# HarborYuan/PolyphonicFormer

Hardware: AMD Instinct MI355X
Metric: frames/sec kernel-update+mask fwd, 1024x2048 N=153 S=3 (higher is better)
Workload: dtype bf16 (feature planes as given; query side: updator half hi/lo bf16, attention / FFN / towers one fp16 plane; one fp16 plane of dynamic kernels, fp16 logits); 1 GPU; cfg2: KernelUpdateIterHead.simple_test_mask_preds, 1024x2048, stride-8 128x256, N=153, S=3, L=133, random-init weights; hip_graph=True, streams=4, feature_input_dtype=bf16, mask_logit_input_dtype=float16, output_dtype=torch.float16, parallelism=frames sharded over 1 GPU(s), no data-path collective

## Files before the change

include/polyhead.h:

```cpp
#ifndef POLYHEAD_H_
#define POLYHEAD_H_

#include <stddef.h>
#include <stdint.h>

#ifdef __cplusplus
extern "C" {
#endif

#define PH_VERSION 100

enum { PH_OK = 0, PH_EINVAL = -1, PH_EUNSUPPORTED = -2, PH_ELAUNCH = -3, PH_EWORKSPACE = -4 };
enum { PH_PREC_BF16 = 1, PH_PREC_BF16_KSPLIT = 2, PH_PREC_SPLIT = 3, PH_PREC_F16 = 5, PH_PREC_BF16_KF16 = 6, PH_PREC_QHYBRID = 7 };
enum { PH_PLANES_C16 = 0x100 };
enum { PH_OUT_F32 = 0, PH_OUT_BF16 = 1, PH_OUT_F16 = 2 };
enum { PH_KERN_BF16_PLANES = 0, PH_KERN_F16 = 1 };
enum { PH_GN_TO_PLANES = 0, PH_GN_UP2_PLANES = 1, PH_GN_ACCUM = 2, PH_GN_TO_NCHW = 3, PH_GN_TO_CPLANES = 4 };
enum { PH_IN_F32_NCHW = 0, PH_IN_PLANES = 1 };

#define PH_C 256
#define PH_HEADS 8

int         ph_version(void);
const char* ph_last_error_string(void);

enum {
    PH_SWITCH_CONV_WGS = 0,
    PH_SWITCH_UP2_WGS = 1,
    PH_SWITCH_QUERY_NRT = 2,
    PH_SWITCH_QUERY_TIMELINE = 3,
    PH_SWITCH_CONV_TILE_ROWS = 4,
    PH_SWITCH_GNSUM_WGS = 5,
    PH_SWITCH_CPLANES_TPW = 6,
    PH_SWITCH_PAN_GENERIC = 7,
    PH_SWITCH_COUNT = 8
};
int ph_set_switch(int id, int value);
int ph_get_switch(int id, int* value);

static inline int64_t ph_hw_padded(int64_t hw) { return (hw + 127) / 128 * 128; }
static inline int     ph_n_padded(int n) { return (n + 31) / 32 * 32; }

int ph_ingest_features(const float* src, uint16_t* planes, int B, int64_t HW, int prec, void* stream);

int ph_binarize(const float* logits, int64_t logits_batch_stride , uint32_t* bits,
                int B, int N, int64_t HW, void* stream);
int ph_binarize_if(const void* logits, int dtype, int64_t logits_batch_stride, uint32_t* bits, int B, int N, int64_t HW,
                   const uint32_t* run_if , void* stream);

int ph_pool(const uint16_t* xplanes, const uint16_t* dplanes, const uint32_t* bits, float* partial,
            int B, int N, int64_t HW, int nsplit, int prec, void* stream);
int ph_pool_rows(const uint16_t* xplanes, const uint16_t* dplanes, const uint32_t* bits, int bits_rows, float* partial,
                 int B, int N, int64_t HW, int nsplit, int prec, void* stream);
int ph_pool_counts(const uint16_t* xplanes, const uint16_t* dplanes, const uint32_t* bits, float* partial, int32_t* pcount,
                   int B, int N, int64_t HW, int nsplit, int prec, void* stream);
int ph_pool_default_nsplit(int B, int64_t HW, int frame_invariant);

enum {
    PH_W_DYN = 0,
    PH_W_INP,
    PH_W_IG,
    PH_W_UG,
    PH_W_FC,
    PH_W_QKV,
    PH_W_OUT,
    PH_W_FFN1,
    PH_W_FFN2,
    PH_W_H0A,
    PH_W_H0B,
    PH_W_CLS,
    PH_W_KERN,
    PH_W_COUNT
};
enum {
    PH_V_DYN_CNT = 0,
    PH_V_DYN_B, PH_V_INP_B, PH_V_IG_B, PH_V_UG_B,
    PH_V_LN_IG_G, PH_V_LN_IG_B,
    PH_V_LN_UG_G, PH_V_LN_UG_B,
    PH_V_LN_PO_G, PH_V_LN_PO_B,
    PH_V_LN_IO_G, PH_V_LN_IO_B,
    PH_V_FC_B, PH_V_LN_FC_G, PH_V_LN_FC_B,
    PH_V_QKV_B, PH_V_OUT_B, PH_V_LN_ATT_G, PH_V_LN_ATT_B,
    PH_V_FFN1_B, PH_V_FFN2_B, PH_V_LN_FFN_G, PH_V_LN_FFN_B,
    PH_V_LN_H0A_G, PH_V_LN_H0A_B, PH_V_LN_H0B_G, PH_V_LN_H0B_B,
    PH_V_CLS_B, PH_V_KERN_B,
    PH_V_COUNT
};
typedef struct {
    int64_t w[2][PH_W_COUNT];
    int64_t v[2][PH_V_COUNT];
    int64_t wb_plane_elems;
    int32_t ffn_dim;
    int32_t num_classes;
} ph_stage_layout;

enum { PH_QUERY_PRE = 1, PH_QUERY_POST = 2, PH_QUERY_BOTH = 3, PH_QUERY_WIDE = 0x100 };
size_t ph_query_workspace_bytes(int B, int N, int prec);
size_t ph_query_workspace_updator_offset(int B, int N, int prec);
int ph_query_stage(const float* partial, int nsplit, const uint32_t* bits,
                   const float* k_in, const float* q_in,
                   const uint16_t* wb, const float* wf, const ph_stage_layout* layout,
                   float* obj, float* dobj, float* cls, int cls_sigmoid ,
                   uint16_t* kern, float* kbias,
                   void* workspace, size_t workspace_bytes,
                   int B, int N, int64_t HW, int prec ,
                   int kern_format ,
                   int phases, void* stream);
int ph_query_stage_counts(const float* partial, int nsplit, const uint32_t* bits, const int32_t* pcount, const float* k_in,
                          const float* q_in, const uint16_t* wb, const float* wf, const ph_stage_layout* layout,
                          float* obj, float* dobj, float* cls, int cls_sigmoid, uint16_t* kern, float* kbias,
                          void* workspace, size_t workspace_bytes, int B, int N, int64_t HW, int prec, int kern_format,
                          int phases, void* stream);

int ph_dynconv(const uint16_t* planes, const uint16_t* kern, int64_t kern_plane_stride, int64_t kern_batch_stride,
               const float* kbias, int64_t kbias_batch_stride, uint32_t* bits_out, void* logits_out, int out_dtype,
               int64_t out_batch_stride, int B, int N, int64_t HW, int prec, void* stream);

int ph_upsample2x(const void* src, void* dst, int dtype, int64_t planes , int H, int W, void* stream);

int ph_dynconv_up2_supported(int N, int H, int W, int prec, int out_dtype);
int ph_dynconv_up2(const uint16_t* planes, const uint16_t* kern, int64_t kern_batch_stride, const float* kbias,
                   int64_t kbias_batch_stride, void* logits_out , void* up_out, int out_dtype, int B, int N, int H,
                   int W, int prec, void* stream);
int ph_dynconv_up2_wgs(const uint16_t* planes, const uint16_t* kern, int64_t kern_batch_stride, const float* kbias,
                       int64_t kbias_batch_stride, void* logits_out , void* up_out, int out_dtype, int B, int N, int H,
                       int W, int prec, int workgroups, void* stream);

int ph_dynconv_poolx_supported(int N, int prec);
int ph_dynconv_poolx(const uint16_t* planes, const uint16_t* kern, int64_t kern_batch_stride, const float* kbias,
                     int64_t kbias_batch_stride, uint32_t* bits_out, float* partial, int nsplit, int B, int N, int64_t HW, int prec,
                     void* stream);

size_t ph_khead_workspace_bytes(int B, int64_t HW, int groups);
int ph_khead_conv_gn(const float* f0, const float* f1, const float* f2, const uint16_t* wplanes,
                     const float* gn_affine, int groups, float eps,
                     uint16_t* loc_planes, uint16_t* sem_planes, uint16_t* x_planes, uint16_t* dfe_planes,
                     float* x_f32 , float* dfe_f32 ,
                     void* workspace, size_t workspace_bytes, int B, int64_t HW, int prec, void* stream);
int ph_khead_fused(const void* f0, const void* f1, const void* f2, const uint16_t* wplanes,
                   const float* gn_affine, int groups, float eps,
                   const uint16_t* w2_init, int n_init, const uint16_t* w2_seg, const float* bias_seg, int n_seg,
                   const uint16_t* w2_dd, const float* bias_dd, int stuff_lo, int n_stuff,
                   uint16_t* x_planes, uint16_t* dfe_planes, float* x_f32 , float* dfe_f32 ,
                   float* mask_preds, float* seg_preds, float* depth_pred,
                   void* workspace, size_t workspace_bytes, int B, int64_t HW, int prec, int input_format, void* stream);
int ph_khead_fused_if(const void* f0, const void* f1, const void* f2, const uint16_t* wplanes,
                      const float* gn_affine, int groups, float eps,
                      const uint16_t* w2_init, int n_init, const uint16_t* w2_seg, const float* bias_seg, int n_seg,
                      const uint16_t* w2_dd, const float* bias_dd, int stuff_lo, int n_stuff,
                      uint16_t* x_planes, uint16_t* dfe_planes, float* x_f32 , float* dfe_f32 ,
                      void* mask_preds, void* seg_preds, void* depth_pred, int logits_dtype, const uint32_t* run_if ,
                      void* workspace, size_t workspace_bytes, int B, int64_t HW, int prec, int input_format, void* stream);
int ph_khead_onepass_supported(int B, int64_t HW, int groups, int prec, int input_format);
size_t ph_khead_onepass_workspace_bytes(int B, int64_t HW);
int ph_khead_onepass(const void* f0, const void* f1, const void* f2, const uint16_t* conv_frags,
                     const float* gn_affine, int groups, float eps,
                     const uint16_t* w2_init, int n_init, const uint16_t* w2_seg, const float* bias_seg, int n_seg,
                     const uint16_t* w2_dd, const float* bias_dd, int stuff_lo, int n_stuff,
                     uint16_t* x_planes, uint16_t* dfe_planes, float* x_f32 , float* dfe_f32 ,
                     void* mask_preds, void* seg_preds, void* depth_pred, int out_dtype,
                     uint32_t* bits , int bits_rows,
                     void* workspace, size_t workspace_bytes, int B, int64_t HW, int prec, int input_format, void* stream);
int ph_khead_onepass_status(const void* workspace, int B, void* stream);
int ph_khead_onepass_timeouts(const void* workspace, int B, int64_t HW, void* stream);
void ph_khead_onepass_set_timeout_us(int microseconds );
void ph_khead_onepass_set_timeline(void* buf);
int ph_khead_proposals(const float* partial, int nsplit, const float* w_init ,
                       const float* w_stuff , float* proposal_feats,
                       int B, int n_thing_queries, int n_stuff, void* stream);

int64_t ph_match_record_floats(int N, int G);
int ph_match_nsplit(int64_t HW, int B);
int ph_match_sums(const float* logits, const float* gt, const float* valid, float* partial, int B, int N, int G,
                  int64_t HW, void* stream);

int ph_mask_loss_sums(const float* pred, const float* target, const float* weight, const int32_t* pos_rows, int P, int64_t HW,
                      int nsplit, double* out, void* stream);
int ph_mask_loss_grad(const float* pred, const float* target, const float* weight, const int32_t* pos_rows, int P, int64_t HW,
                      const float* coef, float* grad, void* stream);
int ph_rank_loss_blocks(int64_t HW);
int ph_rank_loss_sum(const float* pred, const int32_t* rank_target, int B, int N, int64_t HW, int ignore_index, double* out,
                     void* stream);
int ph_rank_loss_grad(const float* pred, const int32_t* rank_target, int B, int N, int64_t HW, int ignore_index, float scale,
                      float* grad, void* stream);
int ph_depth_loss_blocks(int64_t total);
int ph_depth_loss_sums(const float* pred, const float* target, const float* weight, int64_t total, int depth_mode, double* out,
                       void* stream);
int ph_depth_loss_grad(const float* pred, const float* target, const float* weight, int64_t total, int depth_mode, float c0,
                       float c1, float c2, float c3, float* grad, void* stream);
int ph_focal_loss_blocks(int64_t total);
int ph_focal_loss_sum(const float* pred, const int64_t* labels, const float* weight, int64_t R, int L, float gamma, float alpha,
                      double* out, void* stream);
int ph_focal_loss_grad(const float* pred, const int64_t* labels, const float* weight, int64_t R, int L, float gamma, float alpha,
                       float scale, float* grad, void* stream);
int ph_seg_focal_sum(const float* pred, const int32_t* target, int B, int L, int64_t HW, float gamma, float alpha, double* out,
                     void* stream);
int ph_seg_focal_grad(const float* pred, const int32_t* target, int B, int L, int64_t HW, float gamma, float alpha, float scale,
                      float* grad, void* stream);

int ph_rank_target(const float* mask_targets, const uint8_t* pos, int B, int N, int64_t HW, int ignore_index, int32_t* out,
                   void* stream);
int ph_seg_target(const float* sem_seg, const int64_t* sem_cls, int S, const float* pos_masks, const int64_t* pos_labels, int P,
                  int L, int64_t HW, int64_t* out, void* stream);

int ph_depth_cost_sums(const float* depth_logits, const float* gt_depth, const float* gt_masks, int N, int G, int64_t HW,
                       int depth_mode, float eps, float* out, float* nvalid, void* stream);

int ph_rows_x_map(const float* A, int64_t a_batch_stride, int lda, int Mpad, int M, int K, const float* X, float* Y, int B, int64_t HW,
                  int binarize_x, void* stream);
int ph_map_x_map_t_nsplit(int B, int M, int64_t HW);
int ph_map_x_map_t(const float* G, const float* X, float* partial, float* out, int B, int M, int K, int64_t HW, int nsplit,
                  int binarize_g, void* stream);
int ph_upsample2x_bwd(const float* grad_out, float* grad_in, int64_t planes, int H, int W, void* stream);
int ph_rows_x_map_ex(const float* A, int64_t a_batch_stride, int lda, int Mpad, int M, int K, const float* X, float* Y, int B,
                     int64_t HW, int binarize_x, const float* bias, const float* add, void* stream);
int ph_map_x_map_t_ex(const float* G, const float* X, float* partial, float* out, int B, int M, int K, int64_t HW, int nsplit,
                      int binarize_g, float* rs_partial, float* rowsum, int sum_batch, void* stream);
int ph_conv3x3_taps(const float* W, float* taps, int M, int K, int transpose, int flip, int to_weight, void* stream);
int ph_conv3x3_train(const float* taps, int M, int K, const float* X, float* Y, int B, int Hi, int Wi, int Ho, int Wo, int stride,
                     int mode, void* stream);
int ph_conv3x3_wgrad(const float* dY, const float* X, float* partial, float* taps_out, int B, int M, int K, int Hi, int Wi, int Ho,
                     int Wo, int stride, int nsplit, void* stream);
int ph_gn_train_nsplit(int64_t HW, int cpg);
int ph_gn_train_bwd_nsplit(int64_t HW);
int ph_gn_train_fwd(const float* y, const float* gamma, const float* beta, int groups, float eps, const float* add, float* out,
                    float* out_sum, float* stats, double* partial, int B, int C, int64_t HW, void* stream);
int ph_gn_train_bwd(const float* y, const float* stats, const float* gamma, const float* beta, int groups, const float* dyA,
                    const float* dyB, float* dx, float* dgamma, float* dbeta, double* partial, int B, int C, int64_t HW, void* stream);
int ph_hard_count(const float* logits, float* out, int64_t rows, int64_t HW, void* stream);
int ph_map_x_map_t_wide_nsplit(int B, int M, int K, int64_t HW);
int ph_map_x_map_t_wide(const float* G, const float* X, float* partial, float* out, int B, int M, int K, int64_t HW, int nsplit,
                        float* rs_partial, float* rowsum, int sum_batch, void* stream);
int ph_nearest_up_add(float* fine, const float* coarse, int64_t planes, int H, int W, int Hc, int Wc, void* stream);
int ph_nearest_up_add_bwd(const float* g_fine, float* g_coarse, int64_t planes, int H, int W, int Hc, int Wc, int accumulate,
                          void* stream);
int ph_nchw_bias_add(float* y, const float* bias, int B, int C, int64_t HW, void* stream);
int ph_nchw_channel_sums_nsplit(int64_t HW);
int ph_nchw_channel_sums(const float* g, double* partial, float* out, int B, int C, int64_t HW, void* stream);

typedef struct {
    int32_t B, N, L, P, depth_rows, seg_L, has_rank, ignore, depth_mode;
    int64_t HW;
    float lw_mask, lw_dice, dice_eps, lw_rank, lw_depth, dw_si, dw_sq, dw_abs, lw_cls, cls_gamma, cls_alpha, cls_avg, lw_seg, seg_gamma,
        seg_alpha;
} ph_loss_cfg;
size_t ph_train_losses_scratch_bytes(const ph_loss_cfg* cfg);
int ph_train_losses(const ph_loss_cfg* cfg, const float* mask_pred, const float* cls_score, const float* depth_pred,
                    const float* seg_pred, const int32_t* pos_rows, const uint8_t* pos_u8, const int64_t* tptr, const int64_t* wptr,
                    const int32_t* dstart, const int64_t* dit_t, const int64_t* dit_w, const float* dit_s, const int64_t* labels,
                    const float* label_w, const int32_t* sstart, const int64_t* sit_m, const int32_t* sit_l, float* losses,
                    float* g_mask, float* g_cls, float* g_depth, float* g_seg, void* scratch, size_t scratch_bytes, void* stream);

int ph_gemm32(const float* A, int lda, int kcA, const float* B, int ldb, int kcB, float* C, int ldc, int M, int N, int K, int ksplit,
              const float* bias, void* stream);
#define PH_QTRAIN_NPARAM 44
size_t ph_qtrain_saved_floats(int B, int N, int L, int F);
size_t ph_qtrain_scratch_floats(int B, int N, int L, int F);
int ph_qtrain_forward(const float* const* params, const float* pooled, const float* cnt, const float* k, const float* q, float* cls,
                      float* kern, float* kbias, float* obj, float* saved, int B, int N, int L, int F, void* stream);
int ph_qtrain_backward(const float* const* params, const float* pooled, const float* cnt, const float* k, const float* q,
                       const float* saved, const float* g_cls, const float* g_kern, const float* g_kbias, const float* g_obj,
                       float* const* grads, float* g_pooled, float* g_k, float* g_q, float* scratch, int B, int N, int L, int F,
                       void* stream);

int ph_panoptic_select(const float* cls_scores, int64_t cls_batch_stride, int B, int N, int L, int num_proposals,
                       int num_thing_classes, int max_per_img, int32_t* q_idx, int32_t* labels, float* scores,
                       int64_t out_batch_stride, void* stream);
int ph_panoptic_activate(const void* mask_up, const void* depth_up, int dtype, const float* depth_init_up,
                         const int32_t* q_idx, int K, int h2, int w2, int depth_mode ,
                         float* act_mask, float* act_depth, float* act_depth0, void* stream);
int ph_panoptic_argmax(const float* act_mask, const float* scores, int K, const int32_t* geom, int from_probs,
                       int32_t* ids, int32_t* counts , void* stream);
int ph_panoptic_paste(const int32_t* ids, const int32_t* newid, const float* act_depth, const float* act_depth0,
                      const int32_t* geom, int from_probs, int32_t* pan, float* depth_basic, float* depth_final,
                      void* stream);

int ph_panoptic_accept(const int32_t* labels, const float* scores, const int32_t* counts , int64_t in_batch_stride, int B,
                       int K, int num_thing_classes, double instance_score_thr, double overlap_thr, int32_t* newid,
                       int64_t newid_batch_stride, int32_t* nseg, int32_t* seg , int64_t rec_batch_stride, void* stream);
int ph_panoptic_activate_batch(const void* mask_up, const void* depth_up, int dtype, const float* depth_init_up,
                               const int32_t* q_idx, int64_t q_batch_stride, int B, int N, int K, int h2, int w2, int depth_mode,
                               float* act_mask, float* act_depth, float* act_depth0, void* stream);
int ph_panoptic_argmax_batch(const float* act_mask, const float* scores, int64_t scores_batch_stride, int B, int K,
                             const int32_t* geom, int from_probs, int generic_only, int32_t* ids, int32_t* counts,
                             int64_t counts_batch_stride, void* stream);
int ph_panoptic_paste_batch(const int32_t* ids, const int32_t* newid, int64_t newid_batch_stride, const float* act_depth,
                            const float* act_depth0, int B, int K, const int32_t* geom, int from_probs, int32_t* pan,
                            float* depth_basic, float* depth_final, void* stream);
size_t ph_panoptic_merge_workspace_bytes(int B, int K, int h2, int w2, const int32_t* geom);
int ph_panoptic_merge(const float* cls , const void* mask_up, const void* depth_up, int dtype,
                      const float* depth_init_up , int B, int N, int L, int num_proposals, int num_thing_classes,
                      int max_per_img, int h2, int w2, const int32_t* geom , int depth_mode,
                      double instance_score_thr, double overlap_thr, void* workspace, size_t workspace_bytes,
                      int32_t* pan , float* depth_basic, float* depth_final,
                      int32_t* seg_records , void* stream);

size_t ph_segment_boxes_workspace_bytes(int nseg);
int ph_segment_boxes(const int32_t* pan, int H, int W, int nseg, float* rois, float* ext_boxes,
                     void* workspace, size_t workspace_bytes, void* stream);
int ph_roi_align_fpn(const float* const* feats, const int32_t* hw, const float* scales, int nlev, const float* rois,
                     int n, float finest_scale, uint16_t* out_cl, float* out_f32 , int prec, void* stream);
int ph_gemm_rows(const uint16_t* X, const uint16_t* Wp, int64_t w_plane_elems, const float* bias , int relu,
                 float* Yf , uint16_t* Yp , int M, int N, int K, int prec, void* stream);
int ph_im2col7(const uint16_t* in, uint16_t* out, int n, int prec, void* stream);
size_t ph_gemm_rows_workspace_bytes(int M, int N, int K);
int ph_gemm_rows_splitk(const uint16_t* X, int im2col7, const uint16_t* Wp, int64_t w_plane_elems, const float* bias ,
                        int relu, float* Yf , uint16_t* Yp , int M, int N, int K, int prec,
                        void* workspace, size_t workspace_bytes, void* stream);
size_t ph_track_affinity_workspace_bytes(int n, int m);
int ph_track_affinity(const float* emb, const int32_t* labels, const float* memo_emb, const int32_t* memo_labels, int n, int m,
                      int metric, int with_cats, float* score, void* workspace, size_t workspace_bytes, void* stream);
int ph_gn_relu_cl(const float* y, const float* gamma, const float* beta, int groups, float eps, uint16_t* out, int n,
                  int prec, void* stream);

int ph_nhwc_ingest(const float* src, const float* add , uint16_t* dst, int B, int64_t HW, int prec, void* stream);
size_t ph_conv_nhwc_partial_floats(int B, int Ho, int Wo);
int ph_conv_nhwc_workgroups_b(int ksize, int stride, int Ho, int Wo, int prec, int B);
int ph_conv_nhwc(const uint16_t* X, const uint16_t* Wp, int64_t w_plane_elems, float* Y, float* partial, int ksize, int stride,
                 int B, int H, int W, int prec, void* stream);
int ph_gn_finalize(const float* partial, float* stats, int nwg, int groups, int64_t HW, float eps, int B, void* stream);
int ph_gn_sum_planes(const float* const* ys, const float* const* stats, const float* const* gammas, const float* const* betas,
                     int nlev, int groups, uint16_t* planes, int B, int64_t HW, int prec, void* stream);
size_t ph_neck_out_convs_workspace_bytes(int B, int64_t HW, int groups);
int ph_neck_out_convs(const uint16_t* in_planes, int in_channels_last, const uint16_t* wplanes, const float* gn_affine, int groups,
                      float eps, uint16_t* out_planes0, uint16_t* out_planes1, uint16_t* out_planes2, float* out_f32_0,
                      float* out_f32_1, float* out_f32_2, void* workspace, size_t workspace_bytes, int B, int64_t HW, int prec,
                      void* stream);
int ph_gn_apply(const float* y, const float* stats , const float* gamma, const float* beta, int groups, int mode,
                int accumulate, uint16_t* planes , float* outf , int B, int H, int W, int prec,
                void* stream);

int ph_fpn_lateral(const void* x, int x_dtype, const uint16_t* Wp, int64_t w_plane_elems, const float* bias,
                   const uint16_t* coarse , int Hc, int Wc, uint16_t* out, int B, int K, int H, int W, int prec,
                   void* stream);
int ph_fpn_output(const float* y, const float* bias, float* out, int B, int64_t HW, void* stream);
int ph_fpn_output_planes(const float* y, const float* bias, const float* add , uint16_t* planes,
                         float* out_f32 , int B, int64_t HW, int prec , void* stream);

typedef struct {
    float init_score_thr, obj_score_thr, match_score_thr, memo_momentum, one_minus_momentum, nms_conf_thr, nms_backdrop_iou_thr,
        nms_class_iou_thr;
    int32_t memo_tracklet_frames, memo_backdrop_frames, with_cats, metric;
} ph_tracker_cfg;
typedef struct ph_tracker ph_tracker;
size_t ph_tracker_device_bytes(int capacity, int max_dets);
ph_tracker* ph_tracker_create(const ph_tracker_cfg* cfg, void* device_mem, size_t device_bytes, int capacity, int max_dets);
void ph_tracker_destroy(ph_tracker* t);
void ph_tracker_reset(ph_tracker* t);
int64_t ph_tracker_num_tracklets(const ph_tracker* t);
int ph_tracker_rows(const ph_tracker* t);
void ph_tracker_debug_times(const ph_tracker* t, double* out6);
int ph_tracker_match(ph_tracker* t, const float* boxes, const int64_t* labels, const float* embeds_dev, int n, int64_t frame_id,
                     int32_t* kept_out, int64_t* ids_out, void* stream);
int ph_tracker_match_frames(ph_tracker* t, const float* boxes, const int64_t* labels, const float* const* embeds_dev, const int32_t* counts,
                            int nframes, int64_t first_frame_id, int32_t* kept_out, int64_t* ids_out, int32_t* kept_counts, void* stream);

enum { PH_MODE_FP32 = 0, PH_MODE_MIXED = 1, PH_MODE_MIXED16 = 2, PH_MODE_FP16 = 3, PH_MODE_BF16 = 4 };
enum { PH_KNOB_AUTO = 0, PH_KNOB_ON = 1, PH_KNOB_OFF = 2, PH_KNOB_WHERE_SUPPORTED = 3 };
typedef struct {
    int32_t B, N, H, W;
    int32_t S;
    int32_t L;
    int32_t F;
    int32_t mode;
    int32_t out_dtype;
    int32_t frame_invariant;
    int32_t query_full_split;
    int32_t shares_gpu;
    int32_t poolx;
    int32_t fused_up;
    int32_t nsplit;
    int32_t nsplit_px;
    int32_t up2_wgs;
} ph_decode_cfg;

typedef struct {
    int32_t nsplit, nsplit_px, poolx, fused_up;
    int32_t up2_workgroups;
    int32_t feat_prec, query_prec, conv_prec, kern_format;
    int32_t feat_planes;
} ph_decode_geometry;

enum { PH_FEAT_F32 = 0, PH_FEAT_16 = 1, PH_FEAT_PLANES = 2 };
typedef struct {
    int32_t feat_format;
    int32_t m0_dtype;
    const void* x;
    const void* depth_feats;
    const float* k0;
    const float* q0;
    const void* m0;
    const uint32_t* bits;
    float* obj;
    float* dobj;
    float* cls;
    void* mask;
    void* mask_up;
    void* depth_up;
    void* depth;
// ... 452 lines not shown
```

polyphonicformer_amd/_lib.py:

```python
import contextlib
import ctypes as C
import os

import torch

from . import knobs

HERE = os.path.dirname(os.path.abspath(__file__))
LIB_PATH = os.path.join(HERE, "libpolyhead.so")
if knobs.get("PH_ALT_LIB"):
    LIB_PATH = os.path.abspath(knobs.get("PH_ALT_LIB"))

PH_PREC_BF16, PH_PREC_BF16_KSPLIT, PH_PREC_SPLIT, PH_PREC_F16, PH_PREC_BF16_KF16, PH_PREC_QHYBRID = 1, 2, 3, 5, 6, 7
PH_PLANES_C16 = 0x100
PH_QUERY_WIDE = 0x100
PH_OUT_F32, PH_OUT_BF16, PH_OUT_F16 = 0, 1, 2
PH_KERN_BF16_PLANES, PH_KERN_F16 = 0, 1
PH_GN_TO_PLANES, PH_GN_UP2_PLANES, PH_GN_ACCUM, PH_GN_TO_NCHW, PH_GN_TO_CPLANES = 0, 1, 2, 3, 4
PH_IN_F32_NCHW, PH_IN_PLANES = 0, 1

SWITCHES = ("conv_wgs", "up2_wgs", "query_nrt", "query_timeline", "conv_tile_rows", "gnsum_wgs", "cplanes_tpw", "pan_generic")

W_NAMES = ["DYN", "INP", "IG", "UG", "FC", "QKV", "OUT", "FFN1", "FFN2", "H0A", "H0B", "CLS", "KERN"]
V_NAMES = ["DYN_CNT", "DYN_B", "INP_B", "IG_B", "UG_B", "LN_IG_G", "LN_IG_B", "LN_UG_G", "LN_UG_B",
           "LN_PO_G", "LN_PO_B", "LN_IO_G", "LN_IO_B", "FC_B", "LN_FC_G", "LN_FC_B", "QKV_B", "OUT_B",
           "LN_ATT_G", "LN_ATT_B", "FFN1_B", "FFN2_B", "LN_FFN_G", "LN_FFN_B", "LN_H0A_G", "LN_H0A_B",
           "LN_H0B_G", "LN_H0B_B", "CLS_B", "KERN_B"]
W_IDX = {n: i for i, n in enumerate(W_NAMES)}
V_IDX = {n: i for i, n in enumerate(V_NAMES)}


class StageLayout(C.Structure):
    _fields_ = [("w", (C.c_int64 * len(W_NAMES)) * 2), ("v", (C.c_int64 * len(V_NAMES)) * 2),
                ("wb_plane_elems", C.c_int64), ("ffn_dim", C.c_int32), ("num_classes", C.c_int32)]


PH_MODE = {"fp32": 0, "split": 0, "mixed": 1, "mixed16": 2, "fp16": 3, "bf16": 4}
PH_KNOB_AUTO, PH_KNOB_ON, PH_KNOB_OFF, PH_KNOB_WHERE_SUPPORTED = 0, 1, 2, 3
PH_FEAT_F32, PH_FEAT_16, PH_FEAT_PLANES = 0, 1, 2
PH_DECODE_NPARAMS = 83


class DecodeCfg(C.Structure):
    _fields_ = [(n, C.c_int32) for n in ("B", "N", "H", "W", "S", "L", "F", "mode", "out_dtype", "frame_invariant", "query_full_split",
                                          "shares_gpu", "poolx", "fused_up", "nsplit", "nsplit_px", "up2_wgs")]


class DecodeGeometry(C.Structure):
    _fields_ = [(n, C.c_int32) for n in ("nsplit", "nsplit_px", "poolx", "fused_up", "up2_workgroups", "feat_prec", "query_prec",
                                          "conv_prec", "kern_format", "feat_planes")]


class DecodeIO(C.Structure):
    _fields_ = [("feat_format", C.c_int32), ("m0_dtype", C.c_int32)] + \
        [(n, C.c_void_p) for n in ("x", "depth_feats", "k0", "q0", "m0", "bits", "obj", "dobj", "cls", "mask", "mask_up", "depth_up",
                                   "depth")]


PH_KHEAD_NPARAMS = 14
KPACK_PIECES = ("wplanes", "gn", "init_planes", "seg_planes", "dd_planes", "seg_bias", "dd_bias", "init_frag", "seg_frag", "dd_frag",
                "conv_frag", "w_init_f32", "w_seg_f32", "w_dd_f32")
PH_KPACK_COUNT = len(KPACK_PIECES)


class KheadCfg(C.Structure):
    _fields_ = [(n, C.c_int32) for n in ("B", "H", "W", "num_proposals", "num_classes", "num_thing_classes", "cat_stuff", "groups",
                                          "mode", "logit_dtype", "emit_f32", "frame_invariant", "onepass", "nsplit")]


class KheadLayout(C.Structure):
    _fields_ = [("offset", C.c_uint64 * PH_KPACK_COUNT), ("bytes", C.c_uint64 * PH_KPACK_COUNT)]


class KheadGeometry(C.Structure):
    _fields_ = [(n, C.c_int32) for n in ("onepass", "nsplit", "N", "Npad", "HWp", "P", "prec", "n_stuff")]


class KheadIO(C.Structure):
    _fields_ = [("input_format", C.c_int32), ("reserved", C.c_int32)] + \
        [(n, C.c_void_p) for n in ("f0", "f1", "f2", "xp", "dp", "bits", "x_f32", "dfe_f32", "mask_preds", "seg_preds", "depth_pred",
                                   "proposal", "depth_proposal")]


PH_NECK_NPARAMS = 30
PH_NECK_NCONVS = 10
PH_NPACK_OUTS_W, PH_NPACK_OUTS_GN, PH_NPACK_COUNT = 30, 31, 32


class NeckCfg(C.Structure):
    _fields_ = [("B", C.c_int32), ("h", C.c_int32 * 4), ("w", C.c_int32 * 4)] + \
        [(n, C.c_int32) for n in ("groups", "mode", "num_outs", "pos_level", "emit_planes", "emit_f32", "fused_out", "c16",
                                  "tower_buffers")] + [("eps", C.c_float)]


class NeckLayout(C.Structure):
    _fields_ = [("offset", C.c_uint64 * PH_NPACK_COUNT), ("bytes", C.c_uint64 * PH_NPACK_COUNT)]


class NeckGeometry(C.Structure):
    _fields_ = [(n, C.c_int32) for n in ("Ho", "Wo", "HWp", "P", "prec", "fused_out", "c16", "tower_buffers", "nconvs")] + \
        [("tile_rows", C.c_int32 * PH_NECK_NCONVS)]


class NeckIO(C.Structure):
    _fields_ = [("feats", C.c_void_p * 4), ("posenc", C.c_void_p), ("out_planes", C.c_void_p * 3), ("out_f32", C.c_void_p * 3)]


PH_FPN_NPARAMS = PH_FPACK_COUNT = 16


class FpnCfg(C.Structure):
    _fields_ = [("B", C.c_int32), ("k", C.c_int32 * 4), ("h", C.c_int32 * 4), ("w", C.c_int32 * 4)] + \
        [(n, C.c_int32) for n in ("mode", "x_dtype", "emit_f32", "emit_planes")]


class FpnLayout(C.Structure):
    _fields_ = [("offset", C.c_uint64 * PH_FPACK_COUNT), ("bytes", C.c_uint64 * PH_FPACK_COUNT)]


class FpnGeometry(C.Structure):
    _fields_ = [("P", C.c_int32), ("prec", C.c_int32), ("tile_rows", C.c_int32 * 4)]


class FpnIO(C.Structure):
    _fields_ = [("stages", C.c_void_p * 4), ("out_f32", C.c_void_p * 4), ("out_planes", C.c_void_p * 4), ("planes_layout", C.c_int32 * 4),
                ("add", C.c_void_p * 4)]


PH_TRACK_MAX_CONVS = 8
PH_TPACK_FC, PH_TPACK_FC_B, PH_TPACK_EMB, PH_TPACK_EMB_B, PH_TPACK_COUNT = 24, 25, 26, 27, 28


class TrackCfg(C.Structure):
    _fields_ = [(n, C.c_int32) for n in ("num_convs", "fc_out_channels", "embed_channels", "groups", "prec")] + [("eps", C.c_float)]


class TrackLayout(C.Structure):
    _fields_ = [("offset", C.c_uint64 * PH_TPACK_COUNT), ("bytes", C.c_uint64 * PH_TPACK_COUNT)]


class AssocCfg(C.Structure):
    _fields_ = [(n, C.c_int32) for n in ("B", "Ho", "Wo", "K", "max_things", "num_thing_classes", "num_stuff_classes", "nlev")] + \
        [("h", C.c_int32 * 4), ("w", C.c_int32 * 4), ("inv_stride", C.c_float * 4), ("finest_scale", C.c_float), ("track", TrackCfg)]


class AssocGeometry(C.Structure):
    _fields_ = [(n, C.c_int32) for n in ("things_words", "P", "conv_splits", "conv_steps", "fc_splits", "fc_steps", "emb_splits",
                                          "emb_steps", "vec8", "reserved")] + [(n, C.c_uint64) for n in ("staging_bytes", "rois_offset", "roi_planes_offset")]


class AssocIO(C.Structure):
    _fields_ = [("pan", C.c_void_p), ("seg_records", C.c_void_p), ("levels", C.c_void_p * 4), ("level_stride", C.c_int64 * 4),
                ("sem_out", C.c_void_p), ("things_out", C.c_void_p), ("embeds_out", C.c_void_p), ("roi_planes", C.c_void_p)]


PH_DTRK_OK, PH_DTRK_EPOOL, PH_DTRK_EREFUSED, PH_DTRK_ECOUNT = 0, 1, 2, 3
DTRK_STATUS = ("matched", "num_tracklets", "rows", "error", "refused_frame", "frame_id", "free", "frames_seen")
PH_DTRK_ST_WORDS = len(DTRK_STATUS)


class TrackerCfg(C.Structure):
    _fields_ = [(n, C.c_float) for n in ("init_score_thr", "obj_score_thr", "match_score_thr", "memo_momentum", "one_minus_momentum",
                                         "nms_conf_thr", "nms_backdrop_iou_thr", "nms_class_iou_thr")] + \
        [(n, C.c_int32) for n in ("memo_tracklet_frames", "memo_backdrop_frames", "with_cats", "metric")]


class DtrackerLayout(C.Structure):
    _fields_ = [(n, C.c_uint64) for n in ("pool", "trk_id", "trk_seen", "trk_label", "trk_slot", "trk_box", "bd_count", "bd_label", "bd_slot",
                                          "bd_box", "free_stack", "status", "workspace", "total_bytes")] + \
        [(n, C.c_int32) for n in ("capacity", "max_dets", "generations", "reserved")]


class DtrackerIO(C.Structure):
    _fields_ = [("boxes", C.c_void_p), ("box_stride", C.c_int64), ("labels", C.c_void_p), ("label_stride", C.c_int64),
                ("counts", C.c_void_p), ("count_stride", C.c_int64), ("refuse", C.c_void_p), ("refuse_stride", C.c_int64),
                ("embeds", C.c_void_p), ("embed_stride", C.c_int64), ("kept_out", C.c_void_p), ("ids_out", C.c_void_p),
                ("kept_counts", C.c_void_p)]


PH_DVPQ_MAX_THR = 8


class DvpqCfg(C.Structure):
    _fields_ = [(n, C.c_int32) for n in ("B", "H", "W", "capacity", "nthr")] + [("thr", C.c_float * PH_DVPQ_MAX_THR)]


class DvpqIO(C.Structure):
    _fields_ = [(n, C.c_void_p) for n in ("pred_panseg", "pred_sem", "pred_track", "pred_depth", "gt_panseg", "gt_depth", "table_out",
                                          "depth_out")]


PH_ASSIGN_MAX, PH_ASSIGN_MAX_B, PH_ASSIGN_GT_WORDS = 256, 64, 8
PH_ASSIGN_OK, PH_ASSIGN_ENONFINITE, PH_ASSIGN_ESOLVE = 0, 1, 2
PH_EUNSUPPORTED = -2
ASSIGN_SECTIONS = ("tptr", "wptr", "labels", "pos_u8", "pos_rows", "dstart", "dit_t", "dit_w", "dit_s", "label_w", "sstart", "sit_m", "sit_l")


class AssignCfg(C.Structure):
    _fields_ = [(n, C.c_int32) for n in ("B", "Np", "N", "L", "n_thing", "n_stuff", "roi", "has_sem", "has_depth")] + \
        [("pos_weight", C.c_float), ("HW", C.c_int64)]


class AssignLayout(C.Structure):
    _fields_ = [(n, C.c_uint64) for n in ASSIGN_SECTIONS + ("total_bytes",)] + \
        [(n, C.c_int64) for n in ("P", "depth_items", "seg_items", "depth_rows")]


class LossCfg(C.Structure):
    _fields_ = [(n, C.c_int32) for n in ("B", "N", "L", "P", "depth_rows", "seg_L", "has_rank", "ignore", "depth_mode")] + \
        [("HW", C.c_int64)] + \
        [(n, C.c_float) for n in ("lw_mask", "lw_dice", "dice_eps", "lw_rank", "lw_depth", "dw_si", "dw_sq", "dw_abs", "lw_cls",
                                  "cls_gamma", "cls_alpha", "cls_avg", "lw_seg", "seg_gamma", "seg_alpha")]


PH_TRACK_LOSS_MAX_ROIS, PH_TRACK_LOSS_MAX_PAIRS = 128, 64


PH_GTBOX_MAX_FRAMES, PH_GTBOX_BILINEAR, PH_GTBOX_NEAREST = 64, 0, 1
PH_GTPREP_MAX_FRAMES, PH_GTPREP_MAX_SEGMENTS = 64, 254
PH_GTSEG_MAX_KEYS, PH_GTSEG_ROW_WORDS, PH_GTSEG_TABLE_WORDS = 262144, 6, 1 + 254 * 6
PH_GTSEG_I32, PH_GTSEG_U16 = 0, 1
PH_GTSEG_ETOOMANY, PH_GTSEG_EUNMAPPED, PH_GTSEG_EOUTSIDE = 1, 2, 4
PH_EINVAL, PH_EWORKSPACE = -1, -4
PH_IMGPREP_MAX_FRAMES = 64
PH_IMG_NCHW, PH_IMG_NHWC = 0, 1


class TrackLossCfg(C.Structure):
    _fields_ = [("pairs", C.c_int32), ("E", C.c_int32), ("lw_track", C.c_float), ("lw_aux", C.c_float), ("neg_pos_ub", C.c_int32),
                ("pos_margin", C.c_float), ("neg_margin", C.c_float), ("hard_mining", C.c_int32)]


PH_OPTIM_CHUNK, PH_OPTIM_MAX_TENSORS = 4096, 4096
PH_OPTIM_SKIP_NONFINITE, PH_OPTIM_ZERO_GRADS = 1, 2
PH_OPTIM_OK, PH_OPTIM_ENONFINITE = 0, 1


class OptimTensor(C.Structure):
    _fields_ = [(n, C.c_void_p) for n in ("p", "g", "m", "v")] + [("n", C.c_int64), ("lr", C.c_double), ("weight_decay", C.c_double),
                                                                  ("first_item", C.c_int64)]


class OptimCfg(C.Structure):
    _fields_ = [(n, C.c_double) for n in ("beta1", "beta2", "eps", "max_norm")] + [("flags", C.c_int32), ("max_blocks", C.c_int32)]


class OptimState(C.Structure):
    _fields_ = [("step", C.c_int64), ("skipped", C.c_int64), ("status", C.c_int32), ("skip", C.c_int32)] + \
        [(n, C.c_float) for n in ("grad_norm", "clip_coef", "bias1", "bias2_sqrt")]


STRUCTS = {"ph_stage_layout": StageLayout, "ph_decode_cfg": DecodeCfg, "ph_decode_geometry": DecodeGeometry, "ph_decode_io": DecodeIO,
           "ph_khead_cfg": KheadCfg, "ph_khead_layout": KheadLayout, "ph_khead_geometry": KheadGeometry, "ph_khead_io": KheadIO,
           "ph_neck_cfg": NeckCfg, "ph_neck_layout": NeckLayout, "ph_neck_geometry": NeckGeometry, "ph_neck_io": NeckIO,
           "ph_fpn_cfg": FpnCfg, "ph_fpn_layout": FpnLayout, "ph_fpn_geometry": FpnGeometry, "ph_fpn_io": FpnIO,
           "ph_track_cfg": TrackCfg, "ph_track_layout": TrackLayout, "ph_assoc_cfg": AssocCfg, "ph_assoc_geometry": AssocGeometry,
           "ph_assoc_io": AssocIO, "ph_tracker_cfg": TrackerCfg, "ph_dtracker_layout": DtrackerLayout, "ph_dtracker_io": DtrackerIO,
           "ph_dvpq_cfg": DvpqCfg, "ph_dvpq_io": DvpqIO, "ph_assign_cfg": AssignCfg, "ph_assign_layout": AssignLayout,
           "ph_loss_cfg": LossCfg, "ph_track_loss_cfg": TrackLossCfg, "ph_optim_tensor": OptimTensor, "ph_optim_cfg": OptimCfg,
           "ph_optim_state": OptimState}

_P, _I, _L, _Z = C.c_void_p, C.c_int, C.c_int64, C.c_size_t
SIGNATURES = {
    "ph_version": (C.c_int, []),
    "ph_last_error_string": (C.c_char_p, []),
    "ph_set_switch": (C.c_int, [_I, _I]),
    "ph_get_switch": (C.c_int, [_I, C.POINTER(C.c_int)]),
    "ph_ingest_features": (C.c_int, [_P, _P, _I, _L, _I, _P]),
    "ph_binarize": (C.c_int, [_P, _L, _P, _I, _I, _L, _P]),
    "ph_pool": (C.c_int, [_P, _P, _P, _P, _I, _I, _L, _I, _I, _P]),
    "ph_pool_rows": (C.c_int, [_P, _P, _P, _I, _P, _I, _I, _L, _I, _I, _P]),
    "ph_pool_counts": (C.c_int, [_P, _P, _P, _P, _P, _I, _I, _L, _I, _I, _P]),
    "ph_pool_default_nsplit": (C.c_int, [_I, _L, _I]),
    "ph_query_workspace_bytes": (C.c_size_t, [_I, _I, _I]),
    "ph_query_stage": (C.c_int, [_P, _I, _P, _P, _P, _P, _P, C.POINTER(StageLayout), _P, _P, _P, _I, _P, _P,
                                 _P, _Z, _I, _I, _L, _I, _I, _I, _P]),
    "ph_query_stage_counts": (C.c_int, [_P, _I, _P, _P, _P, _P, _P, _P, C.POINTER(StageLayout), _P, _P, _P, _I, _P, _P,
                                        _P, _Z, _I, _I, _L, _I, _I, _I, _P]),
    "ph_query_workspace_updator_offset": (C.c_size_t, [_I, _I, _I]),
    "ph_dynconv": (C.c_int, [_P, _P, _L, _L, _P, _L, _P, _P, _I, _L, _I, _I, _L, _I, _P]),
    "ph_khead_workspace_bytes": (C.c_size_t, [_I, _L, _I]),
    "ph_khead_conv_gn": (C.c_int, [_P, _P, _P, _P, _P, _I, C.c_float, _P, _P, _P, _P, _P, _P, _P, _Z, _I, _L, _I, _P]),
    "ph_khead_fused": (C.c_int, [_P, _P, _P, _P, _P, _I, C.c_float, _P, _I, _P, _P, _I, _P, _P, _I, _I, _P, _P, _P, _P,
                                 _P, _P, _P, _P, _Z, _I, _L, _I, _I, _P]),
    "ph_khead_onepass_supported": (C.c_int, [_I, _L, _I, _I, _I]),
    "ph_khead_onepass_workspace_bytes": (C.c_size_t, [_I, _L]),
    "ph_khead_onepass": (C.c_int, [_P, _P, _P, _P, _P, _I, C.c_float, _P, _I, _P, _P, _I, _P, _P, _I, _I, _P, _P, _P, _P,
                                   _P, _P, _P, _I, _P, _I, _P, _Z, _I, _L, _I, _I, _P]),
    "ph_khead_onepass_status": (C.c_int, [_P, _I, _P]),
    "ph_khead_onepass_timeouts": (C.c_int, [_P, _I, _L, _P]),
    "ph_khead_onepass_set_timeout_us": (None, [_I]),
    "ph_khead_fused_if": (C.c_int, [_P, _P, _P, _P, _P, _I, C.c_float, _P, _I, _P, _P, _I, _P, _P, _I, _I, _P, _P, _P, _P,
                                    _P, _P, _P, _I, _P, _P, _Z, _I, _L, _I, _I, _P]),
    "ph_binarize_if": (C.c_int, [_P, _I, _L, _P, _I, _I, _L, _P, _P]),
    "ph_selftest_hog": (C.c_int, [_I, _I, _I, _P, _P]),
    "ph_khead_onepass_set_timeline": (None, [_P]),
    "ph_khead_proposals": (C.c_int, [_P, _I, _P, _P, _P, _I, _I, _I, _P]),
    "ph_match_record_floats": (C.c_int64, [_I, _I]),
    "ph_match_nsplit": (C.c_int, [_L, _I]),
    "ph_match_sums": (C.c_int, [_P, _P, _P, _P, _I, _I, _I, _L, _P]),
    "ph_upsample2x": (C.c_int, [_P, _P, _I, _L, _I, _I, _P]),
    "ph_dynconv_poolx_supported": (C.c_int, [_I, _I]),
    "ph_dynconv_poolx": (C.c_int, [_P, _P, _L, _P, _L, _P, _P, _I, _I, _I, _L, _I, _P]),
    "ph_dynconv_up2_supported": (C.c_int, [_I, _I, _I, _I, _I]),
    "ph_dynconv_up2": (C.c_int, [_P, _P, _L, _P, _L, _P, _P, _I, _I, _I, _I, _I, _I, _P]),
    "ph_dynconv_up2_wgs": (C.c_int, [_P, _P, _L, _P, _L, _P, _P, _I, _I, _I, _I, _I, _I, _I, _P]),
    "ph_mask_loss_sums": (C.c_int, [_P, _P, _P, _P, _I, _L, _I, _P, _P]),
    "ph_mask_loss_grad": (C.c_int, [_P, _P, _P, _P, _I, _L, _P, _P, _P]),
    "ph_rank_loss_blocks": (C.c_int, [_L]),
    "ph_rank_loss_sum": (C.c_int, [_P, _P, _I, _I, _L, _I, _P, _P]),
    "ph_rank_loss_grad": (C.c_int, [_P, _P, _I, _I, _L, _I, C.c_float, _P, _P]),
    "ph_depth_loss_blocks": (C.c_int, [_L]),
    "ph_depth_loss_sums": (C.c_int, [_P, _P, _P, _L, _I, _P, _P]),
    "ph_depth_loss_grad": (C.c_int, [_P, _P, _P, _L, _I, C.c_float, C.c_float, C.c_float, C.c_float, _P, _P]),
    "ph_focal_loss_blocks": (C.c_int, [_L]),
    "ph_focal_loss_sum": (C.c_int, [_P, _P, _P, _L, _I, C.c_float, C.c_float, _P, _P]),
    "ph_focal_loss_grad": (C.c_int, [_P, _P, _P, _L, _I, C.c_float, C.c_float, C.c_float, _P, _P]),
    "ph_seg_focal_sum": (C.c_int, [_P, _P, _I, _I, _L, C.c_float, C.c_float, _P, _P]),
    "ph_seg_focal_grad": (C.c_int, [_P, _P, _I, _I, _L, C.c_float, C.c_float, C.c_float, _P, _P]),
    "ph_rank_target": (C.c_int, [_P, _P, _I, _I, _L, _I, _P, _P]),
    "ph_seg_target": (C.c_int, [_P, _P, _I, _P, _P, _I, _I, _L, _P, _P]),
    "ph_depth_cost_sums": (C.c_int, [_P, _P, _P, _I, _I, _L, _I, C.c_float, _P, _P, _P]),
    "ph_rows_x_map": (C.c_int, [_P, _L, _I, _I, _I, _I, _P, _P, _I, _L, _I, _P]),
    "ph_map_x_map_t_nsplit": (C.c_int, [_I, _I, _L]),
    "ph_map_x_map_t": (C.c_int, [_P, _P, _P, _P, _I, _I, _I, _L, _I, _I, _P]),
    "ph_upsample2x_bwd": (C.c_int, [_P, _P, _L, _I, _I, _P]),
    "ph_rows_x_map_ex": (C.c_int, [_P, _L, _I, _I, _I, _I, _P, _P, _I, _L, _I, _P, _P, _P]),
    "ph_map_x_map_t_ex": (C.c_int, [_P, _P, _P, _P, _I, _I, _I, _L, _I, _I, _P, _P, _I, _P]),
    "ph_conv3x3_taps": (C.c_int, [_P, _P, _I, _I, _I, _I, _I, _P]),
    "ph_conv3x3_train": (C.c_int, [_P, _I, _I, _P, _P, _I, _I, _I, _I, _I, _I, _I, _P]),
    "ph_conv3x3_wgrad": (C.c_int, [_P, _P, _P, _P, _I, _I, _I, _I, _I, _I, _I, _I, _I, _P]),
    "ph_gn_train_nsplit": (C.c_int, [_L, _I]),
    "ph_gn_train_bwd_nsplit": (C.c_int, [_L]),
    "ph_gn_train_fwd": (C.c_int, [_P, _P, _P, _I, C.c_float, _P, _P, _P, _P, _P, _I, _I, _L, _P]),
    "ph_gn_train_bwd": (C.c_int, [_P, _P, _P, _P, _I, _P, _P, _P, _P, _P, _P, _I, _I, _L, _P]),
    "ph_hard_count": (C.c_int, [_P, _P, _L, _L, _P]),
    "ph_map_x_map_t_wide_nsplit": (C.c_int, [_I, _I, _I, _L]),
    "ph_map_x_map_t_wide": (C.c_int, [_P, _P, _P, _P, _I, _I, _I, _L, _I, _P, _P, _I, _P]),
    "ph_nearest_up_add": (C.c_int, [_P, _P, _L, _I, _I, _I, _I, _P]),
    "ph_nearest_up_add_bwd": (C.c_int, [_P, _P, _L, _I, _I, _I, _I, _I, _P]),
    "ph_nchw_bias_add": (C.c_int, [_P, _P, _I, _I, _L, _P]),
    "ph_nchw_channel_sums_nsplit": (C.c_int, [_L]),
    "ph_nchw_channel_sums": (C.c_int, [_P, _P, _P, _I, _I, _L, _P]),
    "ph_train_losses_scratch_bytes": (C.c_size_t, [_P]),
    "ph_train_losses": (C.c_int, [_P] * 24 + [_Z, _P]),
    "ph_gemm32": (C.c_int, [_P, _I, _I, _P, _I, _I, _P, _I, _I, _I, _I, _I, _P, _P]),
    "ph_qtrain_saved_floats": (C.c_size_t, [_I, _I, _I, _I]),
    "ph_qtrain_scratch_floats": (C.c_size_t, [_I, _I, _I, _I]),
    "ph_qtrain_forward": (C.c_int, [_P, _P, _P, _P, _P, _P, _P, _P, _P, _P, _I, _I, _I, _I, _P]),
    "ph_qtrain_backward": (C.c_int, [_P, _P, _P, _P, _P, _P, _P, _P, _P, _P, _P, _P, _P, _P, _P, _I, _I, _I, _I, _P]),
    "ph_panoptic_select": (C.c_int, [_P, _L, _I, _I, _I, _I, _I, _I, _P, _P, _P, _L, _P]),
    "ph_panoptic_activate": (C.c_int, [_P, _P, _I, _P, _P, _I, _I, _I, _I, _P, _P, _P, _P]),
    "ph_panoptic_argmax": (C.c_int, [_P, _P, _I, C.POINTER(C.c_int32), _I, _P, _P, _P]),
    "ph_panoptic_paste": (C.c_int, [_P, _P, _P, _P, C.POINTER(C.c_int32), _I, _P, _P, _P, _P]),
    "ph_panoptic_accept": (C.c_int, [_P, _P, _P, _L, _I, _I, _I, C.c_double, C.c_double, _P, _L, _P, _P, _L, _P]),
    "ph_panoptic_activate_batch": (C.c_int, [_P, _P, _I, _P, _P, _L, _I, _I, _I, _I, _I, _I, _P, _P, _P, _P]),
    "ph_panoptic_argmax_batch": (C.c_int, [_P, _P, _L, _I, _I, C.POINTER(C.c_int32), _I, _I, _P, _P, _L, _P]),
    "ph_panoptic_paste_batch": (C.c_int, [_P, _P, _L, _P, _P, _I, _I, C.POINTER(C.c_int32), _I, _P, _P, _P, _P]),
    "ph_panoptic_merge_workspace_bytes": (C.c_size_t, [_I, _I, _I, _I, C.POINTER(C.c_int32)]),
    "ph_panoptic_merge": (C.c_int, [_P, _P, _P, _I, _P, _I, _I, _I, _I, _I, _I, _I, _I, C.POINTER(C.c_int32), _I, C.c_double,
                                    C.c_double, _P, _Z, _P, _P, _P, _P, _P]),
    "ph_segment_boxes_workspace_bytes": (C.c_size_t, [_I]),
    "ph_segment_boxes": (C.c_int, [_P, _I, _I, _I, _P, _P, _P, _Z, _P]),
    "ph_roi_align_fpn": (C.c_int, [C.POINTER(C.c_void_p), C.POINTER(C.c_int32), C.POINTER(C.c_float), _I, _P, _I, C.c_float,
                                   _P, _P, _I, _P]),
    "ph_gemm_rows": (C.c_int, [_P, _P, _L, _P, _I, _P, _P, _I, _I, _I, _I, _P]),
    "ph_track_affinity_workspace_bytes": (C.c_size_t, [_I, _I]),
    "ph_track_affinity": (C.c_int, [_P, _P, _P, _P, _I, _I, _I, _I, _P, _P, _Z, _P]),
    "ph_im2col7": (C.c_int, [_P, _P, _I, _I, _P]),
    "ph_gemm_rows_workspace_bytes": (C.c_size_t, [_I, _I, _I]),
    "ph_gemm_rows_splitk": (C.c_int, [_P, _I, _P, _L, _P, _I, _P, _P, _I, _I, _I, _I, _P, _Z, _P]),
    "ph_gn_relu_cl": (C.c_int, [_P, _P, _P, _I, C.c_float, _P, _I, _I, _P]),
    "ph_nhwc_ingest": (C.c_int, [_P, _P, _P, _I, _L, _I, _P]),
    "ph_conv_nhwc_partial_floats": (C.c_size_t, [_I, _I, _I]),
    "ph_conv_nhwc_workgroups_b": (C.c_int, [_I, _I, _I, _I, _I, _I]),
    "ph_conv_nhwc": (C.c_int, [_P, _P, _L, _P, _P, _I, _I, _I, _I, _I, _I, _P]),
    "ph_gn_finalize": (C.c_int, [_P, _P, _I, _I, _L, C.c_float, _I, _P]),
    "ph_gn_sum_planes": (C.c_int, [C.POINTER(C.c_void_p), C.POINTER(C.c_void_p), C.POINTER(C.c_void_p), C.POINTER(C.c_void_p),
                                   _I, _I, _P, _I, _L, _I, _P]),
    "ph_neck_out_convs_workspace_bytes": (C.c_size_t, [_I, _L, _I]),
    "ph_neck_out_convs": (C.c_int, [_P, _I, _P, _P, _I, C.c_float, _P, _P, _P, _P, _P, _P, _P, _Z, _I, _L, _I, _P]),
    "ph_gn_apply": (C.c_int, [_P, _P, _P, _P, _I, _I, _I, _P, _P, _I, _I, _I, _I, _P]),
    "ph_fpn_lateral": (C.c_int, [_P, _I, _P, _L, _P, _P, _I, _I, _P, _I, _I, _I, _I, _I, _P]),
    "ph_fpn_output": (C.c_int, [_P, _P, _P, _I, _L, _P]),
    "ph_fpn_output_planes": (C.c_int, [_P, _P, _P, _P, _P, _I, _L, _I, _P]),
    "ph_tracker_device_bytes": (C.c_size_t, [_I, _I]),
    "ph_tracker_create": (C.c_void_p, [_P, _P, _Z, _I, _I]),
    "ph_tracker_destroy": (None, [_P]),
    "ph_tracker_reset": (None, [_P]),
    "ph_tracker_num_tracklets": (C.c_int64, [_P]),
    "ph_tracker_rows": (C.c_int, [_P]),
    "ph_tracker_debug_times": (None, [_P, _P]),
    "ph_tracker_match": (C.c_int, [_P, _P, _P, _P, _I, _L, _P, _P, _P]),
    "ph_tracker_match_frames": (C.c_int, [_P, _P, _P, _P, _P, _I, _L, _P, _P, _P, _P]),
    "ph_decode_param_name": (C.c_char_p, [_I]),
    "ph_decode_param_numel": (C.c_int64, [C.POINTER(DecodeCfg), _I]),
    "ph_decode_pack_bytes": (C.c_size_t, [C.POINTER(DecodeCfg)]),
    "ph_decode_pack_layout": (C.c_int, [C.POINTER(DecodeCfg), C.POINTER(StageLayout), C.POINTER(C.c_size_t)]),
    "ph_decode_pack_stage": (C.c_int, [C.POINTER(DecodeCfg), C.POINTER(C.c_void_p), _P, _P]),
    "ph_decode_workspace_bytes": (C.c_size_t, [C.POINTER(DecodeCfg)]),
    "ph_decode_create": (C.c_int, [C.POINTER(DecodeCfg), C.POINTER(C.c_void_p), _P, _Z, C.POINTER(C.c_void_p)]),
    "ph_decode_info": (C.c_int, [_P, C.POINTER(DecodeGeometry)]),
    "ph_decode_geometry_of": (C.c_int, [C.POINTER(DecodeCfg), C.POINTER(DecodeGeometry)]),
    "ph_decode_destroy": (None, [_P]),
    "ph_decode_run": (C.c_int, [_P, C.POINTER(DecodeIO), _P]),
    "ph_khead_param_name": (C.c_char_p, [_I]),
    "ph_khead_param_numel": (C.c_int64, [C.POINTER(KheadCfg), _I]),
    "ph_khead_pack_bytes": (C.c_size_t, [C.POINTER(KheadCfg)]),
    "ph_khead_pack_layout": (C.c_int, [C.POINTER(KheadCfg), C.POINTER(KheadLayout)]),
    "ph_khead_pack": (C.c_int, [C.POINTER(KheadCfg), C.POINTER(C.c_void_p), _P, _P]),
    "ph_khead_plan_workspace_bytes": (C.c_size_t, [C.POINTER(KheadCfg)]),
    "ph_khead_plan_create": (C.c_int, [C.POINTER(KheadCfg), _P, _P, _Z, C.POINTER(C.c_void_p)]),
    "ph_khead_plan_info": (C.c_int, [_P, C.POINTER(KheadGeometry)]),
    "ph_khead_geometry_of": (C.c_int, [C.POINTER(KheadCfg), C.POINTER(KheadGeometry)]),
    "ph_khead_plan_destroy": (None, [_P]),
    "ph_khead_plan_run": (C.c_int, [_P, C.POINTER(KheadIO), _P]),
    "ph_khead_plan_status": (C.c_int, [_P, _P]),
    "ph_khead_plan_timeouts": (C.c_int, [_P, _P]),
    "ph_neck_param_name": (C.c_char_p, [_I]),
    "ph_neck_param_numel": (C.c_int64, [C.POINTER(NeckCfg), _I]),
    "ph_neck_pack_bytes": (C.c_size_t, [C.POINTER(NeckCfg)]),
    "ph_neck_pack_layout": (C.c_int, [C.POINTER(NeckCfg), C.POINTER(NeckLayout)]),
    "ph_neck_pack": (C.c_int, [C.POINTER(NeckCfg), C.POINTER(C.c_void_p), _P, _P]),
    "ph_neck_posenc": (C.c_int, [_I, _I, _I, C.c_double, C.c_double, C.c_double, _P, _P]),
    "ph_neck_plan_workspace_bytes": (C.c_size_t, [C.POINTER(NeckCfg)]),
    "ph_neck_plan_create": (C.c_int, [C.POINTER(NeckCfg), _P, _P, _Z, C.POINTER(C.c_void_p)]),
    "ph_neck_plan_info": (C.c_int, [_P, C.POINTER(NeckGeometry)]),
    "ph_neck_geometry_of": (C.c_int, [C.POINTER(NeckCfg), C.POINTER(NeckGeometry)]),
    "ph_neck_plan_destroy": (None, [_P]),
    "ph_neck_plan_run": (C.c_int, [_P, C.POINTER(NeckIO), _P]),
    "ph_neck_plan_run_level": (C.c_int, [_P, _I, C.POINTER(NeckIO), _P]),
    "ph_neck_plan_run_outputs": (C.c_int, [_P, C.POINTER(NeckIO), _P]),
    "ph_neck_plan_level_input": (C.c_int, [_P, _I, C.POINTER(C.c_void_p), C.POINTER(C.c_int32)]),
    "ph_neck_plan_run_level_planes": (C.c_int, [_P, _I, _P]),
    "ph_fpn_param_name": (C.c_char_p, [_I]),
    "ph_fpn_param_numel": (C.c_int64, [C.POINTER(FpnCfg), _I]),
    "ph_fpn_pack_bytes": (C.c_size_t, [C.POINTER(FpnCfg)]),
    "ph_fpn_pack_layout": (C.c_int, [C.POINTER(FpnCfg), C.POINTER(FpnLayout)]),
    "ph_fpn_pack": (C.c_int, [C.POINTER(FpnCfg), C.POINTER(C.c_void_p), _P, _P]),
    "ph_fpn_plan_workspace_bytes": (C.c_size_t, [C.POINTER(FpnCfg)]),
    "ph_fpn_plan_create": (C.c_int, [C.POINTER(FpnCfg), _P, _P, _Z, C.POINTER(C.c_void_p)]),
    "ph_fpn_plan_info": (C.c_int, [_P, C.POINTER(FpnGeometry)]),
    "ph_fpn_geometry_of": (C.c_int, [C.POINTER(FpnCfg), C.POINTER(FpnGeometry)]),
    "ph_fpn_plan_destroy": (None, [_P]),
    "ph_fpn_plan_run_laterals": (C.c_int, [_P, C.POINTER(FpnIO), _P]),
    "ph_fpn_plan_run_output": (C.c_int, [_P, _I, C.POINTER(FpnIO), _P]),
    "ph_fpn_plan_run": (C.c_int, [_P, C.POINTER(FpnIO), _P]),
    "ph_track_param_name": (C.c_char_p, [C.POINTER(TrackCfg), _I]),
    "ph_track_param_numel": (C.c_int64, [C.POINTER(TrackCfg), _I]),
    "ph_track_pack_bytes": (C.c_size_t, [C.POINTER(TrackCfg)]),
    "ph_track_pack_layout": (C.c_int, [C.POINTER(TrackCfg), C.POINTER(TrackLayout)]),
    "ph_track_pack": (C.c_int, [C.POINTER(TrackCfg), C.POINTER(C.c_void_p), _P, _P]),
    "ph_assoc_plan_workspace_bytes": (C.c_size_t, [C.POINTER(AssocCfg)]),
    "ph_assoc_plan_create": (C.c_int, [C.POINTER(AssocCfg), _P, _P, _Z, C.POINTER(C.c_void_p)]),
    "ph_assoc_plan_info": (C.c_int, [_P, C.POINTER(AssocGeometry)]),
    "ph_assoc_plan_destroy": (None, [_P]),
    "ph_assoc_plan_run": (C.c_int, [_P, C.POINTER(AssocIO), _P]),
    "ph_assoc_plan_match": (C.c_int, [_P, _P, _P, _P, _P, _P, _Z, _L, _P, _P, _P]),
    "ph_dtracker_device_bytes": (C.c_size_t, [C.POINTER(TrackerCfg), _I, _I]),
    "ph_dtracker_create": (C.c_int, [C.POINTER(TrackerCfg), _P, _Z, _I, _I, C.POINTER(C.c_void_p)]),
    "ph_dtracker_destroy": (None, [_P]),
    "ph_dtracker_reset": (C.c_int, [_P, _L, _P]),
    "ph_dtracker_get_layout": (C.c_int, [_P, C.POINTER(DtrackerLayout)]),
    "ph_dtracker_run": (C.c_int, [_P, C.POINTER(DtrackerIO), _I, _P]),
    "ph_assoc_plan_track": (C.c_int, [_P, _P, _P, _P, _P, _P, _P, _P]),
    "ph_dtracker_bank_bytes": (C.c_size_t, [C.POINTER(TrackerCfg), _I, _I, _I]),
    "ph_dtracker_bank_create": (C.c_int, [C.POINTER(TrackerCfg), _P, _Z, _I, _I, _I, C.POINTER(C.c_void_p)]),
    "ph_dtracker_get_streams": (C.c_int, [_P, C.POINTER(C.c_int), C.POINTER(C.c_uint64)]),
    "ph_dtracker_reset_streams": (C.c_int, [_P, _L, _L, _P]),
    "ph_dtracker_step": (C.c_int, [_P, C.POINTER(DtrackerIO), _P, _P]),
    "ph_assoc_plan_track_streams": (C.c_int, [_P, _P, _P, _P, _P, _P, _P, _P, _P]),
    "ph_dvpq_workspace_bytes": (C.c_size_t, [C.POINTER(DvpqCfg)]),
    "ph_dvpq_frames": (C.c_int, [C.POINTER(DvpqCfg), C.POINTER(DvpqIO), _P, _Z, _P]),
    "ph_assign_desc_layout": (C.c_int, [C.POINTER(AssignCfg), _P, _P, _P, C.POINTER(AssignLayout)]),
    "ph_assign_solve": (C.c_int, [_P, _I, _I, _I, _P, _L, _P, _P, _P]),
    "ph_assign_desc": (C.c_int, [C.POINTER(AssignCfg), _P, _P, _P, _P, _I, _P, _L, _P, _P, _P, _Z, _P]),
    "ph_track_loss_scratch_bytes": (C.c_size_t, [C.POINTER(TrackLossCfg), _I, _I]),
    "ph_track_loss": (C.c_int, [C.POINTER(TrackLossCfg), _P, _P, C.POINTER(C.c_int32), C.POINTER(C.c_int32), _P, _P, C.POINTER(C.c_int32),
                                _P, _P, _P, _P, _P, _Z, _P]),
    "ph_roi_align_fpn_bwd": (C.c_int, [_P, C.POINTER(C.c_int32), C.POINTER(C.c_float), _I, _P, _I, C.c_float, C.POINTER(C.c_void_p), _P]),
    "ph_gtmask_boxes_workspace_bytes": (C.c_size_t, [_I, C.POINTER(C.c_int32), _I, _I]),
    "ph_gtmask_boxes": (C.c_int, [C.POINTER(C.c_void_p), C.POINTER(C.c_int32), C.POINTER(C.c_int32), C.POINTER(C.c_int32), _P, _L, _I, _I,
                                  _I, _I, _I, _I, _I, _P, _P, _P, _P, _Z, _P]),
    "ph_gt_prepare": (C.c_int, [_P, _P, C.POINTER(C.c_int32), _P, _I, _I, _I, _I, _I, _I, _I, _I, _I, _I, _P, _P, _P, _P, _P, _P, _P]),
    "ph_gt_segments_workspace_bytes": (C.c_size_t, [_I, _I, _I]),
    "ph_gt_segments": (C.c_int, [_P, _I, _I, _I, _I, C.POINTER(C.c_int32), _I, _I, _I, _I, _P, _P, _P, _Z, _P]),
    "ph_gt_index_maps": (C.c_int, [_P, _I, _P, _I, _I, _I, C.POINTER(C.c_int32), _I, _I, _I, _I, _P, C.POINTER(C.c_int32), _P, _P, _P, _P,
                                   _I, _I, _I, _I, C.c_float, C.c_float, C.POINTER(C.c_float), _P, _P, _P]),
    "ph_image_prepare": (C.c_int, [_P, _I, _I, _I, _P, _P, _P, _P, _I, _I, _I, _I, C.POINTER(C.c_float), C.POINTER(C.c_float), _I, _I, _I,
                                   _P, _P]),
    "ph_optim_workspace_bytes": (C.c_size_t, [_P, _I]),
    "ph_optim_step": (C.c_int, [C.POINTER(OptimCfg), _P, _P, _I, C.c_float, _P, _P, _P, _Z, _P]),
    "ph_optim_zero_grads": (C.c_int, [_P, _P, _I, _I, _P]),
    "ph_selftest_mfma16": (C.c_int, [_P, _P, _P, _P]),
    "ph_selftest_mfma32": (C.c_int, [_P, _P, _P, _P]),
    "ph_selftest_readbw": (C.c_int, [_P, _L, _I, _P, _P]),
    "ph_selftest_trread": (C.c_int, [_P, _P, _P]),
}

_lib = None


class PolyheadError(RuntimeError):
    pass


def load():
    global _lib
    if _lib is not None:
        return _lib
    if not os.path.exists(LIB_PATH):
        raise PolyheadError(
            f"{LIB_PATH} is missing: build it with `python -m polyphonicformer_amd.build` "
            "(needs hipcc, gfx950). There is no fallback path.")
    lib = C.CDLL(LIB_PATH)
    for name, (res, args) in SIGNATURES.items():
        fn = getattr(lib, name)
        fn.restype, fn.argtypes = res, args
    _lib = lib
    return lib


def check(rc, what):
    if rc != 0:
        msg = load().ph_last_error_string()
        raise PolyheadError(f"{what} failed with code {rc}: {msg.decode() if msg else ''}")


@contextlib.contextmanager
def switches(**values):
    lib, old = load(), {}
    try:
        for name, v in values.items():
            i, cur = SWITCHES.index(name), C.c_int()
            check(lib.ph_get_switch(i, cur), "ph_get_switch")
            check(lib.ph_set_switch(i, v), f"ph_set_switch({name}, {v})")
            old[i] = cur.value
        yield
    finally:
        for i, v in old.items():
            check(lib.ph_set_switch(i, v), "ph_set_switch")


def ptr(t):
    return None if t is None else C.c_void_p(t.data_ptr())


def stream_ptr():
    return C.c_void_p(torch._C._cuda_getCurrentRawStream(torch._C._cuda_getDevice()))


def _tree(module):
    c = module.__dict__.get("_ph_tree")
    if c is not None:
        sig = tuple(id(ch) for _, m in c[1] for ch in m._modules.values())
        if sig == c[0]:
            return c[1]
    mods = [(n + "." if n else "", m) for n, m in module.named_modules()]
    module.__dict__["_ph_tree"] = (tuple(id(ch) for _, m in mods for ch in m._modules.values()), mods)
    return mods


def param_versions(module):
    return tuple((id(p), p._version) for _, m in _tree(module) for p in m._parameters.values() if p is not None)


def named_params(module):
    out, seen = {}, set()
    for pre, m in _tree(module):
        for k, p in m._parameters.items():
            if p is not None and id(p) not in seen:
                seen.add(id(p))
                out[pre + k] = p
    return out
```

polyphonicformer_amd/csrc/ph_pool.hip:

```cpp
#include "ph_common.h"

constexpr int POOL_CHUNK = 64;
constexpr int POOL_FT = 128 * POOL_CHUNK;
constexpr int POOL_NBUF = 4;

typedef unsigned u32x4_t __attribute__((ext_vector_type(4)));

__device__ __forceinline__ u32x4_t lds_read128_asm(uint32_t byte_addr) {
    u32x4_t v;
    asm volatile("ds_read_b128 %0, %1" : "=v"(v) : "v"(byte_addr));
    return v;
}
__device__ __forceinline__ uint32_t lds_read32_asm(uint32_t byte_addr) {
    uint32_t v;
    asm volatile("ds_read_b32 %0, %1" : "=v"(v) : "v"(byte_addr));
    return v;
}
__device__ __forceinline__ uint32_t lds_addr(const void* p) { return (uint32_t)(uintptr_t)(PH_LDS const void*)p; }

template <int E> __device__ __forceinline__ uint4 expand8(uint32_t byte) {
    constexpr uint32_t ONE = E == PH_E_F16 ? 0x3C00u : 0x3F80u;
    uint32_t r[4];
#pragma unroll
    for (int p = 0; p < 4; ++p) {
        const uint32_t lo = (byte >> (2 * p)) & 1u, hi = (byte >> (2 * p + 1)) & 1u;
        r[p] = lo * ONE + hi * (ONE << 16);
    }
    return make_uint4(r[0], r[1], r[2], r[3]);
}

__device__ __forceinline__ int pool_swz(int row) { return (row >> 1) & 7; }

template <int PA , int NRT , int E >
__global__ __launch_bounds__(256, 2) void k_pool(const uint16_t* __restrict__ xplanes, const uint16_t* __restrict__ dplanes,
                                              const uint32_t* __restrict__ bits, float* __restrict__ partial,
                                              int B, int64_t HWp, int nsplit, int bits_rows, int32_t* __restrict__ pcount) {
    constexpr int Npad = NRT * 32;
    constexpr int PER_CHUNK = 4 * PA;
    constexpr int NBI2 = (Npad + 63) / 64;
    constexpr int NR64 = NBI2 * 64;
    extern __shared__ __attribute__((aligned(16))) uint16_t lds[];
    uint4* lut = (uint4*)(lds + POOL_NBUF * PA * POOL_FT);
    uint32_t* lbits = (uint32_t*)(lut + 256);

    const int tid = threadIdx.x, lane = tid & 63;
    const int wave = __builtin_amdgcn_readfirstlane(tid >> 6);
    const int split = blockIdx.x, cg = blockIdx.y, b = blockIdx.z;
    const int map = cg >> 1;
    const int ch0 = (cg & 1) * 128;
    const int g = lane >> 5;
    const uint16_t* feat = (map == 0 ? xplanes : dplanes);
    const int64_t plane_stride = (int64_t)B * PH_C * HWp;
    const uint16_t* fbase = feat + ((int64_t)b * PH_C + ch0) * HWp;
    const int64_t words_per_row = HWp / 32;
    const uint32_t* brow = bits + (int64_t)b * bits_rows * words_per_row;

    const int nchunks = (int)(HWp / POOL_CHUNK);
    int c0 = (int)((int64_t)split * nchunks / nsplit), c1 = (int)((int64_t)(split + 1) * nchunks / nsplit);
    c0 &= ~1; c1 = split + 1 == nsplit ? nchunks : (c1 & ~1);
    const bool pair_wave = wave < NBI2;
    auto issue_pair_bits = [&](int c, int gb) {
        if (!pair_wave) return;
        int row = wave * 64 + lane;
        if (row > Npad - 1) row = Npad - 1;
        const uint32_t* src = brow + (int64_t)row * words_per_row + c * 2;
        uint32_t* dst = lbits + gb * (NR64 * 4) + wave * 256;
        __builtin_amdgcn_global_load_lds((const __attribute__((address_space(1))) void*)src, (PH_LDS void*)dst, 16, 0, 0);
    };

    lut[tid] = expand8<E>((uint32_t)tid);

    f32x16_t acc[NRT];
#pragma unroll
    for (int rt = 0; rt < NRT; ++rt)
#pragma unroll
        for (int r = 0; r < 16; ++r) acc[rt][r] = 0.f;
    const bool counting = pcount != nullptr && cg == 0 && wave == 0;
    int pc[NRT];
#pragma unroll
    for (int rt = 0; rt < NRT; ++rt) pc[rt] = 0;

    auto issue_piece = [&](int c, int buf, int k) {
        const int j = wave + 4 * k;
        const int p = j >> 4, jj = j & 15;
        const int row = jj * 8 + (lane >> 3);
        const int q = (lane & 7) ^ pool_swz(row);
        const uint16_t* src = fbase + p * plane_stride + (int64_t)row * HWp + (int64_t)c * POOL_CHUNK + q * 8;
        uint16_t* dst = lds + (buf * PA + p) * POOL_FT + jj * 512;
        __builtin_amdgcn_global_load_lds((const __attribute__((address_space(1))) void*)src, (PH_LDS void*)dst, 16, 0, PH_CPOL_STREAM);
    };
    auto issue_chunk = [&](int c, int buf) {
#pragma unroll
        for (int k = 0; k < PER_CHUNK; ++k) issue_piece(c, buf, k);
    };

    if (c0 < c1) issue_pair_bits(c0, 0);
#pragma unroll
    for (int d = 0; d < POOL_NBUF - 1; ++d)
        if (c0 + d < c1) issue_chunk(c0 + d, d);
    __syncthreads();

    const uint32_t lut_addr = lds_addr(lut);
    const int frow = wave * 32 + (lane & 31);
    int cur = 0;
    for (int c = c0; c < c1; ++c) {
        const int younger = (c1 - 1 - c) < (POOL_NBUF - 2) ? (c1 - 1 - c) : (POOL_NBUF - 2);
        const int pos = (c - c0) & 1;
        const bool extra = pos == 1 && younger >= 1 && pair_wave;
        if (younger >= 2) {
            if (extra) asm volatile("s_waitcnt vmcnt(%0)" ::"n"(8 * PA + 1) : "memory");
            else asm volatile("s_waitcnt vmcnt(%0)" ::"n"(8 * PA) : "memory");
        } else if (younger == 1) {
            if (extra) asm volatile("s_waitcnt vmcnt(%0)" ::"n"(4 * PA + 1) : "memory");
            else asm volatile("s_waitcnt vmcnt(%0)" ::"n"(4 * PA) : "memory");
        } else asm volatile("s_waitcnt vmcnt(0)" ::: "memory");
        __builtin_amdgcn_s_barrier();
        __builtin_amdgcn_sched_barrier(0);
        int nb = cur + POOL_NBUF - 1;
        if (nb >= POOL_NBUF) nb -= POOL_NBUF;
        const bool more = c + POOL_NBUF - 1 < c1;
        const uint32_t ft = lds_addr(lds + cur * PA * POOL_FT);
        const uint32_t wb = lds_addr(lbits + (((c - c0) >> 1) & 1) * (NR64 * 4));
        u32x4_t xf[PA][4];
#pragma unroll
        for (int p = 0; p < PA; ++p)
#pragma unroll
            for (int t = 0; t < 4; ++t)
                xf[p][t] = lds_read128_asm(ft + 2 * (p * POOL_FT + frow * POOL_CHUNK + (((g * 4 + t) ^ pool_swz(frow)) * 8)));
        uint32_t w[NRT];
#pragma unroll
        for (int rt = 0; rt < NRT; ++rt)
            w[rt] = lds_read32_asm(wb + 4 * ((rt * 32 + (lane & 31)) * 4 + pos * 2 + g));
        asm volatile("s_waitcnt lgkmcnt(0)" ::: "memory");
        __builtin_amdgcn_sched_barrier(0);
        if (counting) {
#pragma unroll
            for (int rt = 0; rt < NRT; ++rt) pc[rt] += __popc(w[rt]);
        }
        u32x4_t a[2][4];
#pragma unroll
        for (int t = 0; t < 4; ++t) a[0][t] = lds_read128_asm(lut_addr + (((w[0] >> (8 * t)) & 0xFFu) << 4));
#pragma unroll
        for (int rt = 0; rt < NRT; ++rt) {
            if (rt + 1 < NRT) {
#pragma unroll
                for (int t = 0; t < 4; ++t) a[(rt + 1) & 1][t] = lds_read128_asm(lut_addr + (((w[rt + 1] >> (8 * t)) & 0xFFu) << 4));
                asm volatile("s_waitcnt lgkmcnt(4)" ::: "memory");
            } else {
                asm volatile("s_waitcnt lgkmcnt(0)" ::: "memory");
            }
            __builtin_amdgcn_sched_barrier(0);
#pragma unroll
            for (int t = 0; t < 4; ++t)
#pragma unroll
                for (int p = 0; p < PA; ++p)
                    acc[rt] = mfma32e<E>(__builtin_bit_cast(uint4, a[rt & 1][t]), __builtin_bit_cast(uint4, xf[p][t]), acc[rt]);
            __builtin_amdgcn_sched_barrier(0);
            if (rt == 0 && pos == 0 && c + 2 < c1) issue_pair_bits(c + 2, (((c - c0) >> 1) + 1) & 1);
            if (more) {
#pragma unroll
                for (int k = rt; k < PER_CHUNK; k += NRT) issue_piece(c + POOL_NBUF - 1, nb, k);
            }
            __builtin_amdgcn_sched_barrier(0);
        }
        cur = cur + 1 == POOL_NBUF ? 0 : cur + 1;
    }

    if (counting) {
#pragma unroll
        for (int rt = 0; rt < NRT; ++rt) {
            const int tot = pc[rt] + __shfl_xor(pc[rt], 32);
            if (lane < 32) pcount[((int64_t)b * nsplit + split) * Npad + rt * 32 + lane] = tot;
        }
    }
    float* out = partial + (((int64_t)b * nsplit + split) * Npad) * 512 + map * 256 + ch0 + wave * 32 + (lane & 31);
#pragma unroll
    for (int rt = 0; rt < NRT; ++rt)
#pragma unroll
        for (int r = 0; r < 16; ++r) {
            const int row = rt * 32 + (r & 3) + 8 * (r >> 2) + 4 * g;
            out[(int64_t)row * 512] = acc[rt][r];
        }
}

template <int PA, int NRT, int E>
static void launch_pool(const uint16_t* x, const uint16_t* d, const uint32_t* bits, float* partial, int B, int64_t HWp,
                        int nsplit, int bits_rows, int32_t* pcount, hipStream_t s) {
    const size_t lds = (size_t)POOL_NBUF * PA * POOL_FT * sizeof(uint16_t) + 256 * 16 + (size_t)2 * ((NRT * 32 + 63) / 64) * 64 * 16;
    static const bool once = [&] {
        (void)hipFuncSetAttribute((const void*)k_pool<PA, NRT, E>, hipFuncAttributeMaxDynamicSharedMemorySize, (int)lds);
        return true;
    }();
    (void)once;
    hipLaunchKernelGGL((k_pool<PA, NRT, E>), dim3(nsplit, d ? 4 : 2, B), dim3(256), lds, s, x, d, bits, partial, B, HWp,
                       nsplit, bits_rows, pcount);
}

static int pool_run(const uint16_t* xplanes, const uint16_t* dplanes, const uint32_t* bits, int bits_rows, float* partial, int32_t* pcount,
                    int B, int N, int64_t HW, int nsplit, int prec, void* stream, const char* fn) {
    if (!(xplanes && bits && partial && B > 0 && N > 0 && HW > 0)) { ph_set_error("%s: bad pointer or size", fn); return PH_EINVAL; }
    if (!(prec == PH_PREC_BF16 || prec == PH_PREC_SPLIT || prec == PH_PREC_F16)) {
        ph_set_error("%s: prec must be PH_PREC_BF16, PH_PREC_SPLIT or PH_PREC_F16", fn);
        return PH_EINVAL;
    }
    if (N > 256) { ph_set_error("%s: at most 256 queries", fn); return PH_EINVAL; }
    const int64_t HWp = ph_hw_padded(HW);
    if (!(nsplit >= 1 && nsplit <= HWp / POOL_CHUNK)) { ph_set_error("%s: nsplit out of range", fn); return PH_EINVAL; }
    const int nrt = ph_n_padded(N) / 32;
    if (bits_rows == 0) bits_rows = nrt * 32;
    if (bits_rows < nrt * 32) { ph_set_error("%s: bits_rows must be >= N rounded up to 32", fn); return PH_EINVAL; }
    hipStream_t s = (hipStream_t)stream;
#define PH_POOL_CASE(R)                                                                         \
    case R:                                                                                     \
        if (prec == PH_PREC_BF16) launch_pool<1, R, PH_E_BF16>(xplanes, dplanes, bits, partial, B, HWp, nsplit, bits_rows, pcount, s); \
        else if (prec == PH_PREC_F16) launch_pool<1, R, PH_E_F16>(xplanes, dplanes, bits, partial, B, HWp, nsplit, bits_rows, pcount, s); \
        else launch_pool<2, R, PH_E_BF16>(xplanes, dplanes, bits, partial, B, HWp, nsplit, bits_rows, pcount, s);             \
        break;
    switch (nrt) {
        PH_POOL_CASE(1) PH_POOL_CASE(2) PH_POOL_CASE(3) PH_POOL_CASE(4)
        PH_POOL_CASE(5) PH_POOL_CASE(6) PH_POOL_CASE(7) PH_POOL_CASE(8)
        default: ph_set_error("%s: unsupported N", fn); return PH_EUNSUPPORTED;
    }
#undef PH_POOL_CASE
    PH_CHECK_LAUNCH();
    return PH_OK;
}

extern "C" int ph_pool(const uint16_t* xplanes, const uint16_t* dplanes, const uint32_t* bits, float* partial, int B,
                       int N, int64_t HW, int nsplit, int prec, void* stream) {
    return pool_run(xplanes, dplanes, bits, 0, partial, nullptr, B, N, HW, nsplit, prec, stream, __func__);
}

extern "C" int ph_pool_rows(const uint16_t* xplanes, const uint16_t* dplanes, const uint32_t* bits, int bits_rows, float* partial,
                            int B, int N, int64_t HW, int nsplit, int prec, void* stream) {
    return pool_run(xplanes, dplanes, bits, bits_rows, partial, nullptr, B, N, HW, nsplit, prec, stream, __func__);
}

extern "C" int ph_pool_counts(const uint16_t* xplanes, const uint16_t* dplanes, const uint32_t* bits, float* partial, int32_t* pcount,
                              int B, int N, int64_t HW, int nsplit, int prec, void* stream) {
    if (!pcount) { ph_set_error("ph_pool_counts: null pcount"); return PH_EINVAL; }
    return pool_run(xplanes, dplanes, bits, 0, partial, pcount, B, N, HW, nsplit, prec, stream, __func__);
}

extern "C" int ph_pool_default_nsplit(int B, int64_t HW, int frame_invariant) {
    const int64_t nchunks = ph_hw_padded(HW) / 128;
    int64_t ns = 512 / (4 * (int64_t)(frame_invariant || B < 1 ? 1 : B));
    if (ns > 32) ns = 32;
    if (ns > nchunks) ns = nchunks;
    return ns < 1 ? 1 : (int)ns;
}
```

polyphonicformer_amd/csrc/ph_query.hip:

```cpp
#include <stdlib.h>

#include "ph_common.h"

template <int E> __device__ __forceinline__ uint32_t q_f2e(float x) {
    if constexpr (E == PH_E_F16) return f2h(__builtin_amdgcn_fmed3f(x, -65504.f, 65504.f));
    else return f2bf(x);
}

constexpr int LDA = 264;
constexpr float LN_EPS = 1e-5f;

constexpr int NW = 8;
constexpr int CT = 2;
constexpr int WCOLS = CT * 16;
constexpr int NTHREADS = NW * 64;

template <int NRT> struct Tile { f32x4_t v[NRT][CT]; };


struct QArgs {
    const float* partial; const uint32_t* bits; const float* k_in; const float* q_in;
    const uint16_t* wb; const float* wf;
    float* obj; float* dobj; float* cls; uint16_t* kern; float* kbias;
    uint16_t* Qp; uint16_t* Kp; uint16_t* Vt; float* o1;
    ph_stage_layout lay;
    int nsplit, B, N, Npad, cls_sigmoid, kern_f16;
    int64_t HWp;
    const int32_t* pcount;
};

template <int NRT> __device__ __forceinline__ void tile_zero(f32x4_t (&a)[NRT][CT]) {
#pragma unroll
    for (int rt = 0; rt < NRT; ++rt)
#pragma unroll
        for (int ct = 0; ct < CT; ++ct) a[rt][ct] = f32x4_t{0.f, 0.f, 0.f, 0.f};
}

template <int NRT>
__device__ __forceinline__ void tile_add_bias(Tile<NRT>& t, const float* __restrict__ bias, int wave, int lane) {
#pragma unroll
    for (int ct = 0; ct < CT; ++ct) {
        const float bv = bias[wave * WCOLS + ct * 16 + (lane & 15)];
#pragma unroll
        for (int rt = 0; rt < NRT; ++rt)
#pragma unroll
            for (int r = 0; r < 4; ++r) t.v[rt][ct][r] += bv;
    }
}

template <int PA, int NRT, int E = PH_E_BF16>
__device__ __forceinline__ void tile_to_lds(const Tile<NRT>& t, uint16_t* dst, int plane, int wave, int lane) {
    const int i = lane & 15, g = lane >> 4;
#pragma unroll
    for (int rt = 0; rt < NRT; ++rt)
#pragma unroll
        for (int ct = 0; ct < CT; ++ct)
#pragma unroll
            for (int r = 0; r < 4; ++r) {
                const int off = (rt * 16 + g * 4 + r) * LDA + wave * WCOLS + ct * 16 + i;
                if (PA == 1) dst[off] = (uint16_t)q_f2e<E>(t.v[rt][ct][r]);
                else {
                    uint32_t hi, lo;
                    f2bf_split(t.v[rt][ct][r], hi, lo);
                    dst[off] = (uint16_t)hi;
                    dst[off + plane] = (uint16_t)lo;
                }
            }
}

template <int NRT, int NT>
__device__ __forceinline__ void ln_tiles(Tile<NRT> (&t)[NT], const float* const (&gam)[NT], const float* const (&bet)[NT],
                                         float* red, int wave, int lane) {
    constexpr int ROWS = NRT * 16;
    const int i = lane & 15, g = lane >> 4;
    float mean[NT][NRT][4];
#pragma unroll
    for (int n = 0; n < NT; ++n)
#pragma unroll
        for (int rt = 0; rt < NRT; ++rt)
#pragma unroll
            for (int r = 0; r < 4; ++r) {
                float s = 0.f;
#pragma unroll
                for (int ct = 0; ct < CT; ++ct) s += t[n].v[rt][ct][r];
                s = wave_group16_sum(s);
                if (i == 0) red[((0 * NT + n) * NW + wave) * ROWS + rt * 16 + g * 4 + r] = s;
            }
    __syncthreads();
#pragma unroll
    for (int n = 0; n < NT; ++n)
#pragma unroll
        for (int rt = 0; rt < NRT; ++rt) {
            __builtin_amdgcn_sched_barrier(0);
            asm volatile("" ::: "memory");
#pragma unroll
            for (int r = 0; r < 4; ++r) {
                const float* p = red + (0 * NT + n) * NW * ROWS + rt * 16 + g * 4 + r;
                float tot = 0.f;
#pragma unroll
                for (int w = 0; w < NW; ++w) tot += p[w * ROWS];
                mean[n][rt][r] = tot * (1.f / 256.f);
                float s = 0.f;
#pragma unroll
                for (int ct = 0; ct < CT; ++ct) {
                    const float d = t[n].v[rt][ct][r] - mean[n][rt][r];
                    t[n].v[rt][ct][r] = d;
                    s += d * d;
                }
                s = wave_group16_sum(s);
                if (i == 0) red[((1 * NT + n) * NW + wave) * ROWS + rt * 16 + g * 4 + r] = s;
            }
#pragma unroll
            for (int ct = 0; ct < CT; ++ct) asm volatile("" : "+v"(t[n].v[rt][ct]));
        }
    __syncthreads();
#pragma unroll
    for (int n = 0; n < NT; ++n) {
        float gm[CT], bt[CT];
#pragma unroll
        for (int ct = 0; ct < CT; ++ct) {
            gm[ct] = gam[n][wave * WCOLS + ct * 16 + i];
            bt[ct] = bet[n][wave * WCOLS + ct * 16 + i];
        }
#pragma unroll
        for (int rt = 0; rt < NRT; ++rt) {
            __builtin_amdgcn_sched_barrier(0);
            asm volatile("" ::: "memory");
#pragma unroll
            for (int r = 0; r < 4; ++r) {
                const float* p = red + (1 * NT + n) * NW * ROWS + rt * 16 + g * 4 + r;
                float tot = 0.f;
#pragma unroll
                for (int w = 0; w < NW; ++w) tot += p[w * ROWS];
                const float var = tot * (1.f / 256.f);
                const float rstd = fast_rsqrt(var + LN_EPS);
#pragma unroll
                for (int ct = 0; ct < CT; ++ct) t[n].v[rt][ct][r] = t[n].v[rt][ct][r] * rstd * gm[ct] + bt[ct];
            }
#pragma unroll
            for (int ct = 0; ct < CT; ++ct) asm volatile("" : "+v"(t[n].v[rt][ct]));
        }
    }
}

template <int PA, int NRT, int PART, bool QF16 = false>
__device__ __forceinline__ void store_qkv(const Tile<NRT>& T, const QArgs& a, const float* bias, int64_t qk_base,
                                          int64_t qk_plane, int64_t vt_base, int wave, int lane) {
    const int i = lane & 15, g = lane >> 4;
#pragma unroll
    for (int ct = 0; ct < CT; ++ct) {
        const int col = wave * WCOLS + ct * 16 + i;
        const float bv = bias[col];
#pragma unroll
        for (int rt = 0; rt < NRT; ++rt) {
            uint32_t hi[4], lo[4];
#pragma unroll
            for (int r = 0; r < 4; ++r) {
                float v = T.v[rt][ct][r] + bv;
                if (PART == 0) v *= 0.17677669529663687f;
                if (QF16) { hi[r] = q_f2e<PH_E_F16>(v); lo[r] = 0; }
                else if (PA == 2) f2bf_split(v, hi[r], lo[r]);
                else hi[r] = f2bf(v);
            }
            if (PART < 2) {
                uint16_t* dst = (PART == 0 ? a.Qp : a.Kp) + qk_base + (rt * 16 + g * 4) * 256 + col;
#pragma unroll
                for (int r = 0; r < 4; ++r) {
                    dst[r * 256] = (uint16_t)hi[r];
                    if (PA == 2 && !QF16) dst[qk_plane + r * 256] = (uint16_t)lo[r];
                }
            } else {
                uint16_t* dst = a.Vt + vt_base + (int64_t)col * a.Npad + rt * 16 + g * 4;
                *(uint2*)dst = make_uint2(pack2(hi[0], hi[1]), pack2(hi[2], hi[3]));
                if (PA == 2 && !QF16) *(uint2*)(dst + qk_plane) = make_uint2(pack2(lo[0], lo[1]), pack2(lo[2], lo[3]));
            }
        }
    }
}

constexpr int LDPT = 40;

struct WRef2 { const uint16_t* W; int ct0, ks_total, wks0; };
template <int PA> constexpr int kch() { return PA == 1 ? 4 : 2; }
template <int NCT> struct WStreamF { uint4 f[2][4][NCT]; };
template <int PA, int NCT> using WStream = WStreamF<NCT>;

template <int PA, int NCT>
__device__ __forceinline__ void w_chunk_load(uint4 (&d)[4][NCT], const WRef2& r, int kc, int64_t w_plane, int lane) {
#pragma unroll
    for (int p = 0; p < PA; ++p)
#pragma unroll
        for (int k = 0; k < kch<PA>(); ++k)
#pragma unroll
            for (int ct = 0; ct < NCT; ++ct)
                d[p * kch<PA>() + k][ct] = *(const uint4*)(r.W + p * w_plane + ((int64_t)(r.ct0 + ct) * r.ks_total + r.wks0 + kc * kch<PA>() + k) * 512 + lane * 8);
}
template <int PA, int NCT>
__device__ __forceinline__ void w_prime(WStream<PA, NCT>& ws, const WRef2& r, int64_t w_plane, int lane) {
    w_chunk_load<PA, NCT>(ws.f[0], r, 0, w_plane, lane);
}
struct NoNext { __device__ __forceinline__ void operator()() const {} };

template <int PA, int NRT, int NCT, int NKS, int E = PH_E_BF16, typename Next>
__device__ __forceinline__ void gemm_stream(f32x4_t (&acc)[NRT][NCT], const uint16_t* A, int lda, int a_plane, WStream<PA, NCT>& ws,
                                            const WRef2& r, int64_t w_plane, int lane, Next next) {
    constexpr int KCH = kch<PA>(), NCH = NKS / KCH;
    static_assert(NKS % KCH == 0 && NCH % 2 == 0, "a call is an even number of chunks");
    const int i = lane & 15, g = lane >> 4;
    __builtin_amdgcn_sched_barrier(0);
#pragma unroll
    for (int kc = 0; kc < NCH; ++kc) {
        if (kc + 1 < NCH) w_chunk_load<PA, NCT>(ws.f[(kc + 1) & 1], r, kc + 1, w_plane, lane);
        else next();
        __builtin_amdgcn_sched_barrier(0);
#pragma unroll
        for (int k = 0; k < KCH; ++k) {
            uint4 a[PA][NRT];
#pragma unroll
            for (int p = 0; p < PA; ++p)
#pragma unroll
                for (int rt = 0; rt < NRT; ++rt)
                    a[p][rt] = *(const uint4*)(A + p * a_plane + (rt * 16 + i) * lda + (kc * KCH + k) * 32 + g * 8);
#pragma unroll
            for (int ct = 0; ct < NCT; ++ct)
#pragma unroll
                for (int rt = 0; rt < NRT; ++rt) {
                    acc[rt][ct] = mfma16e<E>(a[0][rt], ws.f[kc & 1][k][ct], acc[rt][ct]);
                    if (PA == 2) {
                        acc[rt][ct] = mfma16(a[0][rt], ws.f[kc & 1][(PA - 1) * KCH + k][ct], acc[rt][ct]);
                        acc[rt][ct] = mfma16(a[PA - 1][rt], ws.f[kc & 1][k][ct], acc[rt][ct]);
                    }
                }
        }
        __builtin_amdgcn_sched_barrier(0);
    }
}

template <int PA, int NRT, int NCT, int E = PH_E_BF16>
__device__ __forceinline__ void frag_to_lds(const f32x4_t (&t)[NRT][NCT], uint16_t* dst, int ld, int plane, int col0, int lane) {
    const int i = lane & 15, g = lane >> 4;
#pragma unroll
    for (int rt = 0; rt < NRT; ++rt)
#pragma unroll
        for (int ct = 0; ct < NCT; ++ct)
#pragma unroll
            for (int r = 0; r < 4; ++r) {
                const int off = (rt * 16 + g * 4 + r) * ld + col0 + ct * 16 + i;
                if (PA == 1) dst[off] = (uint16_t)q_f2e<E>(t[rt][ct][r]);
                else {
                    uint32_t hi, lo;
                    f2bf_split(t[rt][ct][r], hi, lo);
                    dst[off] = (uint16_t)hi;
                    dst[off + plane] = (uint16_t)lo;
                }
            }
}

struct QArgs2 {
    QArgs q;
    unsigned long long* tl;
    float* pi;
};

#define PH_TL(k)                                                                                             \
    do {                                                                                                     \
        if (aa.tl && blockIdx.x == 0 && blockIdx.y == 0 && blockIdx.z == 0 && threadIdx.x == 0)              \
            aa.tl[(k)] = __builtin_amdgcn_s_memrealtime();                                                   \
    } while (0)

template <int PA, int NRT, bool QF16 = false>
__global__ __launch_bounds__(NTHREADS) void k_query_pre2(const QArgs2 aa) {
    const QArgs& a = aa.q;
    constexpr int ROWS = NRT * 16;
    constexpr int PLANE = ROWS * LDA;
    extern __shared__ __attribute__((aligned(16))) unsigned char smem[];
    uint16_t* act = (uint16_t*)smem;
    float* red = (float*)(act + PA * PLANE);
    float* cnt = red + 2 * 2 * NW * ROWS;

    const int tid = threadIdx.x, lane = tid & 63;
    const int wave = __builtin_amdgcn_readfirstlane(tid >> 6);
    const int i = lane & 15, g = lane >> 4;
    const int row0 = blockIdx.x * ROWS, br = blockIdx.y, b = blockIdx.z;
    const int N = a.N, Npad = a.Npad;
    const uint16_t* wb = a.wb;
    const int64_t wpl = a.lay.wb_plane_elems;
    const float* wf = a.wf;
    const int64_t* WO = a.lay.w[br];
    const int64_t* VO = a.lay.v[br];
    float* pi = aa.pi + ((((int64_t)b * 2 + br) * Npad + row0) * 2) * 256;

    WStream<PA, CT> ws;
    const WRef2 c_dyn_o{wb + WO[PH_W_DYN], 16 + wave * CT, 8, 0}, c_dyn_i{wb + WO[PH_W_DYN], wave * CT, 8, 0};
    const WRef2 c_inp_i{wb + WO[PH_W_INP], wave * CT, 8, 0}, c_inp_o{wb + WO[PH_W_INP], 16 + wave * CT, 8, 0};
    const WRef2 c_ug{wb + WO[PH_W_UG], wave * CT, 8, 0}, c_ig{wb + WO[PH_W_IG], wave * CT, 8, 0}, c_fc{wb + WO[PH_W_FC], wave * CT, 8, 0};
    const WRef2 c_q{wb + WO[PH_W_QKV], wave * CT, 8, 0}, c_k{wb + WO[PH_W_QKV], 16 + wave * CT, 8, 0}, c_v{wb + WO[PH_W_QKV], 32 + wave * CT, 8, 0};
    auto prime = [&](const WRef2& r) { return [&, r]() { w_prime<PA, CT>(ws, r, wpl, lane); }; };
    constexpr int PT = QF16 ? 1 : PA;
    constexpr int ET = QF16 ? PH_E_F16 : PH_E_BF16;
    auto primeT = [&](const WRef2& r) { return [&, r]() { w_prime<PT, CT>(ws, r, wpl, lane); }; };
    w_prime<PA, CT>(ws, c_dyn_o, wpl, lane);
    PH_TL(0);

    auto put16 = [&](int rr, int cb, const float (&v)[16]) {
#pragma unroll
        for (int e = 0; e < 16; e += 2) {
            uint32_t h0, l0, h1, l1;
            f2bf_split(v[e], h0, l0); f2bf_split(v[e + 1], h1, l1);
            *(uint32_t*)(act + rr * LDA + cb + e) = pack2(h0, h1);
            if (PA == 2) *(uint32_t*)(act + PLANE + rr * LDA + cb + e) = pack2(l0, l1);
        }
    };

    {
        const int r = tid >> 5, cb = (tid & 31) * 8;
        for (int rr = r; rr < ROWS; rr += NTHREADS / 32) {
            const int row = row0 + rr;
            float u[8];
#pragma unroll
            for (int e = 0; e < 8; ++e) u[e] = 0.f;
            int c = 0;
            if (row < Npad) {
                if (a.pcount) {
                    for (int s0 = tid & 31; s0 < a.nsplit; s0 += 32) c += a.pcount[((int64_t)b * a.nsplit + s0) * Npad + row];
                } else {
                    const uint4* bw = (const uint4*)(a.bits + ((int64_t)b * Npad + row) * (a.HWp / 32));
                    const int nq = (int)(a.HWp / 128);
                    for (int w0 = tid & 31; w0 < nq; w0 += 256) {
                        uint4 q[8];
#pragma unroll
                        for (int j = 0; j < 8; ++j) q[j] = w0 + 32 * j < nq ? bw[w0 + 32 * j] : make_uint4(0, 0, 0, 0);
#pragma unroll
                        for (int j = 0; j < 8; ++j) c += __popc(q[j].x) + __popc(q[j].y) + __popc(q[j].z) + __popc(q[j].w);
                    }
                }
                constexpr int TRIP = NRT == 1 ? 16 : 8;
                for (int s0 = 0; s0 < a.nsplit; s0 += TRIP) {
                    float4 v[TRIP][2];
#pragma unroll
                    for (int j = 0; j < TRIP; ++j) {
                        const float* p = a.partial + (((int64_t)b * a.nsplit + s0 + j) * Npad + row) * 512 + br * 256 + cb;
#pragma unroll
                        for (int e = 0; e < 2; ++e)
                            v[j][e] = s0 + j < a.nsplit ? *(const float4*)(p + 4 * e) : make_float4(0.f, 0.f, 0.f, 0.f);
                    }
#pragma unroll
                    for (int j = 0; j < TRIP; ++j)
#pragma unroll
                        for (int e = 0; e < 2; ++e) {
                            u[4 * e] += v[j][e].x; u[4 * e + 1] += v[j][e].y; u[4 * e + 2] += v[j][e].z; u[4 * e + 3] += v[j][e].w;
                        }
                }
            }
#pragma unroll
            for (int e = 0; e < 8; e += 2) {
                uint32_t h0, l0, h1, l1;
                f2bf_split(u[e], h0, l0); f2bf_split(u[e + 1], h1, l1);
                *(uint32_t*)(act + rr * LDA + cb + e) = pack2(h0, h1);
                if (PA == 2) *(uint32_t*)(act + PLANE + rr * LDA + cb + e) = pack2(l0, l1);
            }
            float cf = wave_group16_sum((float)c);
            cf += __shfl_xor(cf, 16);
            if ((tid & 31) == 0) cnt[rr] = cf;
        }
    }
    __syncthreads();

    PH_TL(1);
    const float* vc = wf + VO[PH_V_DYN_CNT];
    const float* bd = wf + VO[PH_V_DYN_B];
    {
        Tile<NRT> Po[1];
        tile_zero(Po[0].v);
        gemm_stream<PA, NRT, CT, 8>(Po[0].v, act, LDA, PLANE, ws, c_dyn_o, wpl, lane, prime(c_dyn_i));
#pragma unroll
        for (int ct = 0; ct < CT; ++ct) {
            const int col = wave * WCOLS + ct * 16 + i;
            const float vc1 = vc[256 + col], bd1 = bd[256 + col];
#pragma unroll
            for (int rt = 0; rt < NRT; ++rt)
#pragma unroll
                for (int r = 0; r < 4; ++r) Po[0].v[rt][ct][r] += cnt[rt * 16 + g * 4 + r] * vc1 + bd1;
        }
        const float* const gm[1] = {wf + VO[PH_V_LN_PO_G]};
        const float* const bt[1] = {wf + VO[PH_V_LN_PO_B]};
        ln_tiles<NRT, 1>(Po, gm, bt, red, wave, lane);
#pragma unroll
        for (int rt = 0; rt < NRT; ++rt)
#pragma unroll
            for (int ct = 0; ct < CT; ++ct)
#pragma unroll
                for (int r = 0; r < 4; ++r)
                    pi[((rt * 16 + g * 4 + r) * 2 + 0) * 256 + wave * WCOLS + ct * 16 + i] = Po[0].v[rt][ct][r];
    }
    Tile<NRT> Pin;
    tile_zero(Pin.v);
    gemm_stream<PA, NRT, CT, 8>(Pin.v, act, LDA, PLANE, ws, c_dyn_i, wpl, lane, prime(c_inp_i));
#pragma unroll
    for (int ct = 0; ct < CT; ++ct) {
        const int col = wave * WCOLS + ct * 16 + i;
        const float vc0 = vc[col], bd0 = bd[col];
#pragma unroll
        for (int rt = 0; rt < NRT; ++rt)
#pragma unroll
            for (int r = 0; r < 4; ++r) Pin.v[rt][ct][r] += cnt[rt * 16 + g * 4 + r] * vc0 + bd0;
    }
    __syncthreads();
    PH_TL(2);
    {
        const int r = tid >> 4, cb = (tid & 15) * 16;
        for (int rr = r; rr < ROWS; rr += NTHREADS / 16) {
            const int row = row0 + rr;
            float kv[16];
#pragma unroll
            for (int e = 0; e < 16; ++e) kv[e] = 0.f;
            if (row < N) {
                const float* kp = a.k_in + ((int64_t)b * N + row) * 256 + cb;
#pragma unroll
                for (int e = 0; e < 16; e += 4) {
                    const float4 v = *(const float4*)(kp + e);
                    kv[e] = v.x; kv[e + 1] = v.y; kv[e + 2] = v.z; kv[e + 3] = v.w;
                }
                if (br == 1) {
                    const float* qp = a.q_in + ((int64_t)b * N + row) * 256 + cb;
#pragma unroll
                    for (int e = 0; e < 16; e += 4) {
                        const float4 v = *(const float4*)(qp + e);
                        kv[e] += v.x; kv[e + 1] += v.y; kv[e + 2] += v.z; kv[e + 3] += v.w;
                    }
                }
            }
            put16(rr, cb, kv);
        }
    }
    __syncthreads();
    PH_TL(3);
    const float* bi = wf + VO[PH_V_INP_B];
    {
        Tile<NRT> Iin;
        tile_zero(Iin.v);
        gemm_stream<PA, NRT, CT, 8>(Iin.v, act, LDA, PLANE, ws, c_inp_i, wpl, lane, prime(c_inp_o));
#pragma unroll
        for (int ct = 0; ct < CT; ++ct) {
            const float bi0 = bi[wave * WCOLS + ct * 16 + i];
#pragma unroll
            for (int rt = 0; rt < NRT; ++rt)
#pragma unroll
                for (int r = 0; r < 4; ++r) Pin.v[rt][ct][r] = (Iin.v[rt][ct][r] + bi0) * Pin.v[rt][ct][r];
        }
    }
    {
        Tile<NRT> Io[1];
        tile_zero(Io[0].v);
        gemm_stream<PA, NRT, CT, 8>(Io[0].v, act, LDA, PLANE, ws, c_inp_o, wpl, lane, prime(c_ug));
#pragma unroll
        for (int ct = 0; ct < CT; ++ct) {
            const float bi1 = bi[256 + wave * WCOLS + ct * 16 + i];
#pragma unroll
            for (int rt = 0; rt < NRT; ++rt)
#pragma unroll
                for (int r = 0; r < 4; ++r) Io[0].v[rt][ct][r] += bi1;
        }
        const float* const gm[1] = {wf + VO[PH_V_LN_IO_G]};
        const float* const bt[1] = {wf + VO[PH_V_LN_IO_B]};
        ln_tiles<NRT, 1>(Io, gm, bt, red, wave, lane);
#pragma unroll
        for (int rt = 0; rt < NRT; ++rt)
#pragma unroll
            for (int ct = 0; ct < CT; ++ct)
#pragma unroll
                for (int r = 0; r < 4; ++r)
                    pi[((rt * 16 + g * 4 + r) * 2 + 1) * 256 + wave * WCOLS + ct * 16 + i] = Io[0].v[rt][ct][r];
    }
    tile_to_lds<PA, NRT>(Pin, act, PLANE, wave, lane);
    __syncthreads();

    PH_TL(4);
    {
        Tile<NRT> Fg;
        auto gate = [&](const WRef2& cur, auto&& next, int b_idx, int g_idx, int be_idx, int which, bool first) {
            Tile<NRT> G[1];
            tile_zero(G[0].v);
            gemm_stream<PA, NRT, CT, 8>(G[0].v, act, LDA, PLANE, ws, cur, wpl, lane, next);
            tile_add_bias(G[0], wf + VO[b_idx], wave, lane);
            const float* const gm[1] = {wf + VO[g_idx]};
            const float* const bt[1] = {wf + VO[be_idx]};
            ln_tiles<NRT, 1>(G, gm, bt, red, wave, lane);
#pragma unroll
            for (int rt = 0; rt < NRT; ++rt) {
                float pv[CT][4];
#pragma unroll
                for (int ct = 0; ct < CT; ++ct)
#pragma unroll
                    for (int r = 0; r < 4; ++r) pv[ct][r] = pi[((rt * 16 + g * 4 + r) * 2 + which) * 256 + wave * WCOLS + ct * 16 + i];
#pragma unroll
                for (int ct = 0; ct < CT; ++ct)
#pragma unroll
                    for (int r = 0; r < 4; ++r) {
                        const float t = fast_sigmoid(G[0].v[rt][ct][r]) * pv[ct][r];
                        Fg.v[rt][ct][r] = first ? t : Fg.v[rt][ct][r] + t;
                    }
            }
        };
        gate(c_ug, prime(c_ig), PH_V_UG_B, PH_V_LN_UG_G, PH_V_LN_UG_B, 0, true);
        gate(c_ig, prime(c_fc), PH_V_IG_B, PH_V_LN_IG_G, PH_V_LN_IG_B, 1, false);
        tile_to_lds<PA, NRT>(Fg, act, PLANE, wave, lane);
    }
    __syncthreads();

    PH_TL(5);
    {
        Tile<NRT> O[1];
        tile_zero(O[0].v);
        gemm_stream<PA, NRT, CT, 8>(O[0].v, act, LDA, PLANE, ws, c_fc, wpl, lane, primeT(c_q));
        tile_add_bias(O[0], wf + VO[PH_V_FC_B], wave, lane);
        const float* const gm[1] = {wf + VO[PH_V_LN_FC_G]};
        const float* const bt[1] = {wf + VO[PH_V_LN_FC_B]};
        ln_tiles<NRT, 1>(O, gm, bt, red, wave, lane);
        float* o1 = a.o1 + (((int64_t)b * 2 + br) * Npad + row0) * 256;
#pragma unroll
        for (int rt = 0; rt < NRT; ++rt)
#pragma unroll
            for (int ct = 0; ct < CT; ++ct)
#pragma unroll
                for (int r = 0; r < 4; ++r) {
                    const float v = fmaxf(O[0].v[rt][ct][r], 0.f);
                    O[0].v[rt][ct][r] = v;
                    o1[(rt * 16 + g * 4 + r) * 256 + wave * WCOLS + ct * 16 + i] = v;
                }
        tile_to_lds<PT, NRT, ET>(O[0], act, PLANE, wave, lane);
    }
    __syncthreads();

    PH_TL(6);
    const int64_t qk_base = (((int64_t)b * 2 + br) * Npad + row0) * 256;
    const int64_t qk_plane = (int64_t)a.B * 2 * Npad * 256;
    const int64_t vt_base = ((int64_t)b * 2 + br) * 256 * Npad + row0;
    const float* qkv_bias = wf + VO[PH_V_QKV_B];
    {
        Tile<NRT> T;
        tile_zero(T.v);
        gemm_stream<PT, NRT, CT, 8, ET>(T.v, act, LDA, PLANE, ws, c_q, wpl, lane, primeT(c_k));
        store_qkv<PA, NRT, 0, QF16>(T, a, qkv_bias, qk_base, qk_plane, vt_base, wave, lane);
        tile_zero(T.v);
        gemm_stream<PT, NRT, CT, 8, ET>(T.v, act, LDA, PLANE, ws, c_k, wpl, lane, primeT(c_v));
        store_qkv<PA, NRT, 1, QF16>(T, a, qkv_bias + 256, qk_base, qk_plane, vt_base, wave, lane);
        tile_zero(T.v);
        gemm_stream<PT, NRT, CT, 8, ET>(T.v, act, LDA, PLANE, ws, c_v, wpl, lane, NoNext());
        store_qkv<PA, NRT, 2, QF16>(T, a, qkv_bias + 512, qk_base, qk_plane, vt_base, wave, lane);
    }
    PH_TL(7);
}

template <int PA> constexpr int post2_hc() { return PA == 1 ? 256 : 128; }
template <int PA, int NRT> constexpr int post2_nhb() {
    return ((size_t)PA * NRT * 16 * LDA * 2 + 2 * (size_t)PA * NRT * 16 * (post2_hc<PA>() + 8) * 2 + 2 * 2 * NW * NRT * 16 * 4 + NW * PA * 16 * LDPT * 2 <= 150 * 1024) ? 2 : 1;
}

template <int PA, int NRT, int E = PH_E_BF16>
__global__ __launch_bounds__(NTHREADS) void k_query_post2(const QArgs2 aa) {
    const QArgs& a = aa.q;
    constexpr int ROWS = NRT * 16;
    constexpr int PLANE = ROWS * LDA;
    constexpr int HC = post2_hc<PA>(), LDH = HC + 8, CTH = HC / 128;
    constexpr int HPLANE = ROWS * LDH;
    constexpr int NHB = post2_nhb<PA, NRT>();
    extern __shared__ __attribute__((aligned(16))) unsigned char smem[];
    uint16_t* act = (uint16_t*)smem;
    uint16_t* hb = act + PA * PLANE;
    float* red = (float*)(hb + NHB * PA * HPLANE);
    uint16_t* ptile = (uint16_t*)(red + 2 * 2 * NW * ROWS);
    const int Npad = a.Npad, N = a.N;

    const int tid = threadIdx.x, lane = tid & 63;
    const int wave = __builtin_amdgcn_readfirstlane(tid >> 6);
    const int i = lane & 15, g = lane >> 4;
    const int row0 = blockIdx.x * ROWS, br = blockIdx.y, b = blockIdx.z;
    const uint16_t* wb = a.wb;
    const int64_t wpl = a.lay.wb_plane_elems;
    const float* wf = a.wf;
    const int64_t* WO = a.lay.w[br];
    const int64_t* VO = a.lay.v[br];

    const int64_t qk_plane = (int64_t)a.B * 2 * Npad * 256;
    const uint16_t* Qb = a.Qp + (((int64_t)b * 2 + br) * Npad + row0) * 256;
    const uint16_t* Kb = a.Kp + ((int64_t)b * 2 + br) * Npad * 256;
    const uint16_t* Vb = a.Vt + ((int64_t)b * 2 + br) * 256 * Npad;

    WStream<PA, CT> ws;
    WStream<PA, 1> ws1;
    const WRef2 c_out{wb + WO[PH_W_OUT], wave * CT, 8, 0};
    const WRef2 c_h0a{wb + WO[PH_W_H0A], wave * CT, 8, 0}, c_h0b{wb + WO[PH_W_H0B], wave * CT, 8, 0};
    const WRef2 c_kern{wb + WO[PH_W_KERN], wave * CT, 8, 0}, c_kb{wb + WO[PH_W_KERN], 16, 8, 0};
    auto prime = [&](const WRef2& r) { return [&, r]() { w_prime<PA, CT>(ws, r, wpl, lane); }; };
    auto ffn1_ref = [&](int c) { return WRef2{wb + WO[PH_W_FFN1], c * (HC / 16) + wave * CTH, 8, 0}; };
    auto ffn1_prime = [&](int c) {
        if constexpr (CTH == CT) w_prime<PA, CT>(ws, ffn1_ref(c), wpl, lane);
        else w_prime<PA, 1>(ws1, ffn1_ref(c), wpl, lane);
    };
    w_prime<PA, CT>(ws, c_out, wpl, lane);
    PH_TL(8);

    Tile<NRT> At;
    {
        const int h = wave;
        const int nkt = Npad / 16;
        uint16_t* Pt = ptile + wave * (PA * 16 * LDPT);
        uint4 qf[PA][NRT];
#pragma unroll
        for (int p = 0; p < PA; ++p)
#pragma unroll
            for (int rt = 0; rt < NRT; ++rt)
                qf[p][rt] = *(const uint4*)(Qb + p * qk_plane + (rt * 16 + i) * 256 + h * 32 + g * 8);
        float mx[NRT][4], sm[NRT][4];
#pragma unroll
        for (int rt = 0; rt < NRT; ++rt)
#pragma unroll
            for (int r = 0; r < 4; ++r) { mx[rt][r] = -INFINITY; sm[rt][r] = 0.f; }
        auto load_k = [&](uint4 (&kf)[PA], int kt) {
#pragma unroll
            for (int p = 0; p < PA; ++p) kf[p] = *(const uint4*)(Kb + p * qk_plane + (kt * 16 + i) * 256 + h * 32 + g * 8);
        };
        auto score = [&](const uint4 (&kf)[PA], int rt) {
            f32x4_t s = {0.f, 0.f, 0.f, 0.f};
            s = mfma16e<E>(qf[0][rt], kf[0], s);
            if (PA == 2) { s = mfma16(qf[0][rt], kf[PA - 1], s); s = mfma16(qf[PA - 1][rt], kf[0], s); }
            return s;
        };
        for (int kt = 0; kt < nkt; ++kt) {
            uint4 kf[PA];
            load_k(kf, kt);
            const bool valid = kt * 16 + i < N;
#pragma unroll
            for (int rt = 0; rt < NRT; ++rt) {
                const f32x4_t s = score(kf, rt);
#pragma unroll
                for (int r = 0; r < 4; ++r) mx[rt][r] = fmaxf(mx[rt][r], valid ? s[r] : -INFINITY);
            }
        }
#pragma unroll
        for (int rt = 0; rt < NRT; ++rt)
#pragma unroll
            for (int r = 0; r < 4; ++r) mx[rt][r] = wave_group16_max(mx[rt][r]);
        tile_zero(At.v);
        for (int ks = 0; ks < nkt / 2; ++ks) {
            uint4 kf[2][PA], vf[2][PA];
            load_k(kf[0], 2 * ks);
            load_k(kf[1], 2 * ks + 1);
#pragma unroll
            for (int ct = 0; ct < 2; ++ct)
#pragma unroll
                for (int p = 0; p < PA; ++p)
                    vf[ct][p] = *(const uint4*)(Vb + p * qk_plane + (int64_t)(h * 32 + ct * 16 + i) * Npad + ks * 32 + g * 8);
#pragma unroll
            for (int rt = 0; rt < NRT; ++rt) {
#pragma unroll
                for (int half = 0; half < 2; ++half) {
                    const f32x4_t s = score(kf[half], rt);
                    const bool valid = (2 * ks + half) * 16 + i < N;
#pragma unroll
                    for (int r = 0; r < 4; ++r) {
                        const float pv = valid ? fast_exp(s[r] - mx[rt][r]) : 0.f;
                        sm[rt][r] += pv;
                        const int off = (g * 4 + r) * LDPT + half * 16 + i;
                        if (PA == 2) {
                            uint32_t hi, lo;
                            f2bf_split(pv, hi, lo);
                            Pt[off] = (uint16_t)hi;
                            Pt[16 * LDPT + off] = (uint16_t)lo;
                        } else Pt[off] = (uint16_t)q_f2e<E>(pv);
                    }
                }
                uint4 pf[PA];
#pragma unroll
                for (int p = 0; p < PA; ++p) pf[p] = *(const uint4*)(Pt + p * 16 * LDPT + i * LDPT + g * 8);
#pragma unroll
                for (int ct = 0; ct < 2; ++ct) {
                    At.v[rt][ct] = mfma16e<E>(pf[0], vf[ct][0], At.v[rt][ct]);
                    if (PA == 2) {
                        At.v[rt][ct] = mfma16(pf[0], vf[ct][PA - 1], At.v[rt][ct]);
                        At.v[rt][ct] = mfma16(pf[PA - 1], vf[ct][0], At.v[rt][ct]);
                    }
                }
            }
        }
#pragma unroll
        for (int rt = 0; rt < NRT; ++rt)
#pragma unroll
            for (int r = 0; r < 4; ++r) {
                const float inv = fast_rcp(wave_group16_sum(sm[rt][r]));
#pragma unroll
                for (int ct = 0; ct < 2; ++ct) At.v[rt][ct][r] *= inv;
            }
    }
    tile_to_lds<PA, NRT, E>(At, act, PLANE, wave, lane);
    __syncthreads();

    PH_TL(9);
    Tile<NRT> O2[1];
    tile_zero(O2[0].v);
    gemm_stream<PA, NRT, CT, 8, E>(O2[0].v, act, LDA, PLANE, ws, c_out, wpl, lane, [&]() { ffn1_prime(0); });
    tile_add_bias(O2[0], wf + VO[PH_V_OUT_B], wave, lane);
    {
        const float* o1 = a.o1 + (((int64_t)b * 2 + br) * Npad + row0) * 256;
#pragma unroll
        for (int rt = 0; rt < NRT; ++rt)
#pragma unroll
            for (int ct = 0; ct < CT; ++ct)
#pragma unroll
                for (int r = 0; r < 4; ++r) O2[0].v[rt][ct][r] += o1[(rt * 16 + g * 4 + r) * 256 + wave * WCOLS + ct * 16 + i];
        const float* const gm[1] = {wf + VO[PH_V_LN_ATT_G]};
        const float* const bt[1] = {wf + VO[PH_V_LN_ATT_B]};
        ln_tiles<NRT, 1>(O2, gm, bt, red, wave, lane);
    }
    tile_to_lds<PA, NRT, E>(O2[0], act, PLANE, wave, lane);
    float* park = aa.pi + ((((int64_t)b * 2 + br) * Npad + row0) * 2) * 256;
#pragma unroll
    for (int rt = 0; rt < NRT; ++rt)
#pragma unroll
        for (int ct = 0; ct < CT; ++ct)
#pragma unroll
            for (int r = 0; r < 4; ++r) park[(rt * 16 + g * 4 + r) * 512 + wave * WCOLS + ct * 16 + i] = O2[0].v[rt][ct][r];
    __syncthreads();

    PH_TL(10);
    Tile<NRT> O3[1];
    tile_zero(O3[0].v);
    {
        const int nchunk = a.lay.ffn_dim / HC;
        const int ffn_ks = a.lay.ffn_dim / 32;
        for (int c = 0; c < nchunk; ++c) {
            uint16_t* hc = hb + (NHB == 2 ? (c & 1) : 0) * PA * HPLANE;
            const WRef2 w2{wb + WO[PH_W_FFN2], wave * CT, ffn_ks, c * (HC / 32)};
            f32x4_t Hc[NRT][CTH];
#pragma unroll
            for (int rt = 0; rt < NRT; ++rt)
#pragma unroll
                for (int ct = 0; ct < CTH; ++ct) Hc[rt][ct] = f32x4_t{0.f, 0.f, 0.f, 0.f};
            if constexpr (CTH == CT) gemm_stream<PA, NRT, CT, 8, E>(Hc, act, LDA, PLANE, ws, ffn1_ref(c), wpl, lane, prime(w2));
            else gemm_stream<PA, NRT, 1, 8, E>(Hc, act, LDA, PLANE, ws1, ffn1_ref(c), wpl, lane, prime(w2));
#pragma unroll
            for (int ct = 0; ct < CTH; ++ct) {
                const float bv = (wf + VO[PH_V_FFN1_B])[c * HC + (wave * CTH + ct) * 16 + i];
#pragma unroll
                for (int rt = 0; rt < NRT; ++rt)
#pragma unroll
                    for (int r = 0; r < 4; ++r) Hc[rt][ct][r] = fmaxf(Hc[rt][ct][r] + bv, 0.f);
            }
            if (NHB == 1 && c > 0) __syncthreads();
            frag_to_lds<PA, NRT, CTH, E>(Hc, hc, LDH, HPLANE, wave * CTH * 16, lane);
            __syncthreads();
            gemm_stream<PA, NRT, CT, HC / 32, E>(O3[0].v, hc, LDH, HPLANE, ws, w2, wpl, lane, [&]() {
                if (c + 1 < nchunk) ffn1_prime(c + 1);
                else w_prime<PA, CT>(ws, br == 0 ? c_h0b : c_h0a, wpl, lane);
            });
        }
    }
    PH_TL(11);
    tile_add_bias(O3[0], wf + VO[PH_V_FFN2_B], wave, lane);
#pragma unroll
    for (int rt = 0; rt < NRT; ++rt)
#pragma unroll
        for (int ct = 0; ct < CT; ++ct)
#pragma unroll
            for (int r = 0; r < 4; ++r) O3[0].v[rt][ct][r] += park[(rt * 16 + g * 4 + r) * 512 + wave * WCOLS + ct * 16 + i];
    {
        const float* const gm[1] = {wf + VO[PH_V_LN_FFN_G]};
        const float* const bt[1] = {wf + VO[PH_V_LN_FFN_B]};
        ln_tiles<NRT, 1>(O3, gm, bt, red, wave, lane);
    }
    {
        float* out = (br == 0 ? a.obj : a.dobj) + ((int64_t)b * N + row0) * 256;
#pragma unroll
        for (int rt = 0; rt < NRT; ++rt)
#pragma unroll
            for (int ct = 0; ct < CT; ++ct)
#pragma unroll
                for (int r = 0; r < 4; ++r) {
                    const int rr = rt * 16 + g * 4 + r;
                    if (row0 + rr < N) out[rr * 256 + wave * WCOLS + ct * 16 + i] = O3[0].v[rt][ct][r];
                }
    }
    tile_to_lds<PA, NRT, E>(O3[0], act, PLANE, wave, lane);
    __syncthreads();

    PH_TL(12);
    Tile<NRT> Hm[1];
    if (br == 0) {
        tile_zero(Hm[0].v);
        gemm_stream<PA, NRT, CT, 8, E>(Hm[0].v, act, LDA, PLANE, ws, c_h0b, wpl, lane, prime(c_h0a));
        {
            const float* const gm[1] = {wf + VO[PH_V_LN_H0B_G]};
            const float* const bt[1] = {wf + VO[PH_V_LN_H0B_B]};
            ln_tiles<NRT, 1>(Hm, gm, bt, red, wave, lane);
        }
        Tile<NRT> Hd[1];
        tile_zero(Hd[0].v);
        const int L = a.lay.num_classes, nct = (L + 15) / 16;
        auto cls_ref = [&](int ct) { return WRef2{wb + WO[PH_W_CLS], ct, 8, 0}; };
        gemm_stream<PA, NRT, CT, 8, E>(Hd[0].v, act, LDA, PLANE, ws, c_h0a, wpl, lane, [&]() {
            w_prime<PA, CT>(ws, c_kern, wpl, lane);
            if (wave < nct) w_prime<PA, 1>(ws1, cls_ref(wave), wpl, lane);
        });
        {
            const float* const gm[1] = {wf + VO[PH_V_LN_H0A_G]};
            const float* const bt[1] = {wf + VO[PH_V_LN_H0A_B]};
            ln_tiles<NRT, 1>(Hd, gm, bt, red, wave, lane);
        }
#pragma unroll
        for (int rt = 0; rt < NRT; ++rt)
#pragma unroll
            for (int ct = 0; ct < CT; ++ct)
#pragma unroll
                for (int r = 0; r < 4; ++r) {
                    Hd[0].v[rt][ct][r] = fmaxf(Hd[0].v[rt][ct][r], 0.f);
                    Hm[0].v[rt][ct][r] = fmaxf(Hm[0].v[rt][ct][r], 0.f);
                }
        tile_to_lds<PA, NRT, E>(Hd[0], act, PLANE, wave, lane);
        __syncthreads();
        const float* bc = wf + VO[PH_V_CLS_B];
        for (int ct = wave; ct < nct; ct += NW) {
            f32x4_t acc[NRT][1];
#pragma unroll
            for (int rt = 0; rt < NRT; ++rt) acc[rt][0] = f32x4_t{0.f, 0.f, 0.f, 0.f};
            gemm_stream<PA, NRT, 1, 8, E>(acc, act, LDA, PLANE, ws1, cls_ref(ct), wpl, lane, [&]() {
                if (ct + NW < nct) w_prime<PA, 1>(ws1, cls_ref(ct + NW), wpl, lane);
            });
            const int col = ct * 16 + i;
            if (col < L) {
                const float bv = bc[col];
#pragma unroll
                for (int rt = 0; rt < NRT; ++rt)
#pragma unroll
                    for (int r = 0; r < 4; ++r) {
                        const int row = row0 + rt * 16 + g * 4 + r;
                        if (row < N) {
                            const float z = acc[rt][0][r] + bv;
                            a.cls[((int64_t)b * N + row) * L + col] = a.cls_sigmoid ? fast_sigmoid(z) : z;
                        }
                    }
            }
        }
        __syncthreads();
    } else {
        tile_zero(Hm[0].v);
        gemm_stream<PA, NRT, CT, 8, E>(Hm[0].v, act, LDA, PLANE, ws, c_h0a, wpl, lane, prime(c_kern));
        const float* const gm[1] = {wf + VO[PH_V_LN_H0A_G]};
        const float* const bt[1] = {wf + VO[PH_V_LN_H0A_B]};
        ln_tiles<NRT, 1>(Hm, gm, bt, red, wave, lane);
    }
    tile_to_lds<PA, NRT, E>(Hm[0], act, PLANE, wave, lane);
    __syncthreads();
    {
        Tile<NRT> Kt;
        tile_zero(Kt.v);
        gemm_stream<PA, NRT, CT, 8, E>(Kt.v, act, LDA, PLANE, ws, c_kern, wpl, lane, [&]() {
            if (wave == 0) w_prime<PA, 1>(ws1, c_kb, wpl, lane);
        });
        const float* bk = wf + VO[PH_V_KERN_B];
        const int64_t kplane = (int64_t)2 * a.B * Npad * 256;
        uint16_t* kd = a.kern + (((int64_t)br * a.B + b) * Npad + row0) * 256;
#pragma unroll
        for (int ct = 0; ct < CT; ++ct) {
            const int col = wave * WCOLS + ct * 16 + i;
            const float bv = bk[col];
#pragma unroll
            for (int rt = 0; rt < NRT; ++rt)
#pragma unroll
                for (int r = 0; r < 4; ++r) {
                    const int off = (rt * 16 + g * 4 + r) * 256 + col;
                    if (a.kern_f16) {
                        kd[off] = (uint16_t)q_f2e<PH_E_F16>(Kt.v[rt][ct][r] + bv);
                    } else {
                        uint32_t hi, lo;
                        f2bf_split(Kt.v[rt][ct][r] + bv, hi, lo);
                        kd[off] = (uint16_t)hi;
                        if (PA == 2) kd[kplane + off] = (uint16_t)lo;
                    }
                }
        }
        if (wave == 0) {
            f32x4_t acc[NRT][1];
#pragma unroll
            for (int rt = 0; rt < NRT; ++rt) acc[rt][0] = f32x4_t{0.f, 0.f, 0.f, 0.f};
            gemm_stream<PA, NRT, 1, 8, E>(acc, act, LDA, PLANE, ws1, c_kb, wpl, lane, NoNext());
            if (i == 0) {
                const float bv = bk[256];
#pragma unroll
                for (int rt = 0; rt < NRT; ++rt)
#pragma unroll
                    for (int r = 0; r < 4; ++r)
                        a.kbias[((int64_t)br * a.B + b) * Npad + row0 + rt * 16 + g * 4 + r] = acc[rt][0][r] + bv;
            }
        }
    }
    PH_TL(13);
}

static size_t q_ws_bytes(int B, int Npad, int PA) {
    return (size_t)PA * 3 * B * 2 * Npad * 256 * sizeof(uint16_t) + (size_t)3 * B * 2 * Npad * 256 * sizeof(float);
}

extern "C" size_t ph_query_workspace_updator_offset(int B, int N, int prec) {
    return (size_t)((prec == PH_PREC_SPLIT || prec == PH_PREC_QHYBRID) ? 2 : 1) * 3 * B * 2 * ph_n_padded(N) * 256 * sizeof(uint16_t);
}

extern "C" size_t ph_query_workspace_bytes(int B, int N, int prec) {
    return q_ws_bytes(B, ph_n_padded(N), (prec == PH_PREC_SPLIT || prec == PH_PREC_QHYBRID) ? 2 : 1);
}

template <int PA, int NRT, bool HY = false>
static void launch_query2(const QArgs2& a, int phases, hipStream_t s) {
    constexpr int ROWS = NRT * 16;
    if constexpr (HY) {
        static_assert(PA == 2, "hybrid = split pre kernel");
        const size_t red = 2 * 2 * NW * ROWS * sizeof(float);
        const size_t lds_pre = (size_t)2 * ROWS * LDA * 2 + red + ROWS * sizeof(float);
        const size_t lds_post = (size_t)ROWS * LDA * 2 + (size_t)post2_nhb<1, NRT>() * ROWS * (post2_hc<1>() + 8) * 2 + red + (size_t)NW * 16 * LDPT * 2;
        static const bool once = [] {
            (void)hipFuncSetAttribute((const void*)k_query_pre2<2, NRT, true>, hipFuncAttributeMaxDynamicSharedMemorySize, 160 * 1024);
            (void)hipFuncSetAttribute((const void*)k_query_post2<1, NRT, PH_E_F16>, hipFuncAttributeMaxDynamicSharedMemorySize, 160 * 1024);
            return true;
        }();
        (void)once;
        const dim3 grid(a.q.Npad / ROWS, 2, a.q.B);
        if (phases & 1) hipLaunchKernelGGL((k_query_pre2<2, NRT, true>), grid, dim3(NTHREADS), lds_pre, s, a);
        if (phases & 2) hipLaunchKernelGGL((k_query_post2<1, NRT, PH_E_F16>), grid, dim3(NTHREADS), lds_post, s, a);
        return;
    }
    const size_t red = 2 * 2 * NW * ROWS * sizeof(float);
    const size_t lds_pre = (size_t)PA * ROWS * LDA * 2 + red + ROWS * sizeof(float);
    const size_t lds_post = (size_t)PA * ROWS * LDA * 2 + (size_t)post2_nhb<PA, NRT>() * PA * ROWS * (post2_hc<PA>() + 8) * 2 + red +
                            (size_t)NW * PA * 16 * LDPT * 2;
    static const bool once = [] {
        (void)hipFuncSetAttribute((const void*)k_query_pre2<PA, NRT>, hipFuncAttributeMaxDynamicSharedMemorySize, 160 * 1024);
        (void)hipFuncSetAttribute((const void*)k_query_post2<PA, NRT>, hipFuncAttributeMaxDynamicSharedMemorySize, 160 * 1024);
        return true;
    }();
    (void)once;
    const dim3 grid(a.q.Npad / ROWS, 2, a.q.B);
    if (phases & 1) hipLaunchKernelGGL((k_query_pre2<PA, NRT>), grid, dim3(NTHREADS), lds_pre, s, a);
    if (phases & 2) hipLaunchKernelGGL((k_query_post2<PA, NRT>), grid, dim3(NTHREADS), lds_post, s, a);
}

static int query_run(const PhQueryKnobs& kn, const float* partial, int nsplit, const uint32_t* bits, const int32_t* pcount, const float* k_in,
                     const float* q_in, const uint16_t* wb, const float* wf, const ph_stage_layout* layout, float* obj, float* dobj,
                     float* cls, int cls_sigmoid, uint16_t* kern, float* kbias, void* workspace,
                     size_t workspace_bytes, int B, int N, int64_t HW, int prec, int kern_format, int phases,
                     void* stream) {
    PH_CHECK_ARG((phases & ~(PH_QUERY_BOTH | PH_QUERY_WIDE)) == 0 && (phases & PH_QUERY_BOTH) != 0,
                 "phases must be PH_QUERY_PRE | PH_QUERY_POST [| PH_QUERY_WIDE]");
    PH_CHECK_ARG(partial && bits && k_in && q_in && wb && wf && layout && obj && dobj && cls && kern && kbias && workspace,
                 "null pointer");
    PH_CHECK_ARG(B > 0 && N > 0 && N <= 256 && HW > 0 && nsplit >= 1, "bad size");
    PH_CHECK_ARG(prec == PH_PREC_BF16 || prec == PH_PREC_SPLIT || prec == PH_PREC_QHYBRID, "prec must be PH_PREC_BF16, PH_PREC_SPLIT or PH_PREC_QHYBRID");
    PH_CHECK_ARG(kern_format == PH_KERN_BF16_PLANES || kern_format == PH_KERN_F16, "bad kern_format");
    PH_CHECK_ARG(prec != PH_PREC_QHYBRID || kern_format == PH_KERN_F16, "PH_PREC_QHYBRID emits the dynamic kernels as one fp16 plane (PH_KERN_F16)");
    PH_CHECK_ARG(layout->ffn_dim > 0 && layout->ffn_dim % 256 == 0, "ffn_dim must be a multiple of 256");
    PH_CHECK_ARG(layout->num_classes > 0 && layout->num_classes <= 1024, "bad num_classes");
    const bool hybrid = prec == PH_PREC_QHYBRID;
    const int PA = (prec == PH_PREC_SPLIT || hybrid) ? 2 : 1, Npad = ph_n_padded(N);
    const bool wide = (phases & PH_QUERY_WIDE) != 0;
    phases &= PH_QUERY_BOTH;
    if (workspace_bytes < q_ws_bytes(B, Npad, PA)) {
        ph_set_error("ph_query_stage: workspace too small (%zu < %zu)", workspace_bytes, q_ws_bytes(B, Npad, PA));
        return PH_EWORKSPACE;
    }
    QArgs a;
    a.partial = partial; a.bits = bits; a.pcount = pcount; a.k_in = k_in; a.q_in = q_in; a.wb = wb; a.wf = wf;
    a.obj = obj; a.dobj = dobj; a.cls = cls; a.kern = kern; a.kbias = kbias;
    const size_t pl = (size_t)PA * B * 2 * Npad * 256;
    a.Qp = (uint16_t*)workspace; a.Kp = a.Qp + pl; a.Vt = a.Kp + pl; a.o1 = (float*)(a.Vt + pl);
    a.lay = *layout; a.cls_sigmoid = cls_sigmoid; a.kern_f16 = kern_format == PH_KERN_F16; a.nsplit = nsplit; a.B = B; a.N = N; a.Npad = Npad; a.HWp = ph_hw_padded(HW);
    hipStream_t s = (hipStream_t)stream;
    QArgs2 a2;
    a2.q = a;
    unsigned long long* tl = kn.timeline;
    a2.tl = tl;
    a2.pi = a.o1 + (size_t)B * 2 * Npad * 256;
    const int t = Npad / 16;
    int nrt = 1;
    if (wide) {
        nrt = t % 5 == 0 ? 5 : (t % 4 == 0 ? 4 : (t % 3 == 0 ? 3 : (t % 2 == 0 ? 2 : 1)));
    } else {
        int smallest = 1;
        for (int c = 5; c >= 2; --c) {
            if (t % c) continue;
            smallest = c;
            if (nrt == 1 && (int64_t)B * 2 * (t / c) >= 200) nrt = c;
        }
        if (nrt == 1) nrt = smallest;
    }
    if (kn.nrt > 0) { nrt = kn.nrt; while (t % nrt) --nrt; }
#define PH_Q2(P, R) launch_query2<P, R>(a2, phases, s)
#define PH_QH(R) launch_query2<2, R, true>(a2, phases, s)
    if (hybrid) { switch (nrt) { case 5: PH_QH(5); break; case 4: PH_QH(4); break; case 3: PH_QH(3); break; case 2: PH_QH(2); break; default: PH_QH(1); } }
    else if (PA == 1) { switch (nrt) { case 5: PH_Q2(1, 5); break; case 4: PH_Q2(1, 4); break; case 3: PH_Q2(1, 3); break; case 2: PH_Q2(1, 2); break; default: PH_Q2(1, 1); } }
    else { switch (nrt) { case 5: PH_Q2(2, 5); break; case 4: PH_Q2(2, 4); break; case 3: PH_Q2(2, 3); break; case 2: PH_Q2(2, 2); break; default: PH_Q2(2, 1); } }
#undef PH_Q2
#undef PH_QH
    if (tl) {
        unsigned long long h[16];
        (void)hipStreamSynchronize(s);
        (void)hipMemcpy(h, tl, sizeof(h), hipMemcpyDeviceToHost);
        fprintf(stderr, "query timeline (100 MHz ticks, x10 ns):");
        for (int k = 1; k < 14; ++k) fprintf(stderr, " %s%lld", k == 8 ? "| " : "", (long long)(h[k] - h[k - 1]));
        fprintf(stderr, "\n");
    }
    PH_CHECK_LAUNCH();
    return PH_OK;
}

static PhQueryKnobs query_switches() {
    PhQueryKnobs k;
    k.nrt = ph_switch(PH_SWITCH_QUERY_NRT);
    if (ph_switch(PH_SWITCH_QUERY_TIMELINE)) {
        static unsigned long long* const tl = [] {
            unsigned long long* p = nullptr;
            if (hipMalloc((void**)&p, 16 * sizeof(unsigned long long)) == hipSuccess) (void)hipMemset(p, 0, 128);
            return p;
        }();
        k.timeline = tl;
    }
    return k;
}

extern "C" int ph_query_stage(const float* partial, int nsplit, const uint32_t* bits, const float* k_in, const float* q_in,
                              const uint16_t* wb, const float* wf, const ph_stage_layout* layout, float* obj, float* dobj,
                              float* cls, int cls_sigmoid, uint16_t* kern, float* kbias, void* workspace,
                              size_t workspace_bytes, int B, int N, int64_t HW, int prec, int kern_format, int phases,
                              void* stream) {
    return query_run(query_switches(), partial, nsplit, bits, nullptr, k_in, q_in, wb, wf, layout, obj, dobj, cls, cls_sigmoid, kern, kbias, workspace,
                     workspace_bytes, B, N, HW, prec, kern_format, phases, stream);
}

extern "C" int ph_query_stage_counts(const float* partial, int nsplit, const uint32_t* bits, const int32_t* pcount, const float* k_in,
                                     const float* q_in, const uint16_t* wb, const float* wf, const ph_stage_layout* layout,
                                     float* obj, float* dobj, float* cls, int cls_sigmoid, uint16_t* kern, float* kbias,
                                     void* workspace, size_t workspace_bytes, int B, int N, int64_t HW, int prec, int kern_format,
                                     int phases, void* stream) {
    if (!pcount) { ph_set_error("ph_query_stage_counts: null pcount"); return PH_EINVAL; }
    return query_run(query_switches(), partial, nsplit, bits, pcount, k_in, q_in, wb, wf, layout, obj, dobj, cls, cls_sigmoid, kern, kbias,
                     workspace, workspace_bytes, B, N, HW, prec, kern_format, phases, stream);
}

int ph_query_stage_counts_k(const PhQueryKnobs& kn, const float* partial, int nsplit, const uint32_t* bits, const int32_t* pcount,
                            const float* k_in, const float* q_in, const uint16_t* wb, const float* wf, const ph_stage_layout* layout,
                            float* obj, float* dobj, float* cls, int cls_sigmoid, uint16_t* kern, float* kbias, void* workspace,
                            size_t workspace_bytes, int B, int N, int64_t HW, int prec, int kern_format, int phases, void* stream) {
    if (!pcount) { ph_set_error("ph_query_stage_counts: null pcount"); return PH_EINVAL; }
    return query_run(kn, partial, nsplit, bits, pcount, k_in, q_in, wb, wf, layout, obj, dobj, cls, cls_sigmoid, kern, kbias, workspace,
                     workspace_bytes, B, N, HW, prec, kern_format, phases, stream);
}
```

polyphonicformer_amd/engine.py:

```python
import contextlib
import ctypes as C
import math

import torch

from . import _lib, knobs
from .pack import pack_stage

import collections

Mode = collections.namedtuple("Mode", "name feat query conv kern_fmt FP KP feat_dtype")
_QH = _lib.PH_PREC_SPLIT if knobs.get("PH_QUERY_FULL_SPLIT") else _lib.PH_PREC_QHYBRID
MODES = {
    "bf16": Mode("bf16", _lib.PH_PREC_BF16, _lib.PH_PREC_BF16, _lib.PH_PREC_BF16, _lib.PH_KERN_BF16_PLANES, 1, 1, torch.bfloat16),
    "mixed": Mode("mixed", _lib.PH_PREC_BF16, _lib.PH_PREC_SPLIT, _lib.PH_PREC_BF16_KSPLIT, _lib.PH_KERN_BF16_PLANES, 1, 2, torch.bfloat16),
    "mixed16": Mode("mixed16", _lib.PH_PREC_BF16, _QH, _lib.PH_PREC_BF16_KF16, _lib.PH_KERN_F16, 1, 1, torch.bfloat16),
    "fp16": Mode("fp16", _lib.PH_PREC_F16, _QH, _lib.PH_PREC_F16, _lib.PH_KERN_F16, 1, 1, torch.float16),
    "fp32": Mode("fp32", _lib.PH_PREC_SPLIT, _lib.PH_PREC_SPLIT, _lib.PH_PREC_SPLIT, _lib.PH_KERN_BF16_PLANES, 2, 2, None),
}
MODES["split"] = MODES["fp32"]
PREC = {"bf16": _lib.PH_PREC_BF16, "split": _lib.PH_PREC_SPLIT, "fp32": _lib.PH_PREC_SPLIT,
        "mixed": _lib.PH_PREC_SPLIT, "mixed16": _lib.PH_PREC_SPLIT, "fp16": _lib.PH_PREC_SPLIT}
KHEAD_PREC = dict(PREC, fp16=_lib.PH_PREC_F16)
OUT_CODE = {torch.float32: _lib.PH_OUT_F32, torch.bfloat16: _lib.PH_OUT_BF16, torch.float16: _lib.PH_OUT_F16}


def mode_of(p):
    if isinstance(p, Mode):
        return p
    if isinstance(p, str):
        return MODES[p]
    return {_lib.PH_PREC_BF16: MODES["bf16"], _lib.PH_PREC_SPLIT: MODES["fp32"], _lib.PH_PREC_F16: MODES["fp16"]}[p]


def hw_padded(hw):
    return (hw + 127) // 128 * 128


def n_padded(n):
    return (n + 31) // 32 * 32


def _require_gpu(t, name):
    if not t.is_cuda:
        raise _lib.PolyheadError(f"{name} must live on the GPU: libpolyhead has no CPU path")


class StagePack:

    def __init__(self, sd, prefix, num_classes, prec, device):
        wb, wf, lay = pack_stage(sd, prefix, num_classes, prec)
        self.wb = wb.to(device)
        self.wf = wf.to(device)
        self.lay = lay
        self.num_classes = num_classes
        self.prec = prec


def default_nsplit(B, HW, frame_invariant=False):
    n = knobs.get("PH_POOL_NSPLIT")
    if n is not None:
        return n
    return int(_lib.load().ph_pool_default_nsplit(B, HW, int(bool(frame_invariant))))


def ingest(x, prec, out=None):
    _require_gpu(x, "x")
    B, Cc, H, W = x.shape
    if Cc != 256:
        raise _lib.PolyheadError("libpolyhead supports 256 channels (the shipped configs)")
    x = x.contiguous().float()
    P = 2 if prec == _lib.PH_PREC_SPLIT else 1
    if out is None:
        out = torch.empty((P, B, 256, hw_padded(H * W)), dtype=torch.int16, device=x.device)
    lib = _lib.load()
    _lib.check(lib.ph_ingest_features(_lib.ptr(x), _lib.ptr(out), B, H * W, prec, _lib.stream_ptr()), "ph_ingest_features")
    return out


def binarize(m, out=None):
    _require_gpu(m, "mask_preds")
    B, N, H, W = m.shape
    m = m.contiguous() if m.dtype in OUT_CODE else m.contiguous().float()
    if out is None:
        out = torch.empty((B, n_padded(N), hw_padded(H * W) // 32), dtype=torch.int32, device=m.device)
    lib = _lib.load()
    _lib.check(lib.ph_binarize_if(_lib.ptr(m), OUT_CODE[m.dtype], 0, _lib.ptr(out), B, N, H * W, None, _lib.stream_ptr()), "ph_binarize")
    return out


def pool(xp, dp, bits, N, HW, prec, nsplit=None, out=None, counts=None):
    B = xp.shape[1]
    if nsplit is None:
        nsplit = default_nsplit(B, HW)
    if out is None:
        out = torch.empty((B, nsplit, n_padded(N), 512), dtype=torch.float32, device=xp.device)
    lib = _lib.load()
    if counts is not None:
        _lib.check(lib.ph_pool_counts(_lib.ptr(xp), _lib.ptr(dp), _lib.ptr(bits), _lib.ptr(out), _lib.ptr(counts), B, N, HW, nsplit, prec,
                                      _lib.stream_ptr()), "ph_pool_counts")
    else:
        _lib.check(lib.ph_pool(_lib.ptr(xp), _lib.ptr(dp), _lib.ptr(bits), _lib.ptr(out), B, N, HW, nsplit, prec,
                               _lib.stream_ptr()), "ph_pool")
    return out


def query_stage(partial, bits, k_in, q_in, pack, N, HW, cls_sigmoid=False, outs=None, workspace=None, phases=3,
                kern_fmt=_lib.PH_KERN_BF16_PLANES, counts=None):
    B, nsplit = partial.shape[0], partial.shape[1]
    dev = partial.device
    prec = pack.prec
    P = 1 if kern_fmt == _lib.PH_KERN_F16 else (2 if prec == _lib.PH_PREC_SPLIT else 1)
    Npad = n_padded(N)
    lib = _lib.load()
    if outs is None:
        outs = dict(obj=torch.empty((B, N, 256), dtype=torch.float32, device=dev),
                    dobj=torch.empty((B, N, 256), dtype=torch.float32, device=dev),
                    cls=torch.empty((B, N, pack.num_classes), dtype=torch.float32, device=dev),
                    kern=torch.empty((P, 2, B, Npad, 256), dtype=torch.int16, device=dev),
                    kbias=torch.empty((2, B, Npad), dtype=torch.float32, device=dev))
    if workspace is None:
        workspace = torch.empty((lib.ph_query_workspace_bytes(B, N, prec),), dtype=torch.uint8, device=dev)
    tail = (_lib.ptr(k_in), _lib.ptr(q_in), _lib.ptr(pack.wb), _lib.ptr(pack.wf), C.byref(pack.lay),
            _lib.ptr(outs["obj"]), _lib.ptr(outs["dobj"]), _lib.ptr(outs["cls"]), 1 if cls_sigmoid else 0, _lib.ptr(outs["kern"]),
            _lib.ptr(outs["kbias"]), _lib.ptr(workspace), workspace.numel(), B, N, HW, prec, kern_fmt, phases, _lib.stream_ptr())
    if counts is not None:
        _lib.check(lib.ph_query_stage_counts(_lib.ptr(partial), nsplit, _lib.ptr(bits), _lib.ptr(counts), *tail), "ph_query_stage_counts")
    else:
        _lib.check(lib.ph_query_stage(_lib.ptr(partial), nsplit, _lib.ptr(bits), *tail), "ph_query_stage")
    return outs


def dynconv(planes, kern, kbias, branch, N, HW, prec, bits_out=None, logits_out=None, out_dtype=_lib.PH_OUT_F32):
    B, Npad = kern.shape[2], kern.shape[3]
    lib = _lib.load()
    kptr = C.c_void_p(kern.data_ptr() + branch * B * Npad * 256 * 2)
    bptr = C.c_void_p(kbias.data_ptr() + branch * B * Npad * 4)
    _lib.check(lib.ph_dynconv(_lib.ptr(planes), kptr, 2 * B * Npad * 256, Npad * 256, bptr, Npad, _lib.ptr(bits_out),
                              _lib.ptr(logits_out), out_dtype, N * HW, B, N, HW, prec, _lib.stream_ptr()), "ph_dynconv")
    return bits_out if bits_out is not None else logits_out


def dynconv_poolx(planes, kern, kbias, N, HW, prec, bits_out, partial):
    B, Npad = kern.shape[2], kern.shape[3]
    lib = _lib.load()
    _lib.check(lib.ph_dynconv_poolx(_lib.ptr(planes), _lib.ptr(kern), Npad * 256, _lib.ptr(kbias), Npad, _lib.ptr(bits_out), _lib.ptr(partial),
                                    partial.shape[1], B, N, HW, prec, _lib.stream_ptr()), "ph_dynconv_poolx")
    return bits_out


def pool_depth_only(dp, bits, N, HW, prec, partial, counts):
    B, nsplit = partial.shape[0], partial.shape[1]
    lib = _lib.load()
    _lib.check(lib.ph_pool_counts(_lib.ptr(dp), None, _lib.ptr(bits), C.c_void_p(partial.data_ptr() + 256 * 4), _lib.ptr(counts), B, N, HW, nsplit, prec,
                                  _lib.stream_ptr()), "ph_pool_counts(depth)")


def dynconv_up2(planes, kern, kbias, branch, N, H, W, prec, up_out, logits_out=None, out_dtype=_lib.PH_OUT_F16, workgroups=0):
    B, Npad = kern.shape[2], kern.shape[3]
    lib = _lib.load()
    kptr = C.c_void_p(kern.data_ptr() + branch * B * Npad * 256 * 2)
    bptr = C.c_void_p(kbias.data_ptr() + branch * B * Npad * 4)
    _lib.check(lib.ph_dynconv_up2_wgs(_lib.ptr(planes), kptr, Npad * 256, bptr, Npad, _lib.ptr(logits_out), _lib.ptr(up_out), out_dtype,
                                      B, N, H, W, prec, int(workgroups), _lib.stream_ptr()), "ph_dynconv_up2")
    return up_out


def static_conv(planes, wplanes, bias, N, HW, prec, logits_out, out_rows):
    B = planes.shape[1]
    Npad = wplanes.shape[1]
    lib = _lib.load()
    _lib.check(lib.ph_dynconv(_lib.ptr(planes), _lib.ptr(wplanes), Npad * 256, 0, _lib.ptr(bias), 0, None,
                              _lib.ptr(logits_out), _lib.PH_OUT_F32, out_rows * HW, B, N, HW, prec, _lib.stream_ptr()),
               "ph_dynconv(static)")
    return logits_out


def upsample2x(src, out=None):
    _require_gpu(src, "src")
    src = src.contiguous()
    H, W = src.shape[-2:]
    planes = src.numel() // (H * W)
    if out is None:
        out = torch.empty(tuple(src.shape[:-2]) + (2 * H, 2 * W), dtype=src.dtype, device=src.device)
    if src.dtype not in OUT_CODE:
        raise _lib.PolyheadError("upsample2x: fp32, bf16 or fp16 only")
    dt = OUT_CODE[src.dtype]
    lib = _lib.load()
    _lib.check(lib.ph_upsample2x(_lib.ptr(src), _lib.ptr(out), dt, planes, H, W, _lib.stream_ptr()), "ph_upsample2x")
    return out


def _knob_code(off, on, on_code):
    return _lib.PH_KNOB_OFF if off else (on_code if on else _lib.PH_KNOB_AUTO)


def native_cfg(B, N, H, W, S, L, F, prec, out_dtype=torch.float32, frame_invariant=False, shares_gpu=False, nsplit=None):
    mode = mode_of(prec)
    poolx, up2 = knobs.get("PH_CONV_POOLX"), knobs.get("PH_CONV_UP2")
    return _lib.DecodeCfg(B=B, N=N, H=H, W=W, S=S, L=L, F=F, mode=_lib.PH_MODE[mode.name], out_dtype=OUT_CODE[out_dtype],
                          frame_invariant=int(bool(frame_invariant)),
                          query_full_split=int(mode.name in ("mixed16", "fp16") and mode.query == _lib.PH_PREC_SPLIT),
                          shares_gpu=int(bool(shares_gpu)),
                          poolx=_knob_code(poolx == "0", poolx == "1", _lib.PH_KNOB_WHERE_SUPPORTED),
                          fused_up=_knob_code(up2 == "0", up2 == "1", _lib.PH_KNOB_WHERE_SUPPORTED),
                          nsplit=int(nsplit or knobs.get("PH_POOL_NSPLIT") or 0),
                          nsplit_px=0 if frame_invariant else knobs.get("PH_POOLX_NSPLIT") or 0,
                          up2_wgs=knobs.get("PH_UP2_SHARED_WGS") or 0)


def _cfg_error(what):
    msg = _lib.load().ph_last_error_string()
    return _lib.PolyheadError(f"{what}: {msg.decode() if msg else ''}")


class DecodePlan:

    def __init__(self, packs, B, N, H, W, prec, out_dtype=torch.float32, device="cuda:0", nsplit=None, frame_invariant=False,
                 shares_gpu=False):
        self.packs, self.S = packs, len(packs)
        self.frame_invariant, self.shares_gpu = frame_invariant, shares_gpu
        self.feat_is_bf16 = False
        self.debug_bits = None
        self.on_first_pool = None
        self.B, self.N, self.H, self.W, self.HW = B, N, H, W, H * W
        self.mode = mode_of(prec)
        self.prec, self.out_dtype = self.mode.feat, out_dtype
        if any(p.prec != self.mode.query for p in packs):
            raise _lib.PolyheadError(f"stage packs are not packed for mode '{self.mode.name}'")
        L = packs[0].num_classes
        self.cfg = native_cfg(B, N, H, W, self.S, L, packs[0].lay.ffn_dim, self.mode, out_dtype, frame_invariant, shares_gpu, nsplit)
        geo = _lib.DecodeGeometry()
        if _lib.load().ph_decode_geometry_of(C.byref(self.cfg), C.byref(geo)) != 0:
            raise _cfg_error("ph_decode_geometry_of")
        self.nsplit, self.nsplit_px, self.poolx, self.fused_up = geo.nsplit, geo.nsplit_px, bool(geo.poolx), bool(geo.fused_up)
        dev = torch.device(device)
        P, KP = self.mode.FP, self.mode.KP
        Npad, HWp = n_padded(N), hw_padded(self.HW)
        e = lambda shape, dt: torch.empty(shape, dtype=dt, device=dev)
        self.x = e((B, 256, H, W), torch.float32)
        self.dfe = e((B, 256, H, W), torch.float32)
        self.k0 = e((B, N, 256), torch.float32)
        self.q0 = e((B, N, 256), torch.float32)
        self.m0 = e((B, N, H, W), torch.float32)
        z = (lambda shape, dt: torch.zeros(shape, dtype=dt, device=dev)) if HWp != self.HW else e
        self.xp = z((P, B, 256, HWp), torch.int16)
        self.dp = z((P, B, 256, HWp), torch.int16)
        self.bits = e((B, Npad, HWp // 32), torch.int32)
        self.partial = e((B, self.nsplit, Npad, 512), torch.float32)
        self.pcount = e((B, self.nsplit, Npad), torch.int32)
        self.ws = e((_lib.load().ph_query_workspace_bytes(B, N, self.mode.query),), torch.uint8)
        self.stage_out = [dict(obj=e((B, N, 256), torch.float32), dobj=e((B, N, 256), torch.float32),
                               cls=e((B, N, L), torch.float32), kern=e((KP, 2, B, Npad, 256), torch.int16),
                               kbias=e((2, B, Npad), torch.float32)) for _ in range(self.S)]
        self.mask = e((B, N, H, W), out_dtype)
        self.depth = e((B, N, H, W), out_dtype)
        self.mask_up = e((B, N, 2 * H, 2 * W), out_dtype)
        self.depth_up = e((B, N, 2 * H, 2 * W), out_dtype)
        self.graph = None
        self.handoff_runs = 0
        self.want_depth_lowres = False
        self.up2_shared_wgs = self.cfg.up2_wgs or \
            (3 * torch.cuda.get_device_properties(device).multi_processor_count // 2 if dev.type == "cuda" else 0)
        if self.poolx:
            self.partial_px = e((B, self.nsplit_px, Npad, 512), torch.float32)
            self.pcount_px = e((B, self.nsplit_px, Npad), torch.int32)

    @property
    def out_code(self):
        return OUT_CODE[self.out_dtype]

    def renew_outputs(self):
        if self.graph is not None:
            raise _lib.PolyheadError("renew_outputs on a captured plan")
        e = lambda t: torch.empty_like(t)
        self.mask, self.depth, self.mask_up, self.depth_up = e(self.mask), e(self.depth), e(self.mask_up), e(self.depth_up)
        last = self.stage_out[-1]
        for k in ("obj", "dobj", "cls"):
            last[k] = e(last[k])

    def set_inputs(self, x, dfe, k0, q0, m0):
        self.feat_is_bf16 = x.dtype in (torch.bfloat16, torch.float16) and dfe.dtype == x.dtype
        if self.feat_is_bf16:
            if self.mode.feat_dtype != x.dtype:
                raise _lib.PolyheadError(f"{x.dtype} feature inputs need a mode with that plane format (bf16: 'bf16' / "
                                         f"'mixed' / 'mixed16', fp16: 'fp16'; this plan: '{self.mode.name}')")
            self.xp.view(x.dtype)[0, :, :, :self.HW].copy_(x.reshape(self.B, 256, self.HW))
            self.dp.view(x.dtype)[0, :, :, :self.HW].copy_(dfe.reshape(self.B, 256, self.HW))
        else:
            self.x.copy_(x)
            self.dfe.copy_(dfe)
        self.k0.copy_(k0.reshape(self.B, self.N, 256))
        self.q0.copy_(q0.reshape(self.B, self.N, 256))
        if m0.dtype in OUT_CODE and self.m0.dtype != m0.dtype:
            self.m0 = torch.empty_like(self.m0, dtype=m0.dtype)
            self.graph = None
        self.m0.copy_(m0)

    def ingest(self):
        if not self.feat_is_bf16:
            ingest(self.x, self.prec, out=self.xp)
            ingest(self.dfe, self.prec, out=self.dp)
        binarize(self.m0, out=self.bits)

    def stages(self, xp=None, dp=None):
        xp = self.xp if xp is None else xp
        dp = self.dp if dp is None else dp
        k, q = self.k0, self.q0
        for s in range(self.S):
            last = s == self.S - 1
            if self.debug_bits is not None:
                self.debug_bits.append(self.bits.clone())
            if s > 0 and self.poolx:
                pool_depth_only(dp, self.bits, self.N, self.HW, self.prec, self.partial_px, self.pcount_px)
                part, cnt = self.partial_px, self.pcount_px
            else:
                pool(xp, dp, self.bits, self.N, self.HW, self.prec, self.nsplit, out=self.partial, counts=self.pcount)
                part, cnt = self.partial, self.pcount
            if s == 0 and self.on_first_pool is not None:
                self.on_first_pool()
            o = query_stage(part, self.bits, k, q, self.packs[s], self.N, self.HW, cls_sigmoid=last,
                            outs=self.stage_out[s], workspace=self.ws, kern_fmt=self.mode.kern_fmt, counts=cnt,
                            phases=3 | (_lib.PH_QUERY_WIDE if self.shares_gpu else 0))
            cv = self.mode.conv
            if not last:
                if self.poolx:
                    dynconv_poolx(xp, o["kern"], o["kbias"], self.N, self.HW, cv, self.bits, self.partial_px)
                else:
                    dynconv(xp, o["kern"], o["kbias"], 0, self.N, self.HW, cv, bits_out=self.bits)
            else:
                if self.fused_up:
                    wg = self.up2_shared_wgs if (self.shares_gpu and self.B * self.H >= 4 * self.up2_shared_wgs) else 0
                    dynconv_up2(xp, o["kern"], o["kbias"], 0, self.N, self.H, self.W, cv, self.mask_up, logits_out=self.mask,
                                out_dtype=self.out_code, workgroups=wg)
                    dynconv_up2(dp, o["kern"], o["kbias"], 1, self.N, self.H, self.W, cv, self.depth_up,
                                logits_out=self.depth if self.want_depth_lowres else None, out_dtype=self.out_code, workgroups=wg)
                else:
                    dynconv(xp, o["kern"], o["kbias"], 0, self.N, self.HW, cv, logits_out=self.mask, out_dtype=self.out_code)
                    upsample2x(self.mask, out=self.mask_up)
                    dynconv(dp, o["kern"], o["kbias"], 1, self.N, self.HW, cv, logits_out=self.depth, out_dtype=self.out_code)
                    upsample2x(self.depth, out=self.depth_up)
            k, q = o["obj"], o["dobj"]

    def run(self):
        self.ingest()
        self.stages()

    def run_from_planes(self, xp, dp, bits, k0, q0):
        self.handoff_runs += 1
        self.bits.copy_(bits)
        self.k0.copy_(k0.reshape(self.B, self.N, 256))
        self.q0.copy_(q0.reshape(self.B, self.N, 256))
        self.stages(xp, dp)

    def capture(self):
        s = torch.cuda.Stream()
        s.wait_stream(torch.cuda.current_stream())
        with torch.cuda.stream(s):
            self.run()
        torch.cuda.current_stream().wait_stream(s)
        torch.cuda.synchronize()
        self.graph = torch.cuda.CUDAGraph()
        with torch.cuda.graph(self.graph):
            self.run()
        return self.graph

    def replay(self):
        self.graph.replay()

    def outputs(self):
        last = self.stage_out[-1]
        depth = self.depth if (not self.fused_up or self.want_depth_lowres) else None
        return dict(obj=last["obj"], dobj=last["dobj"], cls=last["cls"], mask=self.mask, depth=depth,
                    mask_up=self.mask_up, depth_up=self.depth_up)


def _gather_params(module, device, count, name_of, numel_of, slots=None):
    sd = module.state_dict() if hasattr(module, "state_dict") else module
    params = []
    for i in range(count):
        name = name_of(i).decode()
        t = sd[name].detach().to(device=device, dtype=torch.float32).contiguous()
        if t.numel() != numel_of(i):
            raise _lib.PolyheadError(f"{name}: {t.numel()} elements, the cfg needs {numel_of(i)}")
        params.append(t)
    return params, (C.c_void_p * (slots or count))(*[t.data_ptr() for t in params])


def _pack_on_device(params_from, cfg, device, symbols, nparams, slots=None, name_takes_cfg=False):
    lib, ref = _lib.load(), C.byref(cfg)
    bytes_fn, name_fn, numel_fn, pack_fn = (getattr(lib, s) for s in symbols)
    nbytes = bytes_fn(ref)
    if nbytes == 0:
        raise _cfg_error(symbols[0])
    name_of = (lambda i: name_fn(ref, i)) if name_takes_cfg else name_fn
    params, ptrs = _gather_params(params_from, device, nparams, name_of, lambda i: numel_fn(ref, i), slots)
    blob = torch.empty((nbytes,), dtype=torch.uint8, device=device)
    with torch.cuda.device(device):
        _lib.check(pack_fn(ref, ptrs, _lib.ptr(blob), _lib.stream_ptr()), symbols[3])
    return blob


def _pack_piece(blob, layout, i, dtype, shape):
    off, nb = int(layout.offset[i]), int(layout.bytes[i])
    return blob[off:off + nb].view(dtype).reshape(shape) if nb else None


_GRADE_OF_MODE = {code: KHEAD_PREC[name] for name, code in _lib.PH_MODE.items()}
_MODE_NAME = {code: name for name, code in _lib.PH_MODE.items() if name != "split"}


class _NativePack:
    _symbols, _layout_type, _slots, _name_takes_cfg = (), None, None, False

    def __init__(self, blob, cfg):
        lay = self._layout_type()
        _lib.check(getattr(_lib.load(), self._symbols[4])(C.byref(cfg), C.byref(lay)), self._symbols[4])
        self.blob, self.layout, self.cfg = blob, lay, type(cfg).from_buffer_copy(bytes(cfg))
        self.mode = getattr(cfg, "mode", None)
        self.prec = cfg.prec if self.mode is None else _GRADE_OF_MODE[self.mode]
        self.P = 2 if self.prec == _lib.PH_PREC_SPLIT else 1
        self._pieces(cfg)

    def piece(self, i, dtype, shape):
        return _pack_piece(self.blob, self.layout, i, dtype, shape)

    @classmethod
    def pack_on_device(cls, module, cfg, device):
        return cls(_pack_on_device(module, cfg, device, cls._symbols[:4], cls._nparams(cfg), cls._slots, cls._name_takes_cfg), cfg)


class _OwnsHandles:
    _destroy_symbol = None

    def _destroy(self):
        for h in list(getattr(self, "_handles", {}).values()) + [getattr(self, "_h", None)]:
            if h is not None and h.value and _lib._lib is not None:
                getattr(_lib._lib, self._destroy_symbol)(h)
        self._handles, self._h = {}, None

    __del__ = _destroy


def _on(dev):
    return torch.cuda.device(dev) if dev.type == "cuda" else contextlib.nullcontext()


class _NativePlan(_OwnsHandles):
    _symbols, _geometry_type, _zeroed = (), None, False

    def _alloc_workspace(self):
        with _on(self.device):
            nbytes = getattr(_lib.load(), self._symbols[0])(C.byref(self.cfg))
            if nbytes == 0:
                raise _cfg_error(self._symbols[0])
            self.workspace = (torch.zeros if self._zeroed else torch.empty)((nbytes,), dtype=torch.uint8, device=self.device)

    def _create(self, pack, **fields):
        cfg = type(self.cfg).from_buffer_copy(bytes(self.cfg))
        for k, v in fields.items():
            setattr(cfg, k, int(v))
        h = C.c_void_p()
        with _on(self.device):
            _lib.check(getattr(_lib.load(), self._symbols[1])(C.byref(cfg), pack, _lib.ptr(self.workspace), self.workspace.numel(),
                                                             C.byref(h)), self._symbols[1])
        return h

    def _handle_of(self, **fields):
        key = tuple(fields.values())
        if key not in self._handles:
            self._handles[key] = self._create(_lib.ptr(self.pack.blob), **fields)
        return self._handles[key]

    def _info(self, h):
        geo = self._geometry_type()
        _lib.check(getattr(_lib.load(), self._symbols[2])(h, C.byref(geo)), self._symbols[2])
        return geo


def _fan_out_towers(streams, device, tower):
    if streams is None:
        streams = [torch.cuda.Stream(device=device) for _ in range(4)]
    cur = torch.cuda.current_stream()
    for lvl in (0, 3, 2, 1):
        streams[lvl].wait_stream(cur)
        with torch.cuda.stream(streams[lvl]):
            tower(lvl)
    for st in streams:
        cur.wait_stream(st)
    return streams


def native_pack_stage(module, cfg, device):
    return _pack_on_device(module, cfg, device, ("ph_decode_pack_bytes", "ph_decode_param_name", "ph_decode_param_numel",
                                                 "ph_decode_pack_stage"), _lib.PH_DECODE_NPARAMS)


def native_pack_from(pack, cfg):
    lib = _lib.load()
    lay, off = _lib.StageLayout(), C.c_size_t()
    _lib.check(lib.ph_decode_pack_layout(C.byref(cfg), C.byref(lay), C.byref(off)), "ph_decode_pack_layout")
    if bytes(lay) != bytes(pack.lay):
        raise _lib.PolyheadError("the StagePack's layout differs from the native pack layout of this cfg")
    blob = torch.zeros((lib.ph_decode_pack_bytes(C.byref(cfg)),), dtype=torch.uint8, device=pack.wb.device)
    wb = pack.wb.contiguous().view(torch.uint8).reshape(-1)
    wf = pack.wf.contiguous().view(torch.uint8).reshape(-1)
    blob[:wb.numel()].copy_(wb)
    blob[off.value:off.value + wf.numel()].copy_(wf)
    return blob


class NativeDecodePlan(_NativePlan):
    _symbols, _geometry_type, _destroy_symbol = ("ph_decode_workspace_bytes", "ph_decode_create", "ph_decode_info"), _lib.DecodeGeometry, \
        "ph_decode_destroy"

    def __init__(self, packs, B, N, H, W, prec, out_dtype=torch.float32, device="cuda:0", nsplit=None, frame_invariant=False,
                 shares_gpu=False, num_classes=None, ffn_dim=None):
        self.S, self.B, self.N, self.H, self.W, self.HW = len(packs), B, N, H, W, H * W
        self.mode = mode_of(prec)
        self.prec, self.out_dtype, self.frame_invariant, self.shares_gpu = self.mode.feat, out_dtype, frame_invariant, shares_gpu
        dev = torch.device(device)
        self.device = dev
        if all(isinstance(p, StagePack) for p in packs):
            if any(p.prec != self.mode.query for p in packs):
                raise _lib.PolyheadError(f"stage packs are not packed for mode '{self.mode.name}'")
            L, F = packs[0].num_classes, packs[0].lay.ffn_dim
        else:
            L, F = num_classes, ffn_dim
        self.cfg = native_cfg(B, N, H, W, self.S, L, F, self.mode, out_dtype, frame_invariant, shares_gpu, nsplit)
        self._alloc_workspace()
        self.packs = [native_pack_from(p, self.cfg) if isinstance(p, StagePack) else p for p in packs]
        self._h = self._create((C.c_void_p * self.S)(*[p.data_ptr() for p in self.packs]))
        self.geometry = geo = self._info(self._h)
        self.nsplit, self.nsplit_px, self.poolx, self.fused_up = geo.nsplit, geo.nsplit_px, bool(geo.poolx), bool(geo.fused_up)
        Npad, HWp = n_padded(N), hw_padded(self.HW)
        self.xp = torch.empty((self.mode.FP, B, 256, HWp), dtype=torch.int16, device="meta")
        self.bits = torch.empty((B, Npad, HWp // 32), dtype=torch.int32, device="meta")
        self.want_depth_lowres = False
        self.graph = None
        self.handoff_runs = 0
        self._in = None
        self.io = _lib.DecodeIO()
        self._alloc_outputs()

    @property
    def out_code(self):
        return OUT_CODE[self.out_dtype]

    def _alloc_outputs(self):
        e = lambda shape, dt: torch.empty(shape, dtype=dt, device=self.device)
        B, N, H, W = self.B, self.N, self.H, self.W
        self.obj, self.dobj = e((B, N, 256), torch.float32), e((B, N, 256), torch.float32)
        self.cls = e((B, N, self.cfg.L), torch.float32)
        self.mask, self.mask_up, self.depth_up = e((B, N, H, W), self.out_dtype), e((B, N, 2 * H, 2 * W), self.out_dtype), \
            e((B, N, 2 * H, 2 * W), self.out_dtype)
        self.depth = e((B, N, H, W), self.out_dtype) if (not self.fused_up or self.want_depth_lowres) else None
        io = self.io
        io.obj, io.dobj, io.cls = self.obj.data_ptr(), self.dobj.data_ptr(), self.cls.data_ptr()
        io.mask, io.mask_up, io.depth_up = self.mask.data_ptr(), self.mask_up.data_ptr(), self.depth_up.data_ptr()

    def renew_outputs(self):
        if self.graph is not None:
            raise _lib.PolyheadError("renew_outputs on a captured plan")
        self._alloc_outputs()

    def set_inputs(self, x, dfe, k0, q0, m0):
        B, N = self.B, self.N
        f16 = x.dtype in (torch.bfloat16, torch.float16) and dfe.dtype == x.dtype
        if f16 and self.mode.feat_dtype != x.dtype:
            raise _lib.PolyheadError(f"{x.dtype} feature inputs need a mode with that plane format (bf16: 'bf16' / "
                                     f"'mixed' / 'mixed16', fp16: 'fp16'; this plan: '{self.mode.name}')")
        for t, nm, numel in ((x, "x", B * 256 * self.HW), (dfe, "depth_feats", B * 256 * self.HW), (k0, "proposal_feats", B * N * 256),
                             (q0, "depth_proposal", None), (m0, "mask_preds", B * N * self.HW)):
            _require_gpu(t, nm)
            if numel is not None and t.numel() != numel:
                raise _lib.PolyheadError(f"{nm}: {tuple(t.shape)} does not fit the plan (B={B}, N={N}, H={self.H}, W={self.W})")
        cast = (lambda t: t.contiguous()) if f16 else (lambda t: t.float().contiguous())
        new = dict(x=cast(x), dfe=cast(dfe), k0=k0.reshape(B, N, 256).float().contiguous(),
                   q0=q0.reshape(B, N, 256).float().contiguous(),
                   m0=m0.contiguous() if m0.dtype in OUT_CODE else m0.float().contiguous())
        if self.graph is not None and self._in is not None and self._in.get("feat") == 1 and all(
                self._in[k].dtype == v.dtype for k, v in new.items()):
            for k, v in new.items():
                self._in[k].copy_(v)
            return
        self.graph = None
        self._in = dict(new, feat=1)
        self._point_inputs(_lib.PH_FEAT_16 if f16 else _lib.PH_FEAT_F32)

    def _point_inputs(self, feat_format, bits=None):
        i, io = self._in, self.io
        io.feat_format = feat_format
        io.x, io.depth_feats, io.k0, io.q0 = i["x"].data_ptr(), i["dfe"].data_ptr(), i["k0"].data_ptr(), i["q0"].data_ptr()
        io.m0 = None if bits is not None else i["m0"].data_ptr()
        io.m0_dtype = OUT_CODE.get(i["m0"].dtype, _lib.PH_OUT_F32) if bits is None else _lib.PH_OUT_F32
        io.bits = None if bits is None else bits.data_ptr()

    def run(self):
        io = self.io
        if (not self.fused_up or self.want_depth_lowres) and self.depth is None:
            self.depth = torch.empty((self.B, self.N, self.H, self.W), dtype=self.out_dtype, device=self.device)
        io.depth = self.depth.data_ptr() if (not self.fused_up or self.want_depth_lowres) else None
        _lib.check(_lib.load().ph_decode_run(self._h, C.byref(io), _lib.stream_ptr()), "ph_decode_run")

    def run_from_planes(self, xp, dp, bits, k0, q0):
        if tuple(xp.shape) != tuple(self.xp.shape) or tuple(dp.shape) != tuple(self.xp.shape) or tuple(bits.shape) != tuple(self.bits.shape):
            raise _lib.PolyheadError("run_from_planes: planes / bits of another geometry")
        self.handoff_runs += 1
        B, N = self.B, self.N
        self.graph = None
        self._in = dict(x=xp.contiguous(), dfe=dp.contiguous(), k0=k0.reshape(B, N, 256).float().contiguous(),
                        q0=q0.reshape(B, N, 256).float().contiguous(), m0=None, bits=bits.contiguous())
        self._point_inputs(_lib.PH_FEAT_PLANES, bits=self._in["bits"])
        self.run()

    def capture(self):
        if self._in is None or self._in.get("feat") != 1:
            raise _lib.PolyheadError("capture needs set_inputs first")
        ff = self.io.feat_format
        self._in = dict({k: v.clone() for k, v in self._in.items() if k != "feat"}, feat=1)
        self._point_inputs(ff)
        s = torch.cuda.Stream()
        s.wait_stream(torch.cuda.current_stream())
        with torch.cuda.stream(s):
            self.run()
        torch.cuda.current_stream().wait_stream(s)
        torch.cuda.synchronize()
# ... 941 lines not shown
```

polyphonicformer_amd/knobs.py:

```python
import collections
import os

Knob = collections.namedtuple("Knob", "name kind default effect reader doc")

KNOBS = {k.name: k for k in (
    Knob("PH_QUERY_FULL_SPLIT", "flag", False, "import", "engine.MODES",
         "`mixed16` / `fp16` run the all-hi/lo query kernels instead of the hybrid ones (§4.3c)"),
    Knob("PH_CONV_POOLX", "text", "auto", "plan cfg", "engine.native_cfg",
         "`0` never / `1` wherever it exists: the stage-boundary conv also pools (`ph_dynconv_poolx`); anything else: the library's rule"),
    Knob("PH_CONV_UP2", "text", "auto", "plan cfg", "engine.native_cfg",
         "`0` never / `1` wherever it exists: final stage as `ph_dynconv_up2`; anything else: the library's rule (fused from B·H ≥ 512, §4.4b)"),
    Knob("PH_POOL_NSPLIT", "int", None, "plan cfg", "engine.native_cfg, native_khead_cfg, default_nsplit",
         "pixel ranges of the pooling kernels (cfg field `nsplit`; an `nsplit` argument wins).  Known oddity: `0` means the "
         "library's rule in the cfg builders, while `engine.default_nsplit` returns the 0"),
    Knob("PH_POOLX_NSPLIT", "int", None, "plan cfg", "engine.native_cfg",
         "pixel ranges of the fused conv + pooling (cfg field `nsplit_px`); not read for a `frame_invariant` plan"),
    Knob("PH_UP2_SHARED_WGS", "int", None, "plan cfg", "engine.native_cfg",
         "workgroups of the fused final-stage kernel of a plan that `shares_gpu` (default 1.5 per CU: 0 … +1.3 % on the step, "
         "`profiles/r06/knob_sweep.txt`)"),
    Knob("PH_KHEAD_TWOPASS", "flag", False, "plan cfg", "engine.native_khead_cfg",
         "KernelHead post-neck by `ph_khead_fused` (two passes) instead of `ph_khead_onepass` (§4.5b; cfg field `onepass`); "
         "an `onepass=True` argument beside it is an error"),
    Knob("PH_NECK_OUT2", "text", "1", "plan cfg", "engine.native_neck_cfg",
         "`0`: the neck's three output convs per map (round 3's form; cfg field `fused_out`); `2` / `3`: removed measurement "
         "forms, refused; anything else: the library's rule"),
    Knob("PH_NECK_C16", "text", "1", "plan cfg", "engine.native_neck_cfg",
         "`0`: no channels-last planes into level 0's stride-2 conv (cfg field `c16`)"),
    Knob("PH_NECK_STREAMS", "text", "1", "plan cfg", "engine.native_neck_cfg",
         "`0` never / `2` always: the four level towers on their own streams (cfg field `tower_buffers`); anything else: from 4 frames"),
    Knob("PH_VIDEO_API_EAGER", "flag", False, "video", "video (the module API's simple_test)",
         "the per-frame module call launches its heads eagerly instead of replaying a one-slot `VideoStreamRunner` graph"),
    Knob("PH_VIDEO_HOST_SELECT", "flag", False, "video", "video.VideoStreamRunner",
         "the merge's candidate selection on the host, the module API's form (the default of `device_select`: on the device)"),
    Knob("PH_VIDEO_SLOT_PRIO", "text", "", "video", "video.VideoStreamRunner",
         "`low`: the slots' head streams one priority level below the caller's stream; anything else: the same priority"),
    Knob("PH_VIDEO_BORROW", "text", "1", "video", "video.VideoStreamRunner",
         "`0`: every launch copies its frames into slot-owned buffers, none reads the caller's tensors"),
    Knob("PH_VIDEO_CLIP_TOWERS", "text", "1", "video", "video.VideoStreamRunner",
         "neck level towers on their own streams inside the slots' graphs: `0` never, `2` also in the sequential one-frame "
         "loop, anything else from 2 frames per launch"),
    Knob("PH_VIDEO_CLIP_BATCH", "int", None, "video", "video.VideoStreamRunner",
         "frames per heads launch of a clip (unset, empty or 0: half the clip, at most 8; 1: one frame per launch)"),
    Knob("PH_ALT_LIB", "raw", "", "import", "_lib",
         "path of a variant build of libpolyhead.so to load instead (`tools/build_variant.py`, same-box A/B timing)"),
    Knob("PH_EXTRA_HIPCC_FLAGS", "raw", "", "build", "build.build_library",
         "extra hipcc arguments for every source, e.g. `-DK1_TIMELINE` (phase stamps of the one-pass kernel; right results, costs registers)"),
)}


_UNSET = {k.name: k.default for k in KNOBS.values()}
_KIND = {k.name: k.kind for k in KNOBS.values()}


def get(name, _environ=os.environ):
    try:
        v = _environ[name]
    except KeyError:
        return _UNSET[name]
    kind = _KIND[name]
    if kind == "text" or kind == "raw":
        return v
    if kind == "flag":
        return bool(v)
    if not v:
        return None
    try:
        return int(v)
    except ValueError:
        raise ValueError(f"{name}={v!r} is not an integer") from None


def markdown():
    rows = ["| variable | kind | unset | takes effect | read by | meaning |", "|---|---|---|---|---|---|"]
    for k in KNOBS.values():
        unset = {"flag": "off", "int": "none"}.get(k.kind) or (f"`{k.default}`" if k.default else "empty")
        rows.append(f"| `{k.name}` | {k.kind} | {unset} | {k.effect} | `{k.reader}` | {k.doc} |")
    return "\n".join(rows)


if __name__ == "__main__":
    print(markdown())
```

Baseline: 16840 frames/s.

## Pair the last two stages' depth pooling into one launch via split query stage

Splits stage S-2's query into mask-only and depth-only branch launches so the mask branch's kernels can run the fused conv+pool for the last stage first. Both depth-feature poolings (for stage S-2 and stage S-1) then run in one paired pool kernel that reads each depth plane tile once and accumulates against two bit sets. The aim is to remove one full pass over the depth planes and one launch. In exchange the query stage is split into two launches, the pool kernel holds twice the accumulators, and the schedule is reordered.

New measurement: 17310 frames/s (median of 6 runs). 1.03x the previous value.

```diff
diff --git a/include/polyhead.h b/include/polyhead.h
--- a/include/polyhead.h
+++ b/include/polyhead.h
@@ -54,6 +54,9 @@
                  int B, int N, int64_t HW, int nsplit, int prec, void* stream);
 int ph_pool_counts(const uint16_t* xplanes, const uint16_t* dplanes, const uint32_t* bits, float* partial, int32_t* pcount,
                    int B, int N, int64_t HW, int nsplit, int prec, void* stream);
+int ph_pool_depth_pair_supported(int N, int prec);
+int ph_pool_depth_pair(const uint16_t* dplanes, const uint32_t* bitsA, const uint32_t* bitsB, float* partialA, float* partialB,
+                       int32_t* pcountA, int32_t* pcountB, int B, int N, int64_t HW, int nsplit, int prec, void* stream);
 int ph_pool_default_nsplit(int B, int64_t HW, int frame_invariant);
 
 enum {
@@ -94,7 +97,7 @@
     int32_t num_classes;
 } ph_stage_layout;
 
-enum { PH_QUERY_PRE = 1, PH_QUERY_POST = 2, PH_QUERY_BOTH = 3, PH_QUERY_WIDE = 0x100 };
+enum { PH_QUERY_PRE = 1, PH_QUERY_POST = 2, PH_QUERY_BOTH = 3, PH_QUERY_WIDE = 0x100, PH_QUERY_MASK_ONLY = 0x200, PH_QUERY_DEPTH_ONLY = 0x400 };
 size_t ph_query_workspace_bytes(int B, int N, int prec);
 size_t ph_query_workspace_updator_offset(int B, int N, int prec);
 int ph_query_stage(const float* partial, int nsplit, const uint32_t* bits,
diff --git a/polyphonicformer_amd/_lib.py b/polyphonicformer_amd/_lib.py
--- a/polyphonicformer_amd/_lib.py
+++ b/polyphonicformer_amd/_lib.py
@@ -14,6 +14,7 @@
 PH_PREC_BF16, PH_PREC_BF16_KSPLIT, PH_PREC_SPLIT, PH_PREC_F16, PH_PREC_BF16_KF16, PH_PREC_QHYBRID = 1, 2, 3, 5, 6, 7
 PH_PLANES_C16 = 0x100
 PH_QUERY_WIDE = 0x100
+PH_QUERY_MASK_ONLY, PH_QUERY_DEPTH_ONLY = 0x200, 0x400
 PH_OUT_F32, PH_OUT_BF16, PH_OUT_F16 = 0, 1, 2
 PH_KERN_BF16_PLANES, PH_KERN_F16 = 0, 1
 PH_GN_TO_PLANES, PH_GN_UP2_PLANES, PH_GN_ACCUM, PH_GN_TO_NCHW, PH_GN_TO_CPLANES = 0, 1, 2, 3, 4
@@ -301,6 +302,8 @@
     "ph_match_sums": (C.c_int, [_P, _P, _P, _P, _I, _I, _I, _L, _P]),
     "ph_upsample2x": (C.c_int, [_P, _P, _I, _L, _I, _I, _P]),
     "ph_dynconv_poolx_supported": (C.c_int, [_I, _I]),
+    "ph_pool_depth_pair_supported": (C.c_int, [_I, _I]),
+    "ph_pool_depth_pair": (C.c_int, [_P, _P, _P, _P, _P, _P, _P, _I, _I, _L, _I, _I, _P]),
     "ph_dynconv_poolx": (C.c_int, [_P, _P, _L, _P, _L, _P, _P, _I, _I, _I, _L, _I, _P]),
     "ph_dynconv_up2_supported": (C.c_int, [_I, _I, _I, _I, _I]),
     "ph_dynconv_up2": (C.c_int, [_P, _P, _L, _P, _L, _P, _P, _I, _I, _I, _I, _I, _I, _P]),
diff --git a/polyphonicformer_amd/csrc/ph_pool.hip b/polyphonicformer_amd/csrc/ph_pool.hip
--- a/polyphonicformer_amd/csrc/ph_pool.hip
+++ b/polyphonicformer_amd/csrc/ph_pool.hip
@@ -31,13 +31,18 @@
 
 __device__ __forceinline__ int pool_swz(int row) { return (row >> 1) & 7; }
 
-template <int PA , int NRT , int E >
+template <int PA , int NRT , int E , int NS = 1 >
 __global__ __launch_bounds__(256, 2) void k_pool(const uint16_t* __restrict__ xplanes, const uint16_t* __restrict__ dplanes,
                                               const uint32_t* __restrict__ bits, float* __restrict__ partial,
-                                              int B, int64_t HWp, int nsplit, int bits_rows, int32_t* __restrict__ pcount) {
+                                              int B, int64_t HWp, int nsplit, int bits_rows, int32_t* __restrict__ pcount,
+                                              const uint32_t* __restrict__ bitsB, float* __restrict__ partialB,
+                                              int32_t* __restrict__ pcountB) {
     constexpr int Npad = NRT * 32;
+    constexpr int CTW = NS;
     constexpr int PER_CHUNK = 4 * PA;
-    constexpr int NBI2 = (Npad + 63) / 64;
+    constexpr int NBI2 = (NS * Npad + 63) / 64;
+    constexpr int NBW = (NBI2 + 3) / 4;
+    static_assert(NBW <= 2 && (NS == 1 || NS == 2), "mask-word DMA: at most two instructions per wave");
     constexpr int NR64 = NBI2 * 64;
     extern __shared__ __attribute__((aligned(16))) uint16_t lds[];
     uint4* lut = (uint4*)(lds + POOL_NBUF * PA * POOL_FT);
@@ -54,28 +59,39 @@
     const uint16_t* fbase = feat + ((int64_t)b * PH_C + ch0) * HWp;
     const int64_t words_per_row = HWp / 32;
     const uint32_t* brow = bits + (int64_t)b * bits_rows * words_per_row;
+    const uint32_t* browB = NS == 2 ? bitsB + (int64_t)b * bits_rows * words_per_row : nullptr;
 
     const int nchunks = (int)(HWp / POOL_CHUNK);
     int c0 = (int)((int64_t)split * nchunks / nsplit), c1 = (int)((int64_t)(split + 1) * nchunks / nsplit);
     c0 &= ~1; c1 = split + 1 == nsplit ? nchunks : (c1 & ~1);
     const bool pair_wave = wave < NBI2;
+    const int nbw = NBW == 1 ? (pair_wave ? 1 : 0) : (wave + 4 < NBI2 ? 2 : 1);
     auto issue_pair_bits = [&](int c, int gb) {
-        if (!pair_wave) return;
-        int row = wave * 64 + lane;
-        if (row > Npad - 1) row = Npad - 1;
-        const uint32_t* src = brow + (int64_t)row * words_per_row + c * 2;
-        uint32_t* dst = lbits + gb * (NR64 * 4) + wave * 256;
-        __builtin_amdgcn_global_load_lds((const __attribute__((address_space(1))) void*)src, (PH_LDS void*)dst, 16, 0, 0);
+#pragma unroll
+        for (int j = 0; j < NBW; ++j) {
+            const int ins = wave + 4 * j;
+            if (ins >= NBI2) return;
+            int row = ins * 64 + lane;
+            if (row > NS * Npad - 1) row = NS * Npad - 1;
+            const uint32_t* src = (NS == 2 && row >= Npad ? browB + (int64_t)(row - Npad) * words_per_row
+                                                          : brow + (int64_t)row * words_per_row) + c * 2;
+            uint32_t* dst = lbits + gb * (NR64 * 4) + ins * 256;
+            __builtin_amdgcn_global_load_lds((const __attribute__((address_space(1))) void*)src, (PH_LDS void*)dst, 16, 0, 0);
+        }
     };
 
     lut[tid] = expand8<E>((uint32_t)tid);
 
-    f32x16_t acc[NRT];
+    f32x16_t acc[NRT][CTW];
 #pragma unroll
     for (int rt = 0; rt < NRT; ++rt)
 #pragma unroll
-        for (int r = 0; r < 16; ++r) acc[rt][r] = 0.f;
-    const bool counting = pcount != nullptr && cg == 0 && wave == 0;
+        for (int j = 0; j < CTW; ++j)
+#pragma unroll
+            for (int r = 0; r < 16; ++r) acc[rt][j][r] = 0.f;
+    const int set = NS == 2 ? wave >> 1 : 0;
+    const int wch = NS == 2 ? (wave & 1) * 64 : wave * 32;
+    const bool counting = pcount != nullptr && cg == 0 && (NS == 2 ? (wave & 1) == 0 : wave == 0);
     int pc[NRT];
 #pragma unroll
     for (int rt = 0; rt < NRT; ++rt) pc[rt] = 0;
@@ -101,17 +117,19 @@
     __syncthreads();
 
     const uint32_t lut_addr = lds_addr(lut);
-    const int frow = wave * 32 + (lane & 31);
+    const int frow = wch + (lane & 31);
     int cur = 0;
     for (int c = c0; c < c1; ++c) {
         const int younger = (c1 - 1 - c) < (POOL_NBUF - 2) ? (c1 - 1 - c) : (POOL_NBUF - 2);
         const int pos = (c - c0) & 1;
-        const bool extra = pos == 1 && younger >= 1 && pair_wave;
+        const int extra = pos == 1 && younger >= 1 ? nbw : 0;
         if (younger >= 2) {
-            if (extra) asm volatile("s_waitcnt vmcnt(%0)" ::"n"(8 * PA + 1) : "memory");
+            if (NBW == 2 && extra == 2) asm volatile("s_waitcnt vmcnt(%0)" ::"n"(8 * PA + 2) : "memory");
+            else if (extra) asm volatile("s_waitcnt vmcnt(%0)" ::"n"(8 * PA + 1) : "memory");
             else asm volatile("s_waitcnt vmcnt(%0)" ::"n"(8 * PA) : "memory");
         } else if (younger == 1) {
-            if (extra) asm volatile("s_waitcnt vmcnt(%0)" ::"n"(4 * PA + 1) : "memory");
+            if (NBW == 2 && extra == 2) asm volatile("s_waitcnt vmcnt(%0)" ::"n"(4 * PA + 2) : "memory");
+            else if (extra) asm volatile("s_waitcnt vmcnt(%0)" ::"n"(4 * PA + 1) : "memory");
             else asm volatile("s_waitcnt vmcnt(%0)" ::"n"(4 * PA) : "memory");
         } else asm volatile("s_waitcnt vmcnt(0)" ::: "memory");
         __builtin_amdgcn_s_barrier();
@@ -121,40 +139,59 @@
         const bool more = c + POOL_NBUF - 1 < c1;
         const uint32_t ft = lds_addr(lds + cur * PA * POOL_FT);
         const uint32_t wb = lds_addr(lbits + (((c - c0) >> 1) & 1) * (NR64 * 4));
-        u32x4_t xf[PA][4];
-#pragma unroll
-        for (int p = 0; p < PA; ++p)
-#pragma unroll
-            for (int t = 0; t < 4; ++t)
-                xf[p][t] = lds_read128_asm(ft + 2 * (p * POOL_FT + frow * POOL_CHUNK + (((g * 4 + t) ^ pool_swz(frow)) * 8)));
+        u32x4_t xf[CTW][PA][4];
+#pragma unroll
+        for (int j = 0; j < CTW; ++j)
+#pragma unroll
+            for (int p = 0; p < PA; ++p)
+#pragma unroll
+                for (int t = 0; t < 4; ++t)
+                    xf[j][p][t] = lds_read128_asm(ft + 2 * (p * POOL_FT + (frow + 32 * j) * POOL_CHUNK + (((g * 4 + t) ^ pool_swz(frow)) * 8)));
         uint32_t w[NRT];
 #pragma unroll
         for (int rt = 0; rt < NRT; ++rt)
-            w[rt] = lds_read32_asm(wb + 4 * ((rt * 32 + (lane & 31)) * 4 + pos * 2 + g));
+            w[rt] = lds_read32_asm(wb + 4 * ((set * Npad + rt * 32 + (lane & 31)) * 4 + pos * 2 + g));
         asm volatile("s_waitcnt lgkmcnt(0)" ::: "memory");
         __builtin_amdgcn_sched_barrier(0);
         if (counting) {
 #pragma unroll
             for (int rt = 0; rt < NRT; ++rt) pc[rt] += __popc(w[rt]);
         }
+        auto lut_read = [&](uint32_t word, int t) { return lds_read128_asm(lut_addr + (((word >> (8 * t)) & 0xFFu) << 4)); };
+        auto mfma_step = [&](int rt, const u32x4_t& at, int t) {
+#pragma unroll
+            for (int p = 0; p < PA; ++p)
+#pragma unroll
+                for (int j = 0; j < CTW; ++j)
+                    acc[rt][j] = mfma32e<E>(__builtin_bit_cast(uint4, at), __builtin_bit_cast(uint4, xf[j][p][t]), acc[rt][j]);
+        };
         u32x4_t a[2][4];
 #pragma unroll
-        for (int t = 0; t < 4; ++t) a[0][t] = lds_read128_asm(lut_addr + (((w[0] >> (8 * t)) & 0xFFu) << 4));
+        for (int t = 0; t < 4; ++t) a[0][t] = lut_read(w[0], t);
 #pragma unroll
         for (int rt = 0; rt < NRT; ++rt) {
+            constexpr int AHEAD = CTW == 2 ? 2 : 4;
             if (rt + 1 < NRT) {
 #pragma unroll
-                for (int t = 0; t < 4; ++t) a[(rt + 1) & 1][t] = lds_read128_asm(lut_addr + (((w[rt + 1] >> (8 * t)) & 0xFFu) << 4));
-                asm volatile("s_waitcnt lgkmcnt(4)" ::: "memory");
+                for (int t = 0; t < AHEAD; ++t) a[(rt + 1) & 1][t] = lut_read(w[rt + 1], t);
+                if (AHEAD == 2) asm volatile("s_waitcnt lgkmcnt(2)" ::: "memory");
+                else asm volatile("s_waitcnt lgkmcnt(4)" ::: "memory");
             } else {
                 asm volatile("s_waitcnt lgkmcnt(0)" ::: "memory");
             }
             __builtin_amdgcn_sched_barrier(0);
 #pragma unroll
-            for (int t = 0; t < 4; ++t)
-#pragma unroll
-                for (int p = 0; p < PA; ++p)
-                    acc[rt] = mfma32e<E>(__builtin_bit_cast(uint4, a[rt & 1][t]), __builtin_bit_cast(uint4, xf[p][t]), acc[rt]);
+            for (int t = 0; t < AHEAD; ++t) mfma_step(rt, a[rt & 1][t], t);
+            if (AHEAD < 4) {
+                __builtin_amdgcn_sched_barrier(0);
+                if (rt + 1 < NRT) {
+#pragma unroll
+                    for (int t = AHEAD; t < 4; ++t) a[(rt + 1) & 1][t] = lut_read(w[rt + 1], t);
+                }
+                __builtin_amdgcn_sched_barrier(0);
+#pragma unroll
+                for (int t = AHEAD; t < 4; ++t) mfma_step(rt, a[rt & 1][t], t);
+            }
             __builtin_amdgcn_sched_barrier(0);
             if (rt == 0 && pos == 0 && c + 2 < c1) issue_pair_bits(c + 2, (((c - c0) >> 1) + 1) & 1);
             if (more) {
@@ -167,33 +204,37 @@
     }
 
     if (counting) {
+        int32_t* pcs = set ? pcountB : pcount;
 #pragma unroll
         for (int rt = 0; rt < NRT; ++rt) {
             const int tot = pc[rt] + __shfl_xor(pc[rt], 32);
-            if (lane < 32) pcount[((int64_t)b * nsplit + split) * Npad + rt * 32 + lane] = tot;
+            if (lane < 32) pcs[((int64_t)b * nsplit + split) * Npad + rt * 32 + lane] = tot;
         }
     }
-    float* out = partial + (((int64_t)b * nsplit + split) * Npad) * 512 + map * 256 + ch0 + wave * 32 + (lane & 31);
+    float* out = (set ? partialB : partial) + (((int64_t)b * nsplit + split) * Npad) * 512 + map * 256 + ch0 + wch + (lane & 31);
 #pragma unroll
     for (int rt = 0; rt < NRT; ++rt)
 #pragma unroll
-        for (int r = 0; r < 16; ++r) {
-            const int row = rt * 32 + (r & 3) + 8 * (r >> 2) + 4 * g;
-            out[(int64_t)row * 512] = acc[rt][r];
-        }
-}
-
-template <int PA, int NRT, int E>
+        for (int j = 0; j < CTW; ++j)
+#pragma unroll
+            for (int r = 0; r < 16; ++r) {
+                const int row = rt * 32 + (r & 3) + 8 * (r >> 2) + 4 * g;
+                out[(int64_t)row * 512 + 32 * j] = acc[rt][j][r];
+            }
+}
+
+template <int PA, int NRT, int E, int NS = 1>
 static void launch_pool(const uint16_t* x, const uint16_t* d, const uint32_t* bits, float* partial, int B, int64_t HWp,
-                        int nsplit, int bits_rows, int32_t* pcount, hipStream_t s) {
-    const size_t lds = (size_t)POOL_NBUF * PA * POOL_FT * sizeof(uint16_t) + 256 * 16 + (size_t)2 * ((NRT * 32 + 63) / 64) * 64 * 16;
+                        int nsplit, int bits_rows, int32_t* pcount, hipStream_t s, const uint32_t* bitsB = nullptr,
+                        float* partialB = nullptr, int32_t* pcountB = nullptr) {
+    const size_t lds = (size_t)POOL_NBUF * PA * POOL_FT * sizeof(uint16_t) + 256 * 16 + (size_t)2 * ((NS * NRT * 32 + 63) / 64) * 64 * 16;
     static const bool once = [&] {
-        (void)hipFuncSetAttribute((const void*)k_pool<PA, NRT, E>, hipFuncAttributeMaxDynamicSharedMemorySize, (int)lds);
+        (void)hipFuncSetAttribute((const void*)k_pool<PA, NRT, E, NS>, hipFuncAttributeMaxDynamicSharedMemorySize, (int)lds);
         return true;
     }();
     (void)once;
-    hipLaunchKernelGGL((k_pool<PA, NRT, E>), dim3(nsplit, d ? 4 : 2, B), dim3(256), lds, s, x, d, bits, partial, B, HWp,
-                       nsplit, bits_rows, pcount);
+    hipLaunchKernelGGL((k_pool<PA, NRT, E, NS>), dim3(nsplit, d ? 4 : 2, B), dim3(256), lds, s, x, d, bits, partial, B, HWp,
+                       nsplit, bits_rows, pcount, bitsB, partialB, pcountB);
 }
 
 static int pool_run(const uint16_t* xplanes, const uint16_t* dplanes, const uint32_t* bits, int bits_rows, float* partial, int32_t* pcount,
@@ -242,6 +283,37 @@
     return pool_run(xplanes, dplanes, bits, 0, partial, pcount, B, N, HW, nsplit, prec, stream, __func__);
 }
 
+extern "C" int ph_pool_depth_pair_supported(int N, int prec) {
+    return N > 0 && N <= 160 && (prec == PH_PREC_BF16 || prec == PH_PREC_F16);
+}
+
+extern "C" int ph_pool_depth_pair(const uint16_t* dplanes, const uint32_t* bitsA, const uint32_t* bitsB, float* partialA, float* partialB,
+                                  int32_t* pcountA, int32_t* pcountB, int B, int N, int64_t HW, int nsplit, int prec, void* stream) {
+    PH_CHECK_ARG(dplanes && bitsA && bitsB && partialA && partialB && pcountA && pcountB && B > 0 && N > 0 && HW > 0, "bad pointer or size");
+    if (!ph_pool_depth_pair_supported(N, prec)) {
+        ph_set_error("ph_pool_depth_pair: unsupported query count or plane format (use ph_pool_counts once per mask set)");
+        return PH_EUNSUPPORTED;
+    }
+    const int64_t HWp = ph_hw_padded(HW);
+    PH_CHECK_ARG(nsplit >= 1 && nsplit <= HWp / POOL_CHUNK, "nsplit out of range");
+    const int nrt = ph_n_padded(N) / 32;
+    hipStream_t s = (hipStream_t)stream;
+#define PH_PAIR_CASE(R)                                                                                                                  \
+    case R:                                                                                                                              \
+        if (prec == PH_PREC_BF16)                                                                                                        \
+            launch_pool<1, R, PH_E_BF16, 2>(dplanes, nullptr, bitsA, partialA + 256, B, HWp, nsplit, R * 32, pcountA, s, bitsB, partialB + 256, pcountB); \
+        else                                                                                                                             \
+            launch_pool<1, R, PH_E_F16, 2>(dplanes, nullptr, bitsA, partialA + 256, B, HWp, nsplit, R * 32, pcountA, s, bitsB, partialB + 256, pcountB);  \
+        break;
+    switch (nrt) {
+        PH_PAIR_CASE(1) PH_PAIR_CASE(2) PH_PAIR_CASE(3) PH_PAIR_CASE(4) PH_PAIR_CASE(5)
+        default: ph_set_error("ph_pool_depth_pair: unsupported N"); return PH_EUNSUPPORTED;
+    }
+#undef PH_PAIR_CASE
+    PH_CHECK_LAUNCH();
+    return PH_OK;
+}
+
 extern "C" int ph_pool_default_nsplit(int B, int64_t HW, int frame_invariant) {
     const int64_t nchunks = ph_hw_padded(HW) / 128;
     int64_t ns = 512 / (4 * (int64_t)(frame_invariant || B < 1 ? 1 : B));
diff --git a/polyphonicformer_amd/csrc/ph_query.hip b/polyphonicformer_amd/csrc/ph_query.hip
--- a/polyphonicformer_amd/csrc/ph_query.hip
+++ b/polyphonicformer_amd/csrc/ph_query.hip
@@ -260,6 +260,7 @@
     QArgs q;
     unsigned long long* tl;
     float* pi;
+    int br0, nbr;
 };
 
 #define PH_TL(k)                                                                                             \
@@ -281,7 +282,7 @@
     const int tid = threadIdx.x, lane = tid & 63;
     const int wave = __builtin_amdgcn_readfirstlane(tid >> 6);
     const int i = lane & 15, g = lane >> 4;
-    const int row0 = blockIdx.x * ROWS, br = blockIdx.y, b = blockIdx.z;
+    const int row0 = blockIdx.x * ROWS, br = blockIdx.y + aa.br0, b = blockIdx.z;
     const int N = a.N, Npad = a.Npad;
     const uint16_t* wb = a.wb;
     const int64_t wpl = a.lay.wb_plane_elems;
@@ -575,7 +576,7 @@
     const int tid = threadIdx.x, lane = tid & 63;
     const int wave = __builtin_amdgcn_readfirstlane(tid >> 6);
     const int i = lane & 15, g = lane >> 4;
-    const int row0 = blockIdx.x * ROWS, br = blockIdx.y, b = blockIdx.z;
+    const int row0 = blockIdx.x * ROWS, br = blockIdx.y + aa.br0, b = blockIdx.z;
     const uint16_t* wb = a.wb;
     const int64_t wpl = a.lay.wb_plane_elems;
     const float* wf = a.wf;
@@ -923,7 +924,7 @@
             return true;
         }();
         (void)once;
-        const dim3 grid(a.q.Npad / ROWS, 2, a.q.B);
+        const dim3 grid(a.q.Npad / ROWS, a.nbr, a.q.B);
         if (phases & 1) hipLaunchKernelGGL((k_query_pre2<2, NRT, true>), grid, dim3(NTHREADS), lds_pre, s, a);
         if (phases & 2) hipLaunchKernelGGL((k_query_post2<1, NRT, PH_E_F16>), grid, dim3(NTHREADS), lds_post, s, a);
         return;
@@ -938,7 +939,7 @@
         return true;
     }();
     (void)once;
-    const dim3 grid(a.q.Npad / ROWS, 2, a.q.B);
+    const dim3 grid(a.q.Npad / ROWS, a.nbr, a.q.B);
     if (phases & 1) hipLaunchKernelGGL((k_query_pre2<PA, NRT>), grid, dim3(NTHREADS), lds_pre, s, a);
     if (phases & 2) hipLaunchKernelGGL((k_query_post2<PA, NRT>), grid, dim3(NTHREADS), lds_post, s, a);
 }
@@ -948,8 +949,9 @@
                      float* cls, int cls_sigmoid, uint16_t* kern, float* kbias, void* workspace,
                      size_t workspace_bytes, int B, int N, int64_t HW, int prec, int kern_format, int phases,
                      void* stream) {
-    PH_CHECK_ARG((phases & ~(PH_QUERY_BOTH | PH_QUERY_WIDE)) == 0 && (phases & PH_QUERY_BOTH) != 0,
-                 "phases must be PH_QUERY_PRE | PH_QUERY_POST [| PH_QUERY_WIDE]");
+    PH_CHECK_ARG((phases & ~(PH_QUERY_BOTH | PH_QUERY_WIDE | PH_QUERY_MASK_ONLY | PH_QUERY_DEPTH_ONLY)) == 0 && (phases & PH_QUERY_BOTH) != 0 &&
+                     (phases & (PH_QUERY_MASK_ONLY | PH_QUERY_DEPTH_ONLY)) != (PH_QUERY_MASK_ONLY | PH_QUERY_DEPTH_ONLY),
+                 "phases must be PH_QUERY_PRE | PH_QUERY_POST [| PH_QUERY_WIDE] [| PH_QUERY_MASK_ONLY or PH_QUERY_DEPTH_ONLY]");
     PH_CHECK_ARG(partial && bits && k_in && q_in && wb && wf && layout && obj && dobj && cls && kern && kbias && workspace,
                  "null pointer");
     PH_CHECK_ARG(B > 0 && N > 0 && N <= 256 && HW > 0 && nsplit >= 1, "bad size");
@@ -961,6 +963,7 @@
     const bool hybrid = prec == PH_PREC_QHYBRID;
     const int PA = (prec == PH_PREC_SPLIT || hybrid) ? 2 : 1, Npad = ph_n_padded(N);
     const bool wide = (phases & PH_QUERY_WIDE) != 0;
+    const int br0 = (phases & PH_QUERY_DEPTH_ONLY) ? 1 : 0, nbr = (phases & (PH_QUERY_MASK_ONLY | PH_QUERY_DEPTH_ONLY)) ? 1 : 2;
     phases &= PH_QUERY_BOTH;
     if (workspace_bytes < q_ws_bytes(B, Npad, PA)) {
         ph_set_error("ph_query_stage: workspace too small (%zu < %zu)", workspace_bytes, q_ws_bytes(B, Npad, PA));
@@ -978,6 +981,7 @@
     unsigned long long* tl = kn.timeline;
     a2.tl = tl;
     a2.pi = a.o1 + (size_t)B * 2 * Npad * 256;
+    a2.br0 = br0; a2.nbr = nbr;
     const int t = Npad / 16;
     int nrt = 1;
     if (wide) {
diff --git a/polyphonicformer_amd/engine.py b/polyphonicformer_amd/engine.py
--- a/polyphonicformer_amd/engine.py
+++ b/polyphonicformer_amd/engine.py
@@ -156,6 +156,13 @@
                                   _lib.stream_ptr()), "ph_pool_counts(depth)")
 
 
+def pool_depth_pair(dp, bits_a, bits_b, N, HW, prec, partial_a, partial_b, counts_a, counts_b):
+    B, nsplit = partial_a.shape[0], partial_a.shape[1]
+    _lib.check(_lib.load().ph_pool_depth_pair(_lib.ptr(dp), _lib.ptr(bits_a), _lib.ptr(bits_b), _lib.ptr(partial_a), _lib.ptr(partial_b),
+                                              _lib.ptr(counts_a), _lib.ptr(counts_b), B, N, HW, nsplit, prec, _lib.stream_ptr()),
+               "ph_pool_depth_pair")
+
+
 def dynconv_up2(planes, kern, kbias, branch, N, H, W, prec, up_out, logits_out=None, out_dtype=_lib.PH_OUT_F16, workgroups=0):
     B, Npad = kern.shape[2], kern.shape[3]
     lib = _lib.load()
@@ -189,6 +196,9 @@
     lib = _lib.load()
     _lib.check(lib.ph_upsample2x(_lib.ptr(src), _lib.ptr(out), dt, planes, H, W, _lib.stream_ptr()), "ph_upsample2x")
     return out
+
+
+POOL_PAIR = knobs.get("PH_POOL_PAIR") != "0"
 
 
 def _knob_code(off, on, on_code):
@@ -217,7 +227,7 @@
 class DecodePlan:
 
     def __init__(self, packs, B, N, H, W, prec, out_dtype=torch.float32, device="cuda:0", nsplit=None, frame_invariant=False,
-                 shares_gpu=False):
+                 shares_gpu=False, pair=None):
         self.packs, self.S = packs, len(packs)
         self.frame_invariant, self.shares_gpu = frame_invariant, shares_gpu
         self.feat_is_bf16 = False
@@ -265,6 +275,10 @@
         if self.poolx:
             self.partial_px = e((B, self.nsplit_px, Npad, 512), torch.float32)
             self.pcount_px = e((B, self.nsplit_px, Npad), torch.int32)
+        self.pair = bool((POOL_PAIR if pair is None else pair) and self.poolx and self.S >= 3 and
+                         _lib.load().ph_pool_depth_pair_supported(N, self.prec))
+        if self.pair:
+            self.bits_b, self.partial_px_b, self.pcount_px_b = (torch.empty_like(t) for t in (self.bits, self.partial_px, self.pcount_px))
 
     @property
     def out_code(self):
@@ -307,22 +321,37 @@
         xp = self.xp if xp is None else xp
         dp = self.dp if dp is None else dp
         k, q = self.k0, self.q0
+        cv = self.mode.conv
+
+        def query(s, part, bits, cnt, branches=0):
+            return query_stage(part, bits, k, q, self.packs[s], self.N, self.HW, cls_sigmoid=s == self.S - 1,
+                               outs=self.stage_out[s], workspace=self.ws, kern_fmt=self.mode.kern_fmt, counts=cnt,
+                               phases=3 | (_lib.PH_QUERY_WIDE if self.shares_gpu else 0) | branches)
+
         for s in range(self.S):
             last = s == self.S - 1
+            bits = self.bits_b if self.pair and last else self.bits
             if self.debug_bits is not None:
-                self.debug_bits.append(self.bits.clone())
-            if s > 0 and self.poolx:
-                pool_depth_only(dp, self.bits, self.N, self.HW, self.prec, self.partial_px, self.pcount_px)
+                self.debug_bits.append(bits.clone())
+            if self.pair and s == self.S - 2:
+                o = query(s, self.partial_px, bits, None, _lib.PH_QUERY_MASK_ONLY)
+                dynconv_poolx(xp, o["kern"], o["kbias"], self.N, self.HW, cv, self.bits_b, self.partial_px_b)
+                pool_depth_pair(dp, bits, self.bits_b, self.N, self.HW, self.prec, self.partial_px, self.partial_px_b,
+                                self.pcount_px, self.pcount_px_b)
+                query(s, self.partial_px, bits, self.pcount_px, _lib.PH_QUERY_DEPTH_ONLY)
+                k, q = o["obj"], o["dobj"]
+                continue
+            if self.pair and last:
+                part, cnt = self.partial_px_b, self.pcount_px_b
+            elif s > 0 and self.poolx:
+                pool_depth_only(dp, bits, self.N, self.HW, self.prec, self.partial_px, self.pcount_px)
                 part, cnt = self.partial_px, self.pcount_px
             else:
-                pool(xp, dp, self.bits, self.N, self.HW, self.prec, self.nsplit, out=self.partial, counts=self.pcount)
+                pool(xp, dp, bits, self.N, self.HW, self.prec, self.nsplit, out=self.partial, counts=self.pcount)
                 part, cnt = self.partial, self.pcount
             if s == 0 and self.on_first_pool is not None:
                 self.on_first_pool()
-            o = query_stage(part, self.bits, k, q, self.packs[s], self.N, self.HW, cls_sigmoid=last,
-                            outs=self.stage_out[s], workspace=self.ws, kern_fmt=self.mode.kern_fmt, counts=cnt,
-                            phases=3 | (_lib.PH_QUERY_WIDE if self.shares_gpu else 0))
-            cv = self.mode.conv
+            o = query(s, part, bits, cnt)
             if not last:
                 if self.poolx:
                     dynconv_poolx(xp, o["kern"], o["kbias"], self.N, self.HW, cv, self.bits, self.partial_px)
diff --git a/polyphonicformer_amd/knobs.py b/polyphonicformer_amd/knobs.py
--- a/polyphonicformer_amd/knobs.py
+++ b/polyphonicformer_amd/knobs.py
@@ -10,6 +10,9 @@
          "`0` never / `1` wherever it exists: the stage-boundary conv also pools (`ph_dynconv_poolx`); anything else: the library's rule"),
     Knob("PH_CONV_UP2", "text", "auto", "plan cfg", "engine.native_cfg",
          "`0` never / `1` wherever it exists: final stage as `ph_dynconv_up2`; anything else: the library's rule (fused from B·H ≥ 512, §4.4b)"),
+    Knob("PH_POOL_PAIR", "text", "1", "import", "engine.POOL_PAIR",
+         "`0`: the last two stages pool depth_feats in a launch each; anything else: in one paired launch where "
+         "`ph_pool_depth_pair_supported` (`DecodePlan` with the fused conv + pooling and S ≥ 3, §4.2; same bits either way)"),
     Knob("PH_POOL_NSPLIT", "int", None, "plan cfg", "engine.native_cfg, native_khead_cfg, default_nsplit",
          "pixel ranges of the pooling kernels (cfg field `nsplit`; an `nsplit` argument wins).  Known oddity: `0` means the "
          "library's rule in the cfg builders, while `engine.default_nsplit` returns the 0"),
```
